# cxzheng/sprsolve

Hardware: AMD Instinct MI355X
Metric: BiCGStab iterations/s (f64, 50M-row 7-point 3-D Poisson) + CSR SpMV GB/s vs HBM roofline (higher is better)
Workload: dtype f64

## Files before the change

sprsolve_amd/csrc/bicg_fuse.hpp:

```cpp
#pragma once
#include "fused_launch.hpp"
#include "krylov.hpp"

namespace sprs {

template <class T, class V, bool PC>
struct BicgK1 {
    BicgState<T> *S; const Real<T> *partN; const T *partRho; int P; int mode;
    const T *v; const T *r; T *p; const V *dinv; T *y;
    T a, beta;
    unsigned int tag = 0; unsigned long long mb_timeout = 0;
    __device__ __forceinline__ bool prologue() {
        __shared__ Real<T> smD[NWAVE];
        __shared__ T smT[NWAVE];
        const int status = S->status;
        const Real<T> tol2 = S->tol2, r0_norm_tol = S->r0_norm_tol;
        const T w = S->w, rho_old = S->rho_old, alpha = S->alpha;
        T rho; Real<T> r_norm;
        if (mode == 0) {
            Real<T> sN; T sR;
            if (tag != 0) {
                if (status != ST_RUNNING) return false;
                if (!mbox_sum2(MboxSrc{reinterpret_cast<const unsigned long long *>(partN), P, tag, mb_timeout}, sN, sR)) {
                    if (first_thread()) S->status = ST_COMM_TIMEOUT;
                    return false;
                }
            } else {
                reduce_partials2(partN, partRho, P, smD, smT, sN, sR);
                if (status != ST_RUNNING) return false;
            }
            r_norm = ssqrt(sN);
            if (r_norm <= tol2) {
                if (first_thread()) { S->r_norm = r_norm; S->status = ST_CONVERGED; }
                return false;
            }
            rho = sR;
            if (sabs(rho) < r0_norm_tol) {
                if (first_thread()) { S->r_norm = r_norm; S->status = ST_RESTART; }
                return false;
            }
        } else {
            if (status != ST_RUNNING) return false;
            rho = S->rho; r_norm = S->r_norm;
        }
        beta = smul(sdiv(rho, rho_old), sdiv(alpha, w));
        a = smul(sneg(beta), w);
        if (first_thread()) { S->rho = rho; S->r_norm = r_norm; S->beta = beta; }
        return true;
    }
    template <int PK, bool NT> __device__ __forceinline__ void run(int64_t i) const {
        auto vv = ldp<T, PK, NT>(v, i); auto pv = ldp<T, PK, NT>(p, i); auto rv = ldp<T, PK, NT>(r, i);
        Pack<T, PK> yv;
        [[maybe_unused]] Pack<V, PK> dv;
        if (PC) dv = ldp<V, PK, NT>(dinv, i);
#pragma unroll
        for (int e = 0; e < PK; ++e) {
            T t = sadd(smul(vv.v[e], a), smul(pv.v[e], beta));
            t = sadd(t, smul(rv.v[e], sone<T>()));
            pv.v[e] = t;
            if (PC) yv.v[e] = smulv(t, dv.v[e]);
        }
        stp<T, PK, NT>(p, i, pv);
        if (PC) stp<T, PK, NT>(y, i, yv);
    }
    __device__ __forceinline__ void epilogue() const {}
};

template <class T, class V, bool PC>
struct BicgK3 {
    BicgState<T> *S; const T *partB; int P; int check_breakdown;
    const T *v; T *r; const V *dinv; T *z;
    T na;
    unsigned int tag = 0; unsigned long long mb_timeout = 0;
    __device__ __forceinline__ bool prologue() {
        __shared__ T smT[NWAVE];
        const int status = S->status;
        const T rho = S->rho;
        T tmp;
        if (tag != 0) {
            if (status != ST_RUNNING) return false;
            if (!mbox_sum1(MboxSrc{reinterpret_cast<const unsigned long long *>(partB), P, tag, mb_timeout}, tmp)) {
                if (first_thread()) S->status = ST_COMM_TIMEOUT;
                return false;
            }
        } else {
            tmp = reduce_partials(partB, P, smT);
            if (status != ST_RUNNING) return false;
        }
        if (check_breakdown && sabs(tmp) <= 0.0) {
            if (first_thread()) S->status = ST_BREAKDOWN;
            return false;
        }
        const T alpha = sdiv(rho, tmp);
        na = sneg(alpha);
        if (first_thread()) S->alpha = alpha;
        return true;
    }
    template <int PK, bool NT> __device__ __forceinline__ void run(int64_t i) const {
        auto vv = ldp<T, PK, NT>(v, i); auto rv = ldp<T, PK, NT>(r, i);
        Pack<T, PK> zv;
        [[maybe_unused]] Pack<V, PK> dv;
        if (PC) dv = ldp<V, PK, NT>(dinv, i);
#pragma unroll
        for (int e = 0; e < PK; ++e) {
            rv.v[e] = sadd(rv.v[e], smul(vv.v[e], na));
            if (PC) zv.v[e] = smulv(rv.v[e], dv.v[e]);
        }
        stp<T, PK, NT>(r, i, rv);
        if (PC) stp<T, PK, NT>(z, i, zv);
    }
    __device__ __forceinline__ void epilogue() const {}
};

int launch_chain_k4f(const sprs_csr *A, const SpmvRoute &rt, const BicgK3<double, double, false> &pro, const double *r, const double *v, double *s_out,
                     double *t, double *partTT, double *partTR, const int *status);
int launch_chain_k2f(const sprs_csr *A, const SpmvRoute &rt, const BicgK1<double, double, false> &pro, const double *v_old, const double *p, const double *r,
                     double *p_out, double *v_out, const double *r0, double *partB, const int *status);

template <class T, bool PC, bool SV = false>
struct BicgK5 {
    BicgState<T> *S; const T *partTT; const T *partTR; int P;
    const T *y; const T *z; const T *t; const T *r0; T *x; T *r; Real<T> *partN; T *partRho;
    Fin fin;
    T na, nw, w;
    Real<T> accN; T accR;
    unsigned int tag = 0; unsigned long long mb_timeout = 0;
    const T *sv = nullptr;
    __device__ __forceinline__ bool prologue() {
        __shared__ T smT[NWAVE];
        __shared__ T smT2[NWAVE];
        const int status = S->status;
        const T alpha = S->alpha;
        T tt, tr;
        if (tag != 0) {
            if (status != ST_RUNNING) { fin_idle(fin, true); return false; }
            if (!mbox_sum2(MboxSrc{reinterpret_cast<const unsigned long long *>(partTT), P, tag, mb_timeout}, tt, tr)) {
                if (first_thread()) S->status = ST_COMM_TIMEOUT;
                return false;
            }
        } else {
            reduce_partials2(partTT, partTR, P, smT, smT2, tt, tr);
        }
        if (status != ST_RUNNING) { fin_idle(fin, true); return false; }
        w = (sre(tt) > 0.0) ? sdiv(tr, tt) : szero<T>();
        na = sneg(alpha); nw = sneg(w);
        accN = 0.0; accR = szero<T>();
        return true;
    }
    template <int PK, bool NT> __device__ __forceinline__ void run(int64_t i) {
        auto xv = ldp<T, PK, NT>(x, i); auto yv = ldp<T, PK, NT>(y, i); auto rv = ldp<T, PK, NT>(r, i);
        auto tv = ldp<T, PK, NT>(t, i); auto qv = ldp<T, PK, NT>(r0, i);
        [[maybe_unused]] Pack<T, PK> zv;
        if (PC) zv = ldp<T, PK, NT>(z, i);
        if constexpr (SV) {
            const auto vv = ldp<T, PK, NT>(sv, i);
#pragma unroll
            for (int e = 0; e < PK; ++e) rv.v[e] = sadd(rv.v[e], smul(vv.v[e], na));
        }
#pragma unroll
        for (int e = 0; e < PK; ++e) {
            T xx = sadd(xv.v[e], smul(yv.v[e], na));
            xx = sadd(xx, smul(PC ? zv.v[e] : rv.v[e], nw));
            xv.v[e] = xx;
            const T rr = sadd(rv.v[e], smul(tv.v[e], nw));
            rv.v[e] = rr;
            accN = accN + ssq(rr);
            accR = sadd(accR, smul(sconj(qv.v[e]), rr));
        }
        stp<T, PK, NT>(x, i, xv);
        stp<T, PK, NT>(r, i, rv);
    }
    __device__ __forceinline__ void epilogue() {
        __shared__ Real<T> smD[NWAVE];
        __shared__ T smT[NWAVE];
        const Real<T> sN = block_sum(accN, smD);
        const T sR = block_sum(accR, smT);
        if (threadIdx.x == 0) { st_partial(fin, partN + blockIdx.x, sN); st_partial(fin, partRho + blockIdx.x, sR); }
        if (first_thread()) { S->w = w; S->rho_old = S->rho; S->its = S->its + 1; }
        if (fin.counter) finalize_last_block<Real<T>, T>(fin, true, smD, smT);
    }
};

}
```

sprsolve_amd/csrc/capi.hip:

```cpp
#include <sys/mman.h>

#include <cstdlib>
#include <memory>
#include <new>
#include <string>

#include "krylov.hpp"

using namespace sprs;

static_assert(sizeof(sprs_c64) == sizeof(cplx), "Complex<f64> layout");
static_assert(sizeof(sprs_c32) == sizeof(cplxf), "Complex<f32> layout");

#define SPRS_GUARD_BEGIN try {
#define SPRS_GUARD_END                         \
    }                                          \
    catch (const std::bad_alloc &) {           \
        return SPRS_ERR_HIP;                   \
    }                                          \
    catch (...) {                              \
        return SPRS_ERR_HIP;                   \
    }

extern "C" {
// ... 445 lines not shown
    h->dtype = dtype_of<T>::value;
    auto *s = new S<T>();
    h->impl = s;
    int st = mk(s);
    if (st != SPRS_OK) { s->destroy(); delete s; delete h; return st; }
    *out = h;
    return SPRS_OK;
}

template <template <class> class S>
int solver_destroy(sprs_solver_handle *h) {
    if (!h) return SPRS_OK;
    with_solver<S>(h->dtype, h->impl, [](auto *s) { (void)hipStreamSynchronize(s->ctx->stream); s->destroy(); delete s; return (int)SPRS_OK; });
    delete h;
    return SPRS_OK;
}

template <class T, class SolverT>
int solve(SolverT *s, bool host, const sprs_diag *P, const T *rhs, size_t rl, T *x, size_t xl, size_t max_iter, Real<T> tol,
          size_t *its, Real<T> *res) {
    if (!s || !rhs || !x) return SPRS_INVALID_ARGUMENT;
    if (rl != s->n) return SPRS_INCOMPATIBLE_RHS_SIZE;
    if (xl != s->n) return SPRS_INCOMPATIBLE_X_SIZE;
    sprs_ctx *c = s->ctx;
    CtxLock lock(c);
    if (!host && ((reinterpret_cast<uintptr_t>(rhs) | reinterpret_cast<uintptr_t>(x)) & 15) == 0)
        return s->solve_dev(P, rhs, rl, x, xl, max_iter, tol, its, res);
    const hipMemcpyKind in = host ? hipMemcpyHostToDevice : hipMemcpyDeviceToDevice, out = host ? hipMemcpyDeviceToHost : hipMemcpyDeviceToDevice;
    SPRS_HIP_TRY(c, hipSetDevice(c->device));
    if (!s->rhs_buf) SPRS_HIP_TRY(c, hipMalloc((void **)&s->rhs_buf, sizeof(T) * s->stride));
    if (!s->x_buf) SPRS_HIP_TRY(c, hipMalloc((void **)&s->x_buf, sizeof(T) * s->stride));
    SPRS_HIP_TRY(c, hipMemcpyAsync(s->rhs_buf, rhs, sizeof(T) * rl, in, c->stream));
    SPRS_HIP_TRY(c, hipMemcpyAsync(s->x_buf, x, sizeof(T) * xl, in, c->stream));
    int st = s->solve_dev(P, s->rhs_buf, rl, s->x_buf, xl, max_iter, tol, its, res);
    if (st >= SPRS_ERR_HIP) return st;
    SPRS_HIP_TRY(c, hipMemcpyAsync(x, s->x_buf, sizeof(T) * xl, out, c->stream));
    SPRS_HIP_TRY(c, hipStreamSynchronize(c->stream));
    return st;
}

template <class T>
int solve_many(CgMany<T> *s, bool host, const sprs_diag *P, const T *rhs, size_t rl, T *x, size_t xl, size_t k, size_t max_iter,
               Real<T> tol, size_t *its, Real<T> *res, int *status) {
    if (!s || !rhs || !x) return SPRS_INVALID_ARGUMENT;
    if (k < 1 || k > (size_t)s->kmax) return SPRS_INVALID_ARGUMENT;
    if (rl != s->n * k) return SPRS_INCOMPATIBLE_RHS_SIZE;
    if (xl != s->n * k) return SPRS_INCOMPATIBLE_X_SIZE;
    sprs_ctx *c = s->ctx;
    CtxLock lock(c);
    if (!host) return s->solve_dev(P, rhs, rl, x, xl, k, max_iter, tol, its, res, status);
    SPRS_HIP_TRY(c, hipSetDevice(c->device));
    const size_t cap = (s->n * (size_t)s->kmax) + 1;
    if (!s->rhs_buf) SPRS_HIP_TRY(c, hipMalloc((void **)&s->rhs_buf, sizeof(T) * cap));
    if (!s->x_buf) SPRS_HIP_TRY(c, hipMalloc((void **)&s->x_buf, sizeof(T) * cap));
    SPRS_HIP_TRY(c, hipMemcpyAsync(s->rhs_buf, rhs, sizeof(T) * rl, hipMemcpyHostToDevice, c->stream));
    SPRS_HIP_TRY(c, hipMemcpyAsync(s->x_buf, x, sizeof(T) * xl, hipMemcpyHostToDevice, c->stream));
    int st = s->solve_dev(P, s->rhs_buf, rl, s->x_buf, xl, k, max_iter, tol, its, res, status);
    if (st >= SPRS_ERR_HIP || st == SPRS_DIM_MISMATCH || st == SPRS_INVALID_ARGUMENT) return st;
    SPRS_HIP_TRY(c, hipMemcpyAsync(x, s->x_buf, sizeof(T) * xl, hipMemcpyDeviceToHost, c->stream));
    SPRS_HIP_TRY(c, hipStreamSynchronize(c->stream));
    return st;
}

template <template <class> class S, class T>
S<T> *impl_of(sprs_solver_handle *h) { return (h && h->dtype == dtype_of<T>::value) ? (S<T> *)h->impl : nullptr; }

}

template <class F>
static int with_base(void *solver, int kind, F &&f) {
    auto *h = (sprs_solver_handle *)solver;
    if (!h) return SPRS_INVALID_ARGUMENT;
    switch (kind) {
        case SPRS_SOLVER_BICGSTAB: return with_solver<BicgStab>(h->dtype, h->impl, f);
        case SPRS_SOLVER_CG: return with_solver<Cg>(h->dtype, h->impl, f);
        case SPRS_SOLVER_GMRES: return with_solver<Gmres>(h->dtype, h->impl, f);
        case SPRS_SOLVER_MINRES:
        case SPRS_SOLVER_CSMINRES: return with_solver<MinRes>(h->dtype, h->impl, f);
    }
    return SPRS_INVALID_ARGUMENT;
}


#define SPRS_CHK(c) do { if (!(c)) return SPRS_INVALID_ARGUMENT; } while (0)
#define SPRS_G(...) try { __VA_ARGS__ } catch (...) { return SPRS_ERR_HIP; }

extern "C" {

int sprs_csr_destroy(sprs_csr *A) {
    if (!A) return SPRS_OK;
    if (A->ctx) { (void)hipSetDevice(A->ctx->device); (void)hipStreamSynchronize(A->ctx->stream); }
    if (A->owns_arrays) {
        if (A->row_ptr) (void)hipFree(A->row_ptr);
        if (A->col_idx) (void)hipFree(A->col_idx);
        if (A->val) (void)hipFree(A->val);
    }
    if (A->rowblk) (void)hipFree(A->rowblk);
    if (A->blk_desc) (void)hipFree(A->blk_desc);
    if (A->blk_desc_eq) (void)hipFree(A->blk_desc_eq);
    if (A->tail) (void)hipFree(A->tail);
    free_dict(A);
    if (A->x_tmp) (void)hipFree(A->x_tmp);
    if (A->y_tmp) (void)hipFree(A->y_tmp);
    if (A->part) (void)hipFree(A->part);
    if (A->dist) {
        if (A->dist->send_idx) (void)hipFree(A->dist->send_idx);
        if (A->dist->send_buf) (void)hipFree(A->dist->send_buf);
        if (A->dist->ag_buf) (void)hipFree(A->dist->ag_buf);
        if (A->dist->order_int) (void)hipFree(A->dist->order_int);
        if (A->dist->order_bnd) (void)hipFree(A->dist->order_bnd);
        for (void *q : {(void *)A->dist->tile_int.list, (void *)A->dist->tile_int.xstart, (void *)A->dist->tile_int.left}) if (q) (void)hipFree(q);
        if (A->dist->order_int_w) (void)hipFree(A->dist->order_int_w);
        if (A->dist->order_bnd_w) (void)hipFree(A->dist->order_bnd_w);
        if (A->dist->ev_pack) (void)hipEventDestroy(A->dist->ev_pack);
        if (A->dist->ev_halo) (void)hipEventDestroy(A->dist->ev_halo);
        if (A->dist->comm_stream) (void)hipStreamDestroy(A->dist->comm_stream);
        delete A->dist;
    }
    delete A;
    return SPRS_OK;
}
int64_t sprs_csr_rows(const sprs_csr *A) { return A ? A->nrows : -1; }
int64_t sprs_csr_cols(const sprs_csr *A) { return A ? A->ncols : -1; }
int64_t sprs_csr_nnz(const sprs_csr *A) { return A ? A->nnz : -1; }
int sprs_csr_wide_blocks(const sprs_csr *A, int64_t *n_blocks, int64_t *n_uniform) {
    if (!A || !n_blocks || !n_uniform) return SPRS_INVALID_ARGUMENT;
    *n_blocks = 0; *n_uniform = 0;
    const SpmvRoute r = spmv_route(A, SpmvPart::Whole, false);
    if (r.format == 0) {
        *n_blocks = A->n_rowblk; *n_uniform = A->blk_desc_eq ? A->n_eq_blocks : 0;
        return SPRS_OK;
    }
    const sprs_dict *D = A->dict;
    const bool one_line = r.format == 2 && D->wide_desc && (A->nrows < 2 || A->ncols < 2) && A->ctx->spmv_wide != 0;
    const bool wide = (D->wide_desc && r.desc == D->wide_desc) || one_line;
    const void *src = wide ? D->wide_desc : (D->off_desc && r.desc == D->off_desc ? D->off_desc : nullptr);
    const int64_t nb = wide ? D->n_wide : (src ? A->n_rowblk : 0);
    if (!src || nb == 0) return SPRS_OK;
    sprs_ctx *c = A->ctx;
    CtxLock lock(c);
    std::vector<int32_t> d((size_t)nb * 4);
    SPRS_HIP_TRY(c, hipSetDevice(c->device));
    SPRS_HIP_TRY(c, hipMemcpyAsync(d.data(), src, d.size() * sizeof(int32_t), hipMemcpyDeviceToHost, c->stream));
    SPRS_HIP_TRY(c, hipStreamSynchronize(c->stream));
    *n_blocks = nb;
    for (int64_t j = 0; j < nb; ++j) *n_uniform += ((uint32_t)d[(size_t)j * 4 + 1] & sprs::UNI2) != 0;
    return SPRS_OK;
}
int sprs_csr_tile_plan(const sprs_csr *A, int64_t *n_tiles, int64_t *n_tile_blocks, int64_t *n_other_blocks) {
    if (!A || !n_tiles || !n_tile_blocks || !n_other_blocks) return SPRS_INVALID_ARGUMENT;
    *n_tiles = 0; *n_tile_blocks = 0; *n_other_blocks = 0;
    const bool split = A->dist && A->dist->order_int;
    const SpmvRoute r = spmv_route(A, split ? SpmvPart::Interior : SpmvPart::Whole, false);
    if (r.kernel != SpmvKernel::TilePair && r.kernel != SpmvKernel::TileOff) return SPRS_OK;
    const sprs_tile_plan &TP = *r.tile;
    *n_tiles = TP.n_tile; *n_tile_blocks = (int64_t)TP.n_tile * sprs::tile_blocks();
    if (split) *n_other_blocks = (A->n_rowblk + 1) / 2 - *n_tile_blocks;
    else *n_other_blocks = r.kernel == SpmvKernel::TilePair ? TP.n_left : (TP.n_left + 1) / 2;
    return SPRS_OK;
}
int sprs_csr_chain_plan(const sprs_csr *A, int64_t *n_tiles, int64_t *n_segments, int64_t *n_chains, int64_t *n_other_blocks) {
    if (!A || !n_tiles || !n_segments || !n_chains || !n_other_blocks) return SPRS_INVALID_ARGUMENT;
    *n_tiles = 0; *n_segments = 0; *n_chains = 0; *n_other_blocks = 0;
    const SpmvRoute r = spmv_route(A, SpmvPart::Whole, false);
    if (r.kernel != SpmvKernel::Chain) return SPRS_OK;
    *n_tiles = r.chain->n_tile; *n_segments = r.chain->n_seg; *n_chains = r.chain->n_chain; *n_other_blocks = r.chain->n_left;
    return SPRS_OK;
}
int sprs_csr_spmv_route(const sprs_csr *A, int part, int conj_x, int *kernel, int *format, int *grid, int64_t *n_blocks,
                        int *ordered, int *y_nt) {
    if (!A || part < 0 || part > 2 || !kernel || !format || !grid || !n_blocks || !ordered || !y_nt) return SPRS_INVALID_ARGUMENT;
    *kernel = -1; *format = 0; *grid = 0; *n_blocks = 0; *ordered = 0; *y_nt = 0;
    if (part != 0 && !(A->dist && A->dist->order_int)) return SPRS_OK;
    const SpmvRoute r = spmv_route(A, part == 0 ? SpmvPart::Whole : part == 1 ? SpmvPart::Interior : SpmvPart::Boundary, conj_x != 0);
    *kernel = (int)r.kernel; *format = r.format; *grid = r.grid; *n_blocks = r.count; *ordered = r.order ? 1 : 0; *y_nt = r.y_nt ? 1 : 0;
    return SPRS_OK;
}
int sprs_csr_stream_format(const sprs_csr *A, int *n_offsets, int *n_values) {
    if (!A) return -1;
    if (n_offsets) *n_offsets = A->dict ? A->dict->n_off : 0;
    if (n_values) *n_values = A->dict ? (A->dict->n_pair ? A->dict->n_pair : 0) : 0;
    return spmv_route(A, SpmvPart::Whole, false).format;
}

int sprs_diag_precond_destroy(sprs_diag *P) {
    if (!P) return SPRS_OK;
    if (P->ctx) { (void)hipSetDevice(P->ctx->device); (void)hipStreamSynchronize(P->ctx->stream); }
    if (P->dinv) (void)hipFree(P->dinv);
    if (P->in_tmp) (void)hipFree(P->in_tmp);
    if (P->out_tmp) (void)hipFree(P->out_tmp);
    delete P;
    return SPRS_OK;
}
int sprs_bicgstab_destroy(sprs_bicgstab *S) { return solver_destroy<BicgStab>(S); }
int sprs_minres_destroy(sprs_minres *S) { return solver_destroy<MinRes>(S); }
int sprs_csminres_destroy(sprs_csminres *S) { return solver_destroy<MinRes>(S); }
int sprs_cg_destroy(sprs_cg *S) { return solver_destroy<Cg>(S); }
int sprs_gmres_destroy(sprs_gmres *S) { return solver_destroy<Gmres>(S); }
int sprs_cgmany_destroy(sprs_cg_many *S) { return solver_destroy<CgMany>(S); }

#define SPRS_SOLVER_SOLVES(X, T, CT, R, NAME, S)                                                                       \
    int sprs_##NAME##_solve_##X(sprs_##NAME *h, const CT *rhs, size_t rl, CT *x, size_t xl, size_t mi, R tol, size_t *its, R *res) { \
        SPRS_G(return solve<T>(impl_of<S, T>(h), true, nullptr, (const T *)rhs, rl, (T *)x, xl, mi, tol, its, res);)   \
    }                                                                                                                  \
    int sprs_##NAME##_precond_solve_##X(sprs_##NAME *h, const sprs_diag *P, const CT *rhs, size_t rl, CT *x, size_t xl, size_t mi, R tol, size_t *its, R *res) { \
        SPRS_G(if (!P) return SPRS_INVALID_ARGUMENT; return solve<T>(impl_of<S, T>(h), true, P, (const T *)rhs, rl, (T *)x, xl, mi, tol, its, res);) \
    }                                                                                                                  \
    int sprs_##NAME##_solve_dev_##X(sprs_##NAME *h, const sprs_diag *P, const CT *rhs, size_t rl, CT *x, size_t xl, size_t mi, R tol, size_t *its, R *res) { \
        SPRS_G(return solve<T>(impl_of<S, T>(h), false, P, (const T *)rhs, rl, (T *)x, xl, mi, tol, its, res);)        \
    }
#define SPRS_SOLVER_API(X, T, CT, R, NAME, S, CREATE)                                                                  \
    int sprs_##NAME##_create_##X(const sprs_csr *A, size_t n, sprs_##NAME **out) {                                     \
        SPRS_G(return (solver_create<T, sprs_##NAME, S>(A, n, out, [&](auto *s) { return s->create CREATE; }));)       \
    }                                                                                                                  \
    SPRS_SOLVER_SOLVES(X, T, CT, R, NAME, S)

#define SPRS_API(X, T, CT, R)                                                                                          \
    int sprs_csr_create_##X(sprs_ctx *c, int64_t nr, int64_t nc, int64_t nnz, const int32_t *rp, const int32_t *ci,    \
                            const CT *v, int csc, sprs_csr **out) {                                                    \
        SPRS_G(return csr_create_host<T, int32_t>(c, nr, nc, nnz, rp, ci, (const T *)v, csc, out);)                    \
    }                                                                                                                  \
    int sprs_csr_create_i64_##X(sprs_ctx *c, int64_t nr, int64_t nc, int64_t nnz, const int64_t *rp,                   \
                                const int64_t *ci, const CT *v, int csc, sprs_csr **out) {                             \
        SPRS_G(return csr_create_host<T, int64_t>(c, nr, nc, nnz, rp, ci, (const T *)v, csc, out);)                    \
    }                                                                                                                  \
    int sprs_csr_create_dev_##X(sprs_ctx *c, int64_t nr, int64_t nc, int64_t nnz, const int32_t *rp,                   \
                                const int32_t *ci, const CT *v, int adopt, sprs_csr **out) {                           \
        SPRS_G(return csr_create_dev<T>(c, nr, nc, nnz, rp, ci, (const T *)v, adopt, out);)                            \
    }                                                                                                                  \
    int sprs_mul_vec_##X(const sprs_csr *A, const CT *x, size_t xl, CT *y, size_t yl) {                                \
        SPRS_G(return mul_vec_host<T>(A, (const T *)x, xl, (T *)y, yl, nullptr);)                                      \
    }                                                                                                                  \
    int sprs_mul_vec_dot_##X(const sprs_csr *A, const CT *x, size_t xl, CT *y, size_t yl, CT *d) {                     \
        SPRS_G(if (!d) return SPRS_INVALID_ARGUMENT; return mul_vec_host<T>(A, (const T *)x, xl, (T *)y, yl, (T *)d);) \
    }                                                                                                                  \
    int sprs_mul_vec_dev_##X(const sprs_csr *A, const CT *x, CT *y) { return mul_vec_dev<T>(A, (const T *)x, (T *)y, nullptr); } \
    int sprs_mul_vec_dot_dev_##X(const sprs_csr *A, const CT *x, CT *y, CT *d) {                                       \
        if (!d) return SPRS_INVALID_ARGUMENT;                                                                          \
        return mul_vec_dev<T>(A, (const T *)x, (T *)y, (T *)d);                                                        \
    }                                                                                                                  \
    int sprs_mul_vec_dev_timed_##X(const sprs_csr *A, const CT *x, CT *y, int reps, double *ms) {                      \
        return mul_vec_timed<T>(A, (const T *)x, (T *)y, reps, ms);                                                    \
    }                                                                                                                  \
    int sprs_mul_mat_##X(const sprs_csr *A, const CT *x, size_t xl, CT *y, size_t yl, size_t k) {                      \
        SPRS_G(return mul_mat_host<T>(A, (const T *)x, xl, (T *)y, yl, k);)                                            \
    }                                                                                                                  \
    int sprs_mul_mat_dev_##X(const sprs_csr *A, const CT *x, CT *y, size_t k) { return mul_mat_dev<T>(A, (const T *)x, (T *)y, k); } \
                                                               \
    int sprs_cgmany_create_##X(const sprs_csr *A, size_t n, size_t k, sprs_cg_many **out) {                           \
        SPRS_G(if (k < 1 || k > 8) { if (out) *out = nullptr; return SPRS_INVALID_ARGUMENT; }                          \
               return (solver_create<T, sprs_cg_many, CgMany>(A, n, out, [&](auto *s) { return s->create(A, n, k); }));) \
    }                                                                                                                  \
    int sprs_cgmany_solve_##X(sprs_cg_many *h, const sprs_diag *P, const CT *rhs, size_t rl, CT *x, size_t xl, size_t k, size_t mi, R tol, \
                               size_t *its, R *res, int *status) {                                                     \
        SPRS_G(return solve_many<T>(impl_of<CgMany, T>(h), true, P, (const T *)rhs, rl, (T *)x, xl, k, mi, tol, its, res, status);) \
    }                                                                                                                  \
    int sprs_cgmany_solve_dev_##X(sprs_cg_many *h, const sprs_diag *P, const CT *rhs, size_t rl, CT *x, size_t xl, size_t k, size_t mi, R tol, \
                                   size_t *its, R *res, int *status) {                                                 \
        SPRS_G(return solve_many<T>(impl_of<CgMany, T>(h), false, P, (const T *)rhs, rl, (T *)x, xl, k, mi, tol, its, res, status);) \
    }                                                                                                                  \
    int sprs_dot_##X(sprs_ctx *c, size_t n, const CT *x, const CT *y, CT *o) { SPRS_CHK(c && o); return dot_host<T>(c, n, (const T *)x, (const T *)y, false, (T *)o); } \
    int sprs_conj_dot_##X(sprs_ctx *c, size_t n, const CT *x, const CT *y, CT *o) { SPRS_CHK(c && o); return dot_host<T>(c, n, (const T *)x, (const T *)y, true, (T *)o); } \
    int sprs_norm2_##X(sprs_ctx *c, size_t n, const CT *x, R *o) { SPRS_CHK(c && o); return norm2_host<T>(c, n, (const T *)x, o); } \
    int sprs_scale_##X(sprs_ctx *c, size_t n, CT a, CT *x) { SPRS_CHK(c); T aa; memcpy(&aa, &a, sizeof(T)); return launch_scale<T>(c, n, aa, (T *)x); } \
    int sprs_rscale_##X(sprs_ctx *c, size_t n, R a, CT *x) { SPRS_CHK(c); return launch_rscale<T>(c, n, a, (T *)x); }  \
    int sprs_conj_##X(sprs_ctx *c, size_t n, const CT *in, CT *out) { SPRS_CHK(c); return launch_conj<T>(c, n, (const T *)in, (T *)out); } \
    int sprs_axpy_##X(sprs_ctx *c, size_t n, CT a, const CT *x, CT *y) { SPRS_CHK(c); T aa; memcpy(&aa, &a, sizeof(T)); return launch_axpy<T, T>(c, n, aa, (const T *)x, (T *)y); } \
    int sprs_axpby_##X(sprs_ctx *c, size_t n, CT a, const CT *x, CT b, CT *y) {                                        \
        SPRS_CHK(c); T aa, bb; memcpy(&aa, &a, sizeof(T)); memcpy(&bb, &b, sizeof(T));                                 \
        return launch_axpby<T>(c, n, aa, (const T *)x, bb, (T *)y);                                                    \
    }                                                                                                                  \
    int sprs_diag_mul_vec_##X(const sprs_diag *P, const CT *in, size_t il, CT *out, size_t ol) {                       \
        SPRS_G(return diag_apply_host<T>(P, (const T *)in, il, (T *)out, ol);)                                         \
    }                                                                                                                  \
    int sprs_diag_mul_vec_dev_##X(const sprs_diag *P, const CT *in, CT *out) { return diag_apply_dev<T>(P, (const T *)in, (T *)out); } \
    SPRS_SOLVER_API(X, T, CT, R, bicgstab, BicgStab, (A, n))                                                           \
    SPRS_SOLVER_API(X, T, CT, R, minres, MinRes, (A, n, false))                                                        \
    SPRS_SOLVER_API(X, T, CT, R, cg, Cg, (A, n))                                                                       \
                                                                  \
    int sprs_gmres_create_##X(const sprs_csr *A, size_t n, size_t restart, sprs_gmres **out) {                         \
        SPRS_G(if (restart > SPRS_GMRES_MAX_RESTART) return SPRS_INVALID_ARGUMENT;                                     \
               return (solver_create<T, sprs_gmres, Gmres>(A, n, out, [&](auto *s) { return s->create(A, n, restart); }));) \
    }                                                                                                                  \
    SPRS_SOLVER_SOLVES(X, T, CT, R, gmres, Gmres)                                                                      \
                                                                      \
    int sprs_csminres_create_##X(const sprs_csr *A, size_t n, sprs_csminres **out) {                                   \
        SPRS_G(return (solver_create<T, sprs_csminres, MinRes>(A, n, out, [&](auto *s) { return s->create(A, n, true); }));) \
    }                                                                                                                  \
    int sprs_csminres_solve_##X(sprs_csminres *h, const CT *rhs, size_t rl, CT *x, size_t xl, size_t mi, R tol, size_t *its, R *res) { \
        SPRS_G(return solve<T>(impl_of<MinRes, T>(h), true, nullptr, (const T *)rhs, rl, (T *)x, xl, mi, tol, its, res);) \
    }                                                                                                                  \
    int sprs_csminres_solve_dev_##X(sprs_csminres *h, const CT *rhs, size_t rl, CT *x, size_t xl, size_t mi, R tol, size_t *its, R *res) { \
        SPRS_G(return solve<T>(impl_of<MinRes, T>(h), false, nullptr, (const T *)rhs, rl, (T *)x, xl, mi, tol, its, res);) \
    }

SPRS_API(d, double, double, double)
SPRS_API(z, cplx, sprs_c64, double)
SPRS_API(s, float, float, float)
SPRS_API(c, cplxf, sprs_c32, float)

int sprs_axpy_zd(sprs_ctx *c, size_t n, double a, const sprs_c64 *x, sprs_c64 *y) { SPRS_CHK(c); return launch_axpy<cplx, double>(c, n, a, (const cplx *)x, (cplx *)y); }
int sprs_axpy_cs(sprs_ctx *c, size_t n, float a, const sprs_c32 *x, sprs_c32 *y) { SPRS_CHK(c); return launch_axpy<cplxf, float>(c, n, a, (const cplxf *)x, (cplxf *)y); }

int sprs_diag_precond_create_d(sprs_ctx *c, size_t n, const double *d, sprs_diag **out) { SPRS_G(return diag_create<double>(c, n, d, DT_D, out);) }
int sprs_diag_precond_create_zd(sprs_ctx *c, size_t n, const double *d, sprs_diag **out) { SPRS_G(return diag_create<double>(c, n, d, DT_Z, out);) }
int sprs_diag_precond_create_z(sprs_ctx *c, size_t n, const sprs_c64 *d, sprs_diag **out) { SPRS_G(return diag_create<cplx>(c, n, (const cplx *)d, DT_Z, out);) }
int sprs_diag_precond_create_s(sprs_ctx *c, size_t n, const float *d, sprs_diag **out) { SPRS_G(return diag_create<float>(c, n, d, DT_S, out);) }
int sprs_diag_precond_create_cs(sprs_ctx *c, size_t n, const float *d, sprs_diag **out) { SPRS_G(return diag_create<float>(c, n, d, DT_C, out);) }
int sprs_diag_precond_create_c(sprs_ctx *c, size_t n, const sprs_c32 *d, sprs_diag **out) { SPRS_G(return diag_create<cplxf>(c, n, (const cplxf *)d, DT_C, out);) }

int sprs_solver_set_mode(void *solver, int kind, int mode) {
    if (mode != 0 && mode != 1) return SPRS_INVALID_ARGUMENT;
    return with_base(solver, kind, [&](auto *b) { b->mode = mode; return (int)SPRS_OK; });
}
int sprs_solver_set_trace(void *solver, int kind, double *trace_host, size_t cap) {
    return with_base(solver, kind, [&](auto *b) { b->trace = trace_host; b->trace_cap = trace_host ? cap : 0; b->trace_rows = 0; return (int)SPRS_OK; });
}
int sprs_solver_trace_rows(const void *solver, int kind, size_t *rows_out) {
    if (!rows_out) return SPRS_INVALID_ARGUMENT;
// ... 35 lines not shown
```

sprsolve_amd/csrc/internal.hpp:

```cpp
#pragma once
#include <hip/hip_runtime.h>
#include <hip/hip_ext.h>
#include <cstdint>
#include <cstdio>
#include <cstring>
#include <cstdlib>
#include <ctime>
#include <mutex>
#include <type_traits>
#include <vector>

#include "../../include/sprsolve_hip.h"
#include "scalar.hpp"

namespace sprs {

constexpr int BLOCK = 256;
constexpr uint32_t UNI2 = 0x40000000u;
constexpr uint32_t SEAM2 = 0x20000000u;
constexpr int MAX_GRID = 4096;

enum : int { ST_RUNNING = 0, ST_CONVERGED = 1, ST_RESTART = 2, ST_BREAKDOWN = 3, ST_INVALID_PC = 4,
             ST_COMM_TIMEOUT = 5 };

// ... 6 lines not shown
    int world, rank;
};

struct Fin {
    unsigned int *counter = nullptr;
    const void *base0 = nullptr, *base1 = nullptr;
    void *out0 = nullptr, *out1 = nullptr;
    int P = 0;
    const P2pBox *box = nullptr;
    unsigned int tag = 0;
    unsigned int mb_off = 0;
};

}

struct sprs_ctx {
    int device = 0;
    hipStream_t stream = nullptr;
    bool own_stream = false;
    int num_cu = 256;
    int grid = 512;
    int spmv_grid = -1;
    int xcd_chunk = -1;
    int spmv_dict = -1;
    int spmv_wide = -1;
    int spmv_wideload = -1;
    int spmv_eqrows = -1;
    int spmv_period = -1;
    int spmv_triple = -1;
    int spmv_seam = -1;
    int spmv_tile = -1;
    int spmv_chain = -1;
    int spmv_fuse = -1;
    int ew_chunk = -1;
    int stream_nt = -1;
    int spmv_uniform = -1;
    int halo_overlap = 1;
    int gs_graph = 0;
    int p2p_allreduce = -1;
    int p2p_timeout_ms = 20000;
    int poll = 16;
    double *d_part = nullptr;
    double *d_scal = nullptr;
    double *h_scal = nullptr;
    mutable char err[512] = {0};
    hipEvent_t prof_start = nullptr, prof_stop = nullptr;
    mutable std::recursive_mutex mu;
};
struct CtxLock {
    std::unique_lock<std::recursive_mutex> lk;
    explicit CtxLock(const sprs_ctx *c) { if (c) lk = std::unique_lock<std::recursive_mutex>(c->mu); }
};

#define SPRS_HIP_TRY(ctx, expr)                                                                     \
    do {                                                                                            \
        hipError_t e__ = (expr);                                                                    \
        if (e__ != hipSuccess) {                                                                    \
            snprintf((ctx)->err, sizeof((ctx)->err), "%s:%d: %s -> %s", __FILE__, __LINE__, #expr,  \
                     hipGetErrorString(e__));                                                       \
            return SPRS_ERR_HIP;                                                                    \
        }                                                                                           \
    } while (0)

#define SPRS_LAUNCH_SPMV(c, kernel, grid, ...)                                                                            \
    do {                                                                                                                 \
        if ((c)->prof_start && (c)->prof_stop)                                                                           \
            hipExtLaunchKernelGGL(kernel, dim3(grid), dim3(sprs::BLOCK), 0, (c)->stream, (c)->prof_start, (c)->prof_stop, 0, __VA_ARGS__); \
        else                                                                                                             \
            hipLaunchKernelGGL(kernel, dim3(grid), dim3(sprs::BLOCK), 0, (c)->stream, __VA_ARGS__);                      \
    } while (0)

struct CreateTrace {
    bool on; double t0;
    static double now() { timespec ts; clock_gettime(CLOCK_MONOTONIC, &ts); return ts.tv_sec * 1e3 + ts.tv_nsec * 1e-6; }
    CreateTrace() : on(getenv("SPRS_CREATE_TRACE") != nullptr), t0(now()) {}
    void lap(const char *what) { if (!on) return; const double t = now(); fprintf(stderr, "[sprs create] %-28s %8.2f ms\n", what, t - t0); t0 = t; }
};

#define SPRS_TRY(expr)                       \
    do {                                     \
        int s__ = (expr);                    \
        if (s__ != SPRS_OK) return s__;      \
    } while (0)

struct sprs_comm {
    sprs_ctx *ctx = nullptr;
    void *nccl = nullptr;
    int world = 1, rank = 0;
    bool p2p = false;
    void *mbox = nullptr;
    void *peer_map[8] = {nullptr};
    sprs::P2pBox *d_box = nullptr;
    unsigned int seq[4] = {0, 0, 0, 0};
};

struct sprs_tile_plan {
    int32_t *list = nullptr;
    int32_t *xstart = nullptr;
    int32_t *left = nullptr;
    int n_tile = 0, n_left = 0;
    int ul = 0, fl = 0, fh = 0;
    int w = 0;
    int32_t off[8] = {0, 0, 0, 0, 0, 0, 0, 0};
    double val[8] = {0, 0, 0, 0, 0, 0, 0, 0};
    std::vector<int32_t> h_list, h_xstart;
};

struct sprs_chain_plan {
    int32_t *tiles = nullptr;
    int32_t *segs = nullptr;
    int32_t *xstart = nullptr;
    int32_t *left = nullptr;
    int n_tile = 0, n_seg = 0, n_chain = 0, n_left = 0;
    int ul = 0, tri = 0;
    int32_t off[8] = {0, 0, 0, 0, 0, 0, 0, 0};
    double val[8] = {0, 0, 0, 0, 0, 0, 0, 0};
};

struct sprs_dist_info {
    sprs_comm *comm = nullptr;
    int64_t n_local = 0, n_ext = 0;
    std::vector<int> peer;
    std::vector<int64_t> send_off, recv_off;
    int32_t *send_idx = nullptr;
    void *send_buf = nullptr;
    int64_t ag_slice = 0;
    void *ag_buf = nullptr;
    int32_t *order_int = nullptr, *order_bnd = nullptr;
    int32_t n_int = 0, n_bnd = 0;
    int32_t *order_int_w = nullptr, *order_bnd_w = nullptr;
    sprs_tile_plan tile_int;
    bool tile_int_off = false;
    int32_t n_int_w = 0, n_bnd_w = 0;
    hipStream_t comm_stream = nullptr;
    hipEvent_t ev_pack = nullptr, ev_halo = nullptr;
};

struct sprs_dict {
    uint8_t *idx_code = nullptr;
    uint8_t *pair_code = nullptr;
    int32_t *off_tab = nullptr;
    int32_t *pair_off = nullptr;
    void *pair_val = nullptr;
    void *rowval = nullptr;
    int n_off = 0, n_val = 0, n_pair = 0;
    void *wide_desc = nullptr;
    int n_wide = 0;
    int32_t *wide_order = nullptr;
    int32_t *off_order = nullptr;
    int64_t period = 0;
    int64_t max_off = -1;
    sprs_tile_plan tile_pair, tile_off;
    sprs_chain_plan chain_pair;
    void *owide_desc = nullptr;
    int n_owide = 0;
    void *off_desc = nullptr;
    int n_off_uniform = 0;
};

struct sprs_csr {
    sprs_ctx *ctx = nullptr;
    int dtype = 0;
    int64_t nrows = 0, ncols = 0, nnz = 0;
    int32_t *row_ptr = nullptr;
    int32_t *col_idx = nullptr;
    void *val = nullptr;
    bool owns_arrays = true;
    bool was_csc = false;
    int32_t *rowblk = nullptr;
    int32_t n_rowblk = 0;
    void *blk_desc = nullptr;
    void *blk_desc_eq = nullptr;
    int32_t n_eq_blocks = 0;
    void *tail = nullptr;
    void *x_tmp = nullptr, *y_tmp = nullptr;
    double *part = nullptr;
    sprs_dist_info *dist = nullptr;
    sprs_dict *dict = nullptr;
};

struct sprs_diag {
    sprs_ctx *ctx = nullptr;
    int t_dtype = 0;
    int v_complex = 0;
    size_t n = 0;
    void *dinv = nullptr;
    void *in_tmp = nullptr, *out_tmp = nullptr;
};

namespace sprs {

enum class SpmvPart { Whole, Interior, Boundary };
enum class SpmvKernel {
    Csr,
    CsrWide,
    Dict,
    DictWide,
    Pair2,
    TilePair,
    TileOff,
    Chain,
};
struct BlkDesc;
struct SpmvRoute {
    SpmvKernel kernel;
    int format;
    int grid;
    int xcd_chunk;
    const BlkDesc *desc;
    const int32_t *order;
    int count;
    const sprs_tile_plan *tile;
    const sprs_chain_plan *chain;
    bool y_nt;
};
SpmvRoute spmv_route(const sprs_csr *A, SpmvPart part, bool conj_x);
template <class T>
int launch_spmv(const sprs_csr *A, SpmvPart part, const T *x, T *y, int dot_mode, const T *u, T *part0, T *part1,
                const int *status, bool conj_x = false, const Fin *fin = nullptr);
int spmv_num_partials(const sprs_csr *A);
template <class F>
inline void with_dot(int dot_mode, bool flag, F &&f) {
    auto go = [&](auto dm) { if (flag) f(dm, std::true_type{}); else f(dm, std::false_type{}); };
    if (dot_mode == 0) go(std::integral_constant<int, 0>{});
    else if (dot_mode == 1) go(std::integral_constant<int, 1>{});
    else go(std::integral_constant<int, 2>{});
}
int tile_blocks();
int build_rowblocks(sprs_csr *A, const int32_t *host_row_ptr);
int validate_cols_device(const sprs_csr *A);
int rowblk_spans(const sprs_csr *A, std::vector<int32_t> &lo, std::vector<int32_t> &hi);
int build_dict(sprs_csr *A, bool has_vector_blocks, const std::vector<int32_t> &blk, const std::vector<int32_t> &blk_pa);
void free_dict(sprs_csr *A);
bool fused_chunked(const sprs_csr *A);
template <class T>
int launch_dict(const sprs_csr *A, const SpmvRoute &r, const T *x, T *y, int dot_mode, const T *u, T *part0, T *part1,
                const int *status, bool conj_x, const Fin &fin);
int launch_dict_wide(const sprs_csr *A, const SpmvRoute &r, const double *x, double *y, int dot_mode, const double *u,
                     double *part0, double *part1, const int *status, const Fin &fin);
int launch_pair2(const sprs_csr *A, const SpmvRoute &r, const double *x, double *y, int dot_mode, const double *u,
                 double *part0, double *part1, const int *status, const Fin &fin);
int launch_tile_pair(const sprs_csr *A, const SpmvRoute &r, const double *x, double *y, int dot_mode, const double *u,
                     double *part0, double *part1, const int *status, const Fin &fin);
int launch_tile_off(const sprs_csr *A, const SpmvRoute &r, const double *x, double *y, int dot_mode, const double *u,
                    double *part0, double *part1, const int *status, const Fin &fin);
int launch_chain_pair(const sprs_csr *A, const SpmvRoute &r, const double *x, double *y, int dot_mode, const double *u,
                      double *part0, double *part1, const int *status, const Fin &fin);

template <class T>
int launch_spmm(const sprs_csr *A, const T *x, T *y, int ld, int k, int dot_mode, const T *u, T *part, const int *running);
int spmm_grid(const sprs_csr *A);

template <class T, class S> int launch_axpy(sprs_ctx *c, size_t n, S a, const T *x, T *y);
template <class T> int launch_axpby(sprs_ctx *c, size_t n, T a, const T *x, T b, T *y);
template <class T> int launch_scale(sprs_ctx *c, size_t n, T a, T *x);
template <class T> int launch_rscale(sprs_ctx *c, size_t n, Real<T> a, T *x);
template <class T> int launch_conj(sprs_ctx *c, size_t n, const T *in, T *out);
template <class T, class V> int launch_diag_apply(sprs_ctx *c, size_t n, const V *dinv, const T *in, T *out);
template <class V> int launch_diag_inv(sprs_ctx *c, size_t n, const V *diag, V *dinv);
template <class T> int dot_host(sprs_ctx *c, size_t n, const T *x, const T *y, bool conj, T *out, sprs_comm *comm = nullptr);
template <class T> int norm2_host(sprs_ctx *c, size_t n, const T *x, Real<T> *out, sprs_comm *comm = nullptr);
template <class T> int reduce_partials_host(sprs_ctx *c, const T *part, int P, T *out, sprs_comm *comm = nullptr);

template <class T> int halo_exchange(const sprs_csr *A, T *x_ext);
template <class T> int halo_begin(const sprs_csr *A, T *x_ext);
int halo_wait(const sprs_csr *A);
template <class T>
int dist_spmv(const sprs_csr *A, T *x_ext, T *y, int dot_mode, const T *u, T *part0, T *part1, const int *status, bool conj_x,
              const Fin *fin = nullptr);
int allreduce_sum(sprs_comm *comm, void *dev, size_t count, bool f32 = false);

inline int grid_for(const sprs_ctx *c) {
    int g = c->grid;
    if (g < 8) g = 8;
    if (g > MAX_GRID) g = MAX_GRID;
    return g & ~7;
}

inline bool stream_loads_nt(const sprs_ctx *c, size_t vector_bytes) {
    if (c->stream_nt >= 0) return c->stream_nt != 0;
    return vector_bytes >= (size_t)72 << 20;
}
inline bool is_cache_resident(const sprs_csr *A) {
    const double s = (double)dtype_size(A->dtype);
    return (double)A->nnz * (s + 4) + 3.0 * A->nrows * s < 192.0 * 1024 * 1024;
}

inline bool tile_wanted(const sprs_ctx *c, size_t vector_bytes) {
    if (c->spmv_tile >= 0) return c->spmv_tile != 0;
    return vector_bytes >= (size_t)44 << 20;
}

inline int balanced_grid(const sprs_ctx *c, int64_t work) {
    const int g0 = grid_for(c);
    if (work <= g0) return (int)(work < 1 ? 1 : work);
    const int64_t trips = (work + g0 - 1) / g0;
    int64_t g = (work + trips - 1) / trips;
    g = (g + 7) & ~(int64_t)7;
    return (int)(g > g0 ? g0 : g);
}

}
```

sprsolve_amd/csrc/spmv.hip:

```cpp
#include <algorithm>
#include <memory>
#include <system_error>
#include <thread>

#include "device.hpp"

namespace sprs {

struct BlkDescHost { int32_t ra, rb, pa, nn; };

template <class F>
static void host_parallel_for(int64_t n, int64_t min_chunk, F &&f) {
    auto call = [&](int64_t a, int64_t b, int t) {
        if constexpr (std::is_invocable_v<F, int64_t, int64_t, int>) f(a, b, t); else f(a, b);
    };
    int64_t T = std::min<int64_t>(std::max(1u, std::thread::hardware_concurrency()), 16);
    T = std::max<int64_t>(1, std::min<int64_t>(T, n / std::max<int64_t>(min_chunk, 1)));
    if (T <= 1) { call(0, n, 0); return; }
    std::vector<std::thread> th;
    const int64_t per = (n + T - 1) / T;
    for (int64_t t = 0; t < T; ++t) {
        const int64_t a = t * per, b = std::min<int64_t>(n, a + per);
        if (a >= b) break;
        try { th.emplace_back(call, a, b, (int)t); } catch (const std::system_error &) { call(a, b, (int)t); }
// ... 367 lines not shown
    for (; b < bend; b += bstep) {
        const BlkDesc d = desc[order ? order[b] : b];
        if (run_state != ST_RUNNING) { fin_idle(fin, DOT == 2); return; }
        const bool eq_rows = eq_desc != 0 && ((uint32_t)d.rb & UNI2) != 0;
        const int ra = d.ra, rb = d.rb & (eq_desc ? 0x3fffffff : 0x7fffffff);
        if (d.rb >= 0) {
            const int pa = d.pa, nn = eq_desc ? (d.nn & 0xffff) : d.nn;
            const int shift = pa & 3, tot = nn + shift;
            const int r = ra + lane;
            const bool has_row = r < rb;
            const int rcl = has_row ? r : rb - 1;
            int s, e;
            if (eq_rows) { const int L = d.nn >> 16; s = (rcl - ra) * L; e = s + L; }
            else { s = row_ptr[rcl] - pa; e = row_ptr[rcl + 1] - pa; }
            [[maybe_unused]] T uu;
            if (DOT != 0) uu = u[rcl];
            if (nn > 0) {
                const int g0 = (pa - shift) >> 2, lastq = (tot - 1) >> 2;
                v4i32 c[2]; D2v v[2][2];
#pragma unroll
                for (int i = 0; i < 2; ++i) {
                    const int G = g0 + min(lane + i * WAVE, lastq);
                    const bool tl = G == g_last;
                    const v4i32 *cp = tl ? tail_c : col4 + G;
                    const D2v *vp = tl ? tail_v : val2 + 2 * (int64_t)G;
                    c[i] = *cp; v[i][0] = vp[0]; v[i][1] = vp[1];
                }
                T xg[8];
#pragma unroll
                for (int i = 0; i < 2; ++i) { xg[4 * i] = x[c[i].x]; xg[4 * i + 1] = x[c[i].y]; xg[4 * i + 2] = x[c[i].z]; xg[4 * i + 3] = x[c[i].w]; }
#pragma unroll
                for (int i = 0; i < 2; ++i) {
                    const int k = 4 * (lane + i * WAVE);
                    const D2v p0{xg[4 * i] * v[i][0].a, xg[4 * i + 1] * v[i][0].b}, p1{xg[4 * i + 2] * v[i][1].a, xg[4 * i + 3] * v[i][1].b};
                    if (k < tot) { *reinterpret_cast<D2v *>(prod + k) = p0; *reinterpret_cast<D2v *>(prod + k + 2) = p1; }
                }
            }
            wave_lds_fence();
            if (has_row) {
                T acc = 0.0;
                const int len = e - s;
                const T *pr = prod + shift;
                if (len <= 8) {
                    T pv[8];
#pragma unroll
                    for (int j = 0; j < 8; ++j) pv[j] = pr[min(s + j, CAP + 3)];
#pragma unroll
                    for (int j = 0; j < 8; ++j)
                        if (j < len) acc = acc + pv[j];
                } else {
                    for (int k = s; k < e; ++k) acc = acc + pr[k];
                }
                if constexpr (YNT) __builtin_nontemporal_store(acc, y + r);
                else y[r] = acc;
                if (DOT == 1) d0 = d0 + uu * acc;
                if (DOT == 2) { d0 = d0 + acc * acc; d1 = d1 + acc * uu; }
            }
            wave_lds_fence();
        } else {
            const int r = ra;
            const int s = row_ptr[r], e = row_ptr[r + 1];
            T acc = 0.0;
            for (int k = s + lane; k < e; k += WAVE) { const int cj = col_idx[k]; const T vj = val[k]; acc = acc + x[cj] * vj; }
            acc = wave_sum(acc);
            if (lane == 0) {
                y[r] = acc;
                if (DOT == 1) d0 = d0 + u[r] * acc;
                if (DOT == 2) { d0 = d0 + acc * acc; d1 = d1 + acc * u[r]; }
            }
        }
    }
    if (run_state != ST_RUNNING) { fin_idle(fin, DOT == 2); return; }
    if (DOT >= 1) {
        d0 = block_sum(d0, red);
        if (tid == 0) st_partial(fin, part0 + blockIdx.x, d0);
    }
    if (DOT == 2) {
        d1 = block_sum(d1, red);
        if (tid == 0) st_partial(fin, part1 + blockIdx.x, d1);
    }
    if (DOT >= 1 && fin.counter) finalize_last_block<T, T>(fin, DOT == 2, red, red);
}

__global__ __launch_bounds__(BLOCK) void rowblk_span_kernel(int n_rowblk, const int32_t *__restrict__ rowblk,
                                                            const int32_t *__restrict__ row_ptr,
                                                            const int32_t *__restrict__ col_idx, int32_t *__restrict__ lo,
                                                            int32_t *__restrict__ hi) {
    const int lane = threadIdx.x & (WAVE - 1);
    for (int b = blockIdx.x * NWAVE + (threadIdx.x >> 6); b < n_rowblk; b += gridDim.x * NWAVE) {
        const int ra = (int)((uint32_t)rowblk[b] & ~VEC_FLAG), rb = (int)((uint32_t)rowblk[b + 1] & ~VEC_FLAG);
        const int pa = row_ptr[ra], pb = row_ptr[rb];
        int mn = INT32_MAX, mx = -1;
        for (int k = pa + lane; k < pb; k += WAVE) { const int cidx = col_idx[k]; mn = min(mn, cidx); mx = max(mx, cidx); }
        for (int off = WAVE / 2; off > 0; off >>= 1) { mn = min(mn, __shfl_down(mn, off, WAVE)); mx = max(mx, __shfl_down(mx, off, WAVE)); }
        if (lane == 0) { lo[b] = mn; hi[b] = mx; }
    }
}

__global__ __launch_bounds__(BLOCK) void validate_cols_kernel(int64_t nnz, const int32_t *__restrict__ col_idx, int32_t ncols,
                                                              int *__restrict__ bad) {
    int local = 0;
    for (int64_t k = (int64_t)blockIdx.x * BLOCK + threadIdx.x; k < nnz; k += (int64_t)gridDim.x * BLOCK) {
        const int32_t cidx = col_idx[k];
        local |= (cidx < 0) | (cidx >= ncols);
    }
    if (local) atomicOr(bad, 1);
}
int validate_cols_device(const sprs_csr *A) {
    sprs_ctx *c = A->ctx;
    if (A->nnz == 0) return SPRS_OK;
    CtxLock lock(c);
    int *d_bad = reinterpret_cast<int *>(c->d_scal);
    SPRS_HIP_TRY(c, hipMemsetAsync(d_bad, 0, sizeof(int), c->stream));
    const int g = (int)std::min<int64_t>((A->nnz + BLOCK - 1) / BLOCK, 2048);
    hipLaunchKernelGGL(validate_cols_kernel, dim3(g), dim3(BLOCK), 0, c->stream, A->nnz, A->col_idx, (int32_t)A->ncols, d_bad);
    SPRS_HIP_TRY(c, hipGetLastError());
    int bad = 0;
    SPRS_HIP_TRY(c, hipMemcpyAsync(&bad, d_bad, sizeof(int), hipMemcpyDeviceToHost, c->stream));
    SPRS_HIP_TRY(c, hipStreamSynchronize(c->stream));
    return bad ? SPRS_INVALID_ARGUMENT : SPRS_OK;
}

int rowblk_spans(const sprs_csr *A, std::vector<int32_t> &lo, std::vector<int32_t> &hi) {
    sprs_ctx *c = A->ctx;
    const int nb = A->n_rowblk;
    lo.assign((size_t)nb, INT32_MAX); hi.assign((size_t)nb, -1);
    if (nb == 0) return SPRS_OK;
    int32_t *d_lo = nullptr, *d_hi = nullptr;
    SPRS_HIP_TRY(c, hipMalloc((void **)&d_lo, sizeof(int32_t) * nb));
    SPRS_HIP_TRY(c, hipMalloc((void **)&d_hi, sizeof(int32_t) * nb));
    const int g = std::max(1, std::min(2048, (nb + NWAVE - 1) / NWAVE));
    hipLaunchKernelGGL(rowblk_span_kernel, dim3(g), dim3(BLOCK), 0, c->stream, nb, A->rowblk, A->row_ptr, A->col_idx, d_lo, d_hi);
    hipError_t e1 = hipMemcpyAsync(lo.data(), d_lo, sizeof(int32_t) * nb, hipMemcpyDeviceToHost, c->stream);
    hipError_t e2 = hipMemcpyAsync(hi.data(), d_hi, sizeof(int32_t) * nb, hipMemcpyDeviceToHost, c->stream);
    hipError_t e3 = hipStreamSynchronize(c->stream);
    (void)hipFree(d_lo); (void)hipFree(d_hi);
    SPRS_HIP_TRY(c, e1); SPRS_HIP_TRY(c, e2); SPRS_HIP_TRY(c, e3);
    return SPRS_OK;
}

SpmvRoute spmv_route(const sprs_csr *A, SpmvPart part, bool conj_x) {
    const sprs_ctx *c = A->ctx;
    const sprs_dict *D = A->dict;
    const sprs_dist_info *P = A->dist;
    const bool whole = part == SpmvPart::Whole, f64 = A->dtype == DT_D;
    const bool wide = c->spmv_wide != 0, uni = c->spmv_uniform != 0, tiles = c->spmv_tile != 0 && wide;
    const bool wideload = A->tail != nullptr && c->spmv_wideload != 0;
    SpmvRoute r{};
    if (D && c->spmv_dict != 0 && (uint64_t)std::max(A->ncols, A->nrows + 1) * std::max<size_t>(dtype_size(A->dtype), 4) < (1ull << 32)) {
        if (D->pair_code && c->spmv_dict != 1) r.format = 2;
        else if (c->spmv_dict != -1 || !dtype_is_complex(A->dtype)) r.format = 1;
    }
    const bool pair = r.format == 2;
    const sprs_chain_plan *chain = pair && !P && c->spmv_chain != 0 && tiles && uni && D->chain_pair.n_tile > 0 ? &D->chain_pair : nullptr;
    const sprs_tile_plan *tile = !tiles ? nullptr
                               : pair ? (D->tile_pair.n_tile > 0 ? &D->tile_pair : nullptr)
                               : (r.format == 1 && wideload && uni && D->tile_off.n_tile > 0 ? &D->tile_off : nullptr);

    int g = c->spmv_grid;
    if (g <= 0) {
        if (chain) {
            g = c->num_cu * 2;
        } else {
            g = c->num_cu * ((r.format == 0 && wideload && !is_cache_resident(A)) ? 3 : 4);
            if (tile) g = std::min(g, std::max(64, (tile->n_tile / 3) & ~7));
        }
    }
    g = std::min(std::max(g, 8), MAX_GRID / 2) & ~7;
    r.order = whole ? nullptr : part == SpmvPart::Interior ? P->order_int : P->order_bnd;
    r.count = whole ? A->n_rowblk : part == SpmvPart::Interior ? P->n_int : P->n_bnd;
    const int need = std::max(8, (((r.count + NWAVE - 1) / NWAVE + 7) / 8) * 8);
    r.grid = std::min(g, need);
    r.xcd_chunk = c->xcd_chunk < 0 ? (is_cache_resident(A) ? 1 : 0) : c->xcd_chunk;
    r.y_nt = stream_loads_nt(c, (size_t)A->nrows * dtype_size(A->dtype));

    if (r.format == 0) {
        r.kernel = f64 && wideload ? SpmvKernel::CsrWide : SpmvKernel::Csr;
        r.desc = reinterpret_cast<const BlkDesc *>(A->blk_desc_eq ? A->blk_desc_eq : A->blk_desc);
        return r;
    }
    if (f64 && whole && c->spmv_period != 0 && D->wide_order) r.xcd_chunk = 0;
    const sprs_tile_plan *tp = whole ? tile : part == SpmvPart::Interior && tiles && P->tile_int.n_tile > 0 && P->tile_int_off == !pair ? &P->tile_int : nullptr;
    if (f64 && pair) {
        r.desc = reinterpret_cast<const BlkDesc *>(D->wide_desc);
        if (chain && whole) { r.kernel = SpmvKernel::Chain; r.chain = chain; return r; }
        if (tp) { r.kernel = SpmvKernel::TilePair; r.tile = tp; return r; }
        const int32_t *order_w = whole ? (c->spmv_period != 0 ? D->wide_order : nullptr) : part == SpmvPart::Interior ? P->order_int_w : P->order_bnd_w;
        if (D->wide_desc && wide && (whole || order_w) && A->nrows >= 2 && A->ncols >= 2) {
            r.kernel = SpmvKernel::Pair2;
            r.order = order_w;
            r.count = whole ? D->n_wide : part == SpmvPart::Interior ? P->n_int_w : P->n_bnd_w;
            return r;
        }
    }
    if (!pair && whole && c->spmv_period > 0 && D->off_order) { r.order = D->off_order; r.xcd_chunk = 0; }
    r.desc = reinterpret_cast<const BlkDesc *>((!pair && D->off_desc && uni) ? D->off_desc : A->blk_desc);
    r.kernel = SpmvKernel::Dict;
    if (f64 && !pair && wideload) {
        r.kernel = SpmvKernel::DictWide;
        if (tp && D->owide_desc && uni && !conj_x) { r.kernel = SpmvKernel::TileOff; r.tile = tp; }
    }
    return r;
}

bool fused_chunked(const sprs_csr *A) {
    const sprs_ctx *c = A->ctx;
    if (c->ew_chunk >= 0) return c->ew_chunk != 0;
    if (A->dist || c->xcd_chunk == 0 || !is_cache_resident(A)) return false;
    return A->dict && A->dict->max_off >= 0 && A->dict->max_off * 32 <= (int64_t)A->nrows;
}

template <class T>
int launch_spmv(const sprs_csr *A, SpmvPart part, const T *x, T *y, int dot_mode, const T *u, T *part0, T *part1,
                const int *status, bool conj_x, const Fin *finp) {
    const Fin fin = (finp && dot_mode != 0) ? *finp : Fin{};
    const SpmvRoute r = spmv_route(A, part, conj_x);
    sprs_ctx *c = A->ctx;
    const T *v = reinterpret_cast<const T *>(A->val);
    const int eq = A->blk_desc_eq ? 1 : 0;
    if constexpr (dtype_of<T>::value == DT_D) {
        switch (r.kernel) {
            case SpmvKernel::CsrWide: {
                const v4i32 *tc = reinterpret_cast<const v4i32 *>(A->tail);
                const D2v *tv = reinterpret_cast<const D2v *>(reinterpret_cast<const char *>(A->tail) + 16);
                const int g_last = (int)((A->nnz - 1) >> 2);
                with_dot(dot_mode, r.y_nt, [&](auto dm, auto ynt) {
                    SPRS_LAUNCH_SPMV(c, (spmv_wide_kernel<decltype(dm)::value, decltype(ynt)::value>), r.grid, r.count, r.xcd_chunk, eq, r.desc,
                                     r.order, A->row_ptr, A->col_idx, v, tc, tv, g_last, x, y, u, part0, part1, status, fin);
                });
                SPRS_HIP_TRY(c, hipGetLastError());
                return SPRS_OK;
            }
            case SpmvKernel::DictWide: return launch_dict_wide(A, r, x, y, dot_mode, u, part0, part1, status, fin);
            case SpmvKernel::Pair2: return launch_pair2(A, r, x, y, dot_mode, u, part0, part1, status, fin);
            case SpmvKernel::TilePair: return launch_tile_pair(A, r, x, y, dot_mode, u, part0, part1, status, fin);
            case SpmvKernel::TileOff: return launch_tile_off(A, r, x, y, dot_mode, u, part0, part1, status, fin);
            case SpmvKernel::Chain: return launch_chain_pair(A, r, x, y, dot_mode, u, part0, part1, status, fin);
            default: break;
        }
    }
    if (r.kernel == SpmvKernel::Dict) return launch_dict<T>(A, r, x, y, dot_mode, u, part0, part1, status, conj_x, fin);
    if (r.kernel != SpmvKernel::Csr) return SPRS_INVALID_ARGUMENT;
    with_dot(dot_mode, conj_x && is_complex<T>::value, [&](auto dm, auto cj) {
        SPRS_LAUNCH_SPMV(c, (spmv_kernel<T, decltype(dm)::value, decltype(cj)::value>), r.grid, r.count, r.xcd_chunk, eq, r.desc, r.order,
                         A->row_ptr, A->col_idx, v, x, y, u, part0, part1, status, fin);
    });
    SPRS_HIP_TRY(c, hipGetLastError());
    return SPRS_OK;
}

int spmv_num_partials(const sprs_csr *A) {
    if (A->dist && A->dist->order_int)
        return spmv_route(A, SpmvPart::Interior, false).grid + spmv_route(A, SpmvPart::Boundary, false).grid;
    return spmv_route(A, SpmvPart::Whole, false).grid;
}

#define SPRS_INST_SPMV(T) \
    template int launch_spmv<T>(const sprs_csr *, SpmvPart, const T *, T *, int, const T *, T *, T *, const int *, bool, const Fin *);
SPRS_INST_SPMV(double)
SPRS_INST_SPMV(cplx)
SPRS_INST_SPMV(float)
SPRS_INST_SPMV(cplxf)

}
```

sprsolve_amd/csrc/spmv_chain.hip:

```cpp
#include "spmv_dict_dev.hpp"
#include "bicg_fuse.hpp"

namespace sprs {
namespace {

constexpr int CH_ROWS = CH_B * 2 * WAVE;
constexpr int CH_W = TILE_W;
constexpr int CH_WL = CH_ROWS + 2 * CH_W;

struct NoPro { __device__ __forceinline__ bool prologue() { return true; } };
template <int FUSE, class PRO, int DOT, bool UX, int UL, bool TRI>
__global__ __launch_bounds__(BLOCK) void spmv_chain_kernel(const int4 *__restrict__ tiles, const int2 *__restrict__ segs, const int32_t *__restrict__ xstart,
                                                           const BlkDesc *__restrict__ desc, const TilePat pat,
                                                           int n_left, const int32_t *__restrict__ left_order,
                                                           const int32_t *__restrict__ row_ptr, const uint8_t *__restrict__ code,
                                                           const int32_t *__restrict__ off_tab, const double *__restrict__ val_tab,
                                                           const double *__restrict__ x, double *__restrict__ y, const double *__restrict__ u,
                                                           double *__restrict__ part0, double *__restrict__ part1,
                                                           const int *__restrict__ status, int nrows, int ncols, const Fin fin,
                                                           PRO pro, const double *__restrict__ in1, const double *__restrict__ in2,
                                                           double *__restrict__ own) {
    using T = double;
    constexpr int NV = FUSE == 0 ? 1 : FUSE;
    static_assert(FUSE == 0 || (FUSE == 2 && DOT == 2 && UX) || (FUSE == 3 && DOT == 1 && !UX), "fused flavours: K3 into K4, K1 into K2");
// ... 90 lines not shown
                for (int q = 0; q < NQ; ++q) {
                    const u4v w4 = __builtin_nontemporal_load(reinterpret_cast<const u4v *>(u + (ts + ((q * NWAVE + wv) << 7) + 2 * lane)));
                    __builtin_memcpy(&uu[q], &w4, 16);
                }
            }
            T opl[UL], oph[UL], ux0 = 0.0, ux1 = 0.0;
            auto read_ops = [&](int q) {
                const int l = ((q * NWAVE + wv) << 7) + 2 * lane;
                const D2 f0 = *reinterpret_cast<const D2 *>(wp + l), f1 = *reinterpret_cast<const D2 *>(wn + l);
                opl[0] = f0.lo; oph[0] = f0.hi; opl[UL - 1] = f1.lo; oph[UL - 1] = f1.hi;
                if constexpr (TRI) {
#pragma unroll
                    for (int t = 0; t < NN; ++t) {
                        if (t == TC - 1 || t == TC + 1) continue;
                        const D2 v2 = *reinterpret_cast<const D2 *>(wc + l + pat.off[1 + t]);
                        opl[1 + t] = v2.lo; oph[1 + t] = v2.hi;
                    }
                    if constexpr (NN >= 3) {
                        const int oc = pat.off[1 + TC];
                        opl[TC] = wc[l + oc - 1]; oph[TC] = opl[1 + TC];
                        opl[2 + TC] = oph[1 + TC]; oph[2 + TC] = wc[l + oc + 2];
                    }
                } else {
#pragma unroll
                    for (int t = 0; t < NN; ++t) { opl[1 + t] = wc[l + pat.off[1 + t]]; oph[1 + t] = wc[l + pat.off[1 + t] + 1]; }
                }
                if ((DOT != 0 && UX) || FUSE != 0) { const D2 c2 = *reinterpret_cast<const D2 *>(wc + l); ux0 = c2.lo; ux1 = c2.hi; }
            };
            read_ops(0);
#pragma unroll
            for (int q = 0; q < NQ; ++q) {
                const uint32_t rbq = (uint32_t)__builtin_amdgcn_readfirstlane((int)rbc[q]);
                const bool seam = (rbq & SEAM2) != 0;
                T pl[UL], ph[UL];
#pragma unroll
                for (int t = 0; t < UL; ++t) { pl[t] = opl[t]; ph[t] = oph[t]; }
                const T u0 = (DOT != 0 && !UX) ? uu[q].lo : ux0, u1 = (DOT != 0 && !UX) ? uu[q].hi : ux1;
                [[maybe_unused]] const D2 mine{ux0, ux1};
                if (q + 1 < NQ) read_ops(q + 1);
                T acc0 = 0.0, acc1 = 0.0;
                if (!seam) {
#pragma unroll
                    for (int t = 0; t < UL; ++t) {
                        acc0 = acc0 + pl[t] * pat.val[t];
                        acc1 = acc1 + ph[t] * pat.val[t];
                    }
                } else {
                    const int seam1 = __builtin_amdgcn_readfirstlane(nnc[q]) >> 16, seam2 = (int)(rbq & 0x3ffffffu);
                    const int kk = seam1 & 127, maskA = (seam1 >> 7) & 255, maskB = seam2 & 255;
                    const bool a0 = 2 * lane == kk, a1 = 2 * lane + 1 == kk, b0s = 2 * lane == kk + 1, b1s = 2 * lane + 1 == kk + 1;
                    if ((seam2 & 0x3000000) == 0) {
#pragma unroll
                        for (int t = 0; t < UL; ++t) {
                            const bool am = ((maskA >> t) & 1) == 0, bm = ((maskB >> t) & 1) == 0;
                            const T n0 = acc0 + pl[t] * pat.val[t], n1 = acc1 + ph[t] * pat.val[t];
                            if (!am && !bm) { acc0 = n0; acc1 = n1; }
                            else {
                                acc0 = ((am && a0) || (bm && b0s)) ? acc0 : n0;
                                acc1 = ((am && a1) || (bm && b1s)) ? acc1 : n1;
                            }
                        }
                    } else {
                        const T valA = s_pair[(seam2 >> 8) & 255].val, valB = s_pair[(seam2 >> 16) & 255].val;
                        const bool ovA = ((seam2 >> 24) & 1) != 0, ovB = ((seam2 >> 25) & 1) != 0;
                        const int pm0 = a0 ? maskA : (b0s ? maskB : 255), pm1 = a1 ? maskA : (b1s ? maskB : 255);
                        const bool o0 = (a0 && ovA) || (b0s && ovB), o1 = (a1 && ovA) || (b1s && ovB);
                        const T v0 = a0 ? valA : valB, v1 = a1 ? valA : valB;
#pragma unroll
                        for (int t = 0; t < UL; ++t) {
                            const T n0 = acc0 + pl[t] * (o0 ? v0 : pat.val[t]), n1 = acc1 + ph[t] * (o1 ? v1 : pat.val[t]);
                            acc0 = ((pm0 >> t) & 1) ? n0 : acc0;
                            acc1 = ((pm1 >> t) & 1) ? n1 : acc1;
                        }
                    }
                }
                const D2 yy{acc0, acc1};
                u4v qv;
                __builtin_memcpy(&qv, &yy, 16);
                __builtin_nontemporal_store(qv, reinterpret_cast<u4v *>(y + (ts + ((q * NWAVE + wv) << 7) + 2 * lane)));
                if constexpr (FUSE == 3) {
                    u4v ov;
                    __builtin_memcpy(&ov, &mine, 16);
                    __builtin_nontemporal_store(ov, reinterpret_cast<u4v *>(own + (ts + ((q * NWAVE + wv) << 7) + 2 * lane)));
                }
                if (DOT == 1) { d0 = d0 + u0 * acc0; d0 = d0 + u1 * acc1; }
                if (DOT == 2) { d0 = d0 + acc0 * acc0; d1 = d1 + acc0 * u0; d0 = d0 + acc1 * acc1; d1 = d1 + acc1 * u1; }
            }
            __syncthreads();
            ts_prev = ts;
            const int o = sp; sp = sc; sc = sn; sn = o;
        };
        if constexpr (PF == 2) {
            for (int k = 0; k < L; k += 2) { body(k, R0); if (k + 1 < L) body(k + 1, R1); }
        } else {
            for (int k = 0; k < L; ++k) body(k, R0);
        }
    }
    if (n_left > 0) {
        __syncthreads();
        uint32_t (*s_c)[CW2] = reinterpret_cast<uint32_t (*)[CW2]>(&win[0][0]);
        for (int i = lane; i < CW2; i += WAVE) s_c[wv][i] = 0;
        if constexpr (FUSE == 0)
            pair2_walk<DOT, true>(n_left, 0, desc, left_order, row_ptr, code, XPlain{reinterpret_cast<const char *>(x)}, y, u, nrows, ncols, s_pair, s_c, d0, d1);
        else
            pair2_walk<DOT, true, XFused<NV>>(n_left, 0, desc, left_order, row_ptr, code,
                                              XFused<NV>{reinterpret_cast<const char *>(x), reinterpret_cast<const char *>(in1), reinterpret_cast<const char *>(in2), c0, c1},
                                              y, UX ? nullptr : u, nrows, ncols, s_pair, s_c, d0, d1, own);
    }
    if (DOT >= 1) {
        d0 = block_sum(d0, red);
        if (tid == 0) st_partial(fin, part0 + blockIdx.x, d0);
    }
    if (DOT == 2) {
        d1 = block_sum(d1, red);
        if (tid == 0) st_partial(fin, part1 + blockIdx.x, d1);
    }
    if (DOT >= 1 && fin.counter) finalize_last_block<T, T>(fin, DOT == 2, red, red);
}

}

int chain_rows() { return CH_ROWS; }

int launch_chain_pair(const sprs_csr *A, const SpmvRoute &r, const double *x, double *y, int dot_mode, const double *u,
                      double *part0, double *part1, const int *status, const Fin &fin) {
    sprs_ctx *c = A->ctx;
    const sprs_dict *D = A->dict;
    const sprs_chain_plan &CP = *r.chain;
    const int g = r.grid;
    const BlkDesc *wd = r.desc;
    const double *pvd = reinterpret_cast<const double *>(D->pair_val);
    TilePat tp;
    for (int t = 0; t < 8; ++t) { tp.off[t] = CP.off[t]; tp.val[t] = CP.val[t]; }
    const bool ux = dot_mode != 0 && u == x;
#define SPRS_CSPMV(DM, UXV, U, TR) SPRS_LAUNCH_SPMV(c, (spmv_chain_kernel<0, NoPro, DM, UXV, U, TR>), g, reinterpret_cast<const int4 *>(CP.tiles), reinterpret_cast<const int2 *>(CP.segs), \
                                                    CP.xstart, wd, tp, CP.n_left, CP.left, A->row_ptr, D->pair_code, D->pair_off, pvd, x, y, u, part0, part1, status,   \
                                                    (int)A->nrows, (int)A->ncols, fin, NoPro{}, nullptr, nullptr, nullptr)
#define SPRS_CSHAPE(U, TR)                                                                                           \
    if (CP.ul == U && (CP.tri != 0) == TR) {                                                                         \
        if (dot_mode == 0) SPRS_CSPMV(0, false, U, TR);                                                              \
        else if (dot_mode == 1) { if (ux) SPRS_CSPMV(1, true, U, TR); else SPRS_CSPMV(1, false, U, TR); }            \
        else if (ux) SPRS_CSPMV(2, true, U, TR); else SPRS_CSPMV(2, false, U, TR);                                   \
    }
    SPRS_CHAIN_SHAPES(SPRS_CSHAPE)
#undef SPRS_CSHAPE
#undef SPRS_CSPMV
    SPRS_HIP_TRY(c, hipGetLastError());
    return SPRS_OK;
}


int launch_chain_k4f(const sprs_csr *A, const SpmvRoute &rt, const BicgK3<double, double, false> &pro, const double *r, const double *v, double *s_out,
                     double *t, double *partTT, double *partTR, const int *status) {
    sprs_ctx *c = A->ctx;
    const sprs_dict *D = A->dict;
    const sprs_chain_plan &CP = *rt.chain;
    const int g = rt.grid;
    const BlkDesc *wd = rt.desc;
    const double *pvd = reinterpret_cast<const double *>(D->pair_val);
    TilePat tp;
    for (int k = 0; k < 8; ++k) { tp.off[k] = CP.off[k]; tp.val[k] = CP.val[k]; }
    typedef BicgK3<double, double, false> K3;
#define SPRS_C4F(U, TR)                                                                                                 \
    if (CP.ul == U && (CP.tri != 0) == TR)                                                                              \
        SPRS_LAUNCH_SPMV(c, (spmv_chain_kernel<2, K3, 2, true, U, TR>), g, reinterpret_cast<const int4 *>(CP.tiles), reinterpret_cast<const int2 *>(CP.segs), \
                         CP.xstart, wd, tp, CP.n_left, CP.left, A->row_ptr, D->pair_code, D->pair_off, pvd, r, t, (const double *)nullptr, partTT, partTR, status, \
                         (int)A->nrows, (int)A->ncols, Fin{}, pro, v, (const double *)nullptr, s_out);
    SPRS_CHAIN_SHAPES(SPRS_C4F)
#undef SPRS_C4F
    SPRS_HIP_TRY(c, hipGetLastError());
    return SPRS_OK;
}

int launch_chain_k2f(const sprs_csr *A, const SpmvRoute &rt, const BicgK1<double, double, false> &pro, const double *v_old, const double *p, const double *r,
                     double *p_out, double *v_out, const double *r0, double *partB, const int *status) {
    sprs_ctx *c = A->ctx;
    const sprs_dict *D = A->dict;
    const sprs_chain_plan &CP = *rt.chain;
    const int g = rt.grid;
    const BlkDesc *wd = rt.desc;
    const double *pvd = reinterpret_cast<const double *>(D->pair_val);
    TilePat tp;
    for (int k = 0; k < 8; ++k) { tp.off[k] = CP.off[k]; tp.val[k] = CP.val[k]; }
    typedef BicgK1<double, double, false> K1;
#define SPRS_C2F(U, TR)                                                                                                 \
    if (CP.ul == U && (CP.tri != 0) == TR)                                                                              \
        SPRS_LAUNCH_SPMV(c, (spmv_chain_kernel<3, K1, 1, false, U, TR>), g, reinterpret_cast<const int4 *>(CP.tiles), reinterpret_cast<const int2 *>(CP.segs), \
                         CP.xstart, wd, tp, CP.n_left, CP.left, A->row_ptr, D->pair_code, D->pair_off, pvd, v_old, v_out, r0, partB, (double *)nullptr, status, \
                         (int)A->nrows, (int)A->ncols, Fin{}, pro, p, r, p_out);
    SPRS_CHAIN_SHAPES(SPRS_C2F)
#undef SPRS_C2F
    SPRS_HIP_TRY(c, hipGetLastError());
    return SPRS_OK;
}

}
```

sprsolve_amd/csrc/spmv_dict.hip:

```cpp
#include <algorithm>
#include <cstring>
#include <map>

#include "spmv_dict_dev.hpp"
#include "minres_fuse.hpp"

namespace sprs {

namespace {

constexpr int HSLOTS = 1024;
constexpr uint32_t EMPTY32 = 0x80000000u;
constexpr uint64_t EMPTY64 = 0xFFFFFFFFFFFFFFFFull;

__device__ __forceinline__ uint32_t hash32(uint32_t k) { k ^= k >> 16; k *= 0x7feb352du; k ^= k >> 15; k *= 0x846ca68bu; k ^= k >> 16; return k; }
__device__ __forceinline__ uint32_t hash64(uint64_t k) { k ^= k >> 33; k *= 0xff51afd7ed558ccdull; k ^= k >> 33; return (uint32_t)k; }

__device__ __forceinline__ uint64_t key_of(double v) { return (uint64_t)__double_as_longlong(v); }
__device__ __forceinline__ uint64_t key_of(float v) { return (uint64_t)__float_as_uint(v); }

__device__ __forceinline__ int probe32(uint32_t *tab, int *count, uint32_t key, bool insert) {
    uint32_t h = hash32(key) & (HSLOTS - 1);
    for (int t = 0; t < HSLOTS; ++t, h = (h + 1) & (HSLOTS - 1)) {
        uint32_t cur = __hip_atomic_load(tab + h, __ATOMIC_RELAXED, __HIP_MEMORY_SCOPE_AGENT);
// ... 397 lines not shown
            if (sub) continue;
            mask[h] = 0;
            if (len[h] == 1) {
                const int cd = code[start[h]], o = off_tab[cd];
                for (int q = 0; q < Lmax && mask[h] == 0; ++q) if (off_tab[A[q]] == o) mask[h] = 1 << q;
                if (mask[h] != 0) ovc[h] = cd; else bad = true;
            } else bad = true;
        }
        if (__builtin_amdgcn_ballot_w64(bad) != 0) continue;
        if ((int64_t)d.ra + omin < 0 || (int64_t)d.rb - 1 + omax > (int64_t)ncols - 1) continue;
        const uint64_t e0 = __builtin_amdgcn_ballot_w64(mask[0] != full), e1 = __builtin_amdgcn_ballot_w64(mask[1] != full);
        const int ne = __builtin_popcountll(e0) + __builtin_popcountll(e1);
        if (ne < 1 || ne > 2) continue;
        const int k = e0 ? (int)__builtin_ctzll(e0) : WAVE + (int)__builtin_ctzll(e1);
        const int k1 = k + 1;
        if (ne == 2 && k1 >= 2 * WAVE) continue;
        const int mA = __shfl(k < WAVE ? mask[0] : mask[1], k & (WAVE - 1), WAVE);
        const int cA = __shfl(k < WAVE ? ovc[0] : ovc[1], k & (WAVE - 1), WAVE);
        int mB = full, cB = -1;
        if (k1 < 2 * WAVE) {
            mB = __shfl(k1 < WAVE ? mask[0] : mask[1], k1 & (WAVE - 1), WAVE);
            cB = __shfl(k1 < WAVE ? ovc[0] : ovc[1], k1 & (WAVE - 1), WAVE);
        }
        if (ne == 2 && mB == full) continue;
        if (lane == 0) {
            int centre = 0;
            for (int j = 1; triple != 0 && j + 1 < Lmax && centre == 0; ++j) {
                const int o = off_tab[A[j]];
                if (off_tab[A[j - 1]] == o - 1 && off_tab[A[j + 1]] == o + 1) centre = j;
            }
            const uint32_t mB8 = mB == full ? 0xffu : (uint32_t)mB;
            const uint32_t rbw = UNI2 | SEAM2 | mB8 | ((uint32_t)(cA < 0 ? 0 : cA) << 8) | ((uint32_t)(cB < 0 ? 0 : cB) << 16) |
                                 (cA >= 0 ? 1u << 24 : 0u) | (cB >= 0 ? 1u << 25 : 0u);
            desc[b] = BlkDesc{d.ra, (int32_t)rbw, pA, Lmax | (centre << 8) | (k << 16) | (mA << 23)};
        }
    }
}

template <int DOT, bool YNT>
__global__ __launch_bounds__(BLOCK) void spmv_pair2_kernel(int n_wide, int xcd_chunk, const BlkDesc *__restrict__ desc,
                                                           const int32_t *__restrict__ order,
                                                           const int32_t *__restrict__ row_ptr,
                                                           const uint8_t *__restrict__ code,
                                                           const int32_t *__restrict__ off_tab,
                                                           const double *__restrict__ val_tab, const double *__restrict__ x,
                                                           double *__restrict__ y, const double *__restrict__ u,
                                                           double *__restrict__ part0, double *__restrict__ part1,
                                                           const int *__restrict__ status, int nrows, int ncols, const Fin fin) {
    using T = double;
    __shared__ PairEnt<T> s_pair[TAB];
    __shared__ __attribute__((aligned(16))) uint32_t s_c[NWAVE][CW2];
    __shared__ T red[NWAVE];
    const int run_state = status != nullptr ? *status : (int)ST_RUNNING;

    const int tid = threadIdx.x, lane = tid & (WAVE - 1);
    const int wv = __builtin_amdgcn_readfirstlane(tid >> 6);
    stage_pair(s_pair, tid, off_tab[tid] * 8, val_tab[tid]);
    for (int i = lane; i < CW2; i += WAVE) s_c[wv][i] = 0;
    __syncthreads();
    if (run_state != ST_RUNNING) { fin_idle(fin, DOT == 2); return; }

    T d0 = 0.0, d1 = 0.0;
    pair2_walk<DOT, YNT>(n_wide, xcd_chunk, desc, order, row_ptr, code, XPlain{reinterpret_cast<const char *>(x)}, y, u, nrows, ncols, s_pair, s_c, d0, d1);
    if (DOT >= 1) {
        d0 = block_sum(d0, red);
        if (tid == 0) st_partial(fin, part0 + blockIdx.x, d0);
    }
    if (DOT == 2) {
        d1 = block_sum(d1, red);
        if (tid == 0) st_partial(fin, part1 + blockIdx.x, d1);
    }
    if (DOT >= 1 && fin.counter) finalize_last_block<T, T>(fin, DOT == 2, red, red);
}

__global__ __launch_bounds__(BLOCK) void tile_mark_kernel(int n_cand, const BlkDesc *__restrict__ desc, const uint8_t *__restrict__ code,
                                                          unsigned long long *__restrict__ pat_out, int *__restrict__ len_out) {
    const int t = blockIdx.x * BLOCK + threadIdx.x;
    if (t >= n_cand) return;
    unsigned long long pat0 = 0;
    int L0 = 0, ra0 = 0;
    bool ok = true;
    for (int i = 0; i < TILE_B && ok; ++i) {
        const BlkDesc d = desc[t * TILE_B + i];
        const uint32_t rb = (uint32_t)d.rb;
        ok = (rb & UNI2) != 0;
        if (!ok) break;
        const bool seam = (rb & SEAM2) != 0;
        const int L = d.nn & 0xff;
        const int nr = seam ? 2 * WAVE : (int)(rb & ~UNI2) - d.ra;
        unsigned long long pat = 0;
        for (int j = 0; j < L && j < 8; ++j) pat |= (unsigned long long)code[d.pa + j] << (8 * j);
        if (i == 0) { pat0 = pat; L0 = L; ra0 = d.ra; }
        ok = nr == 2 * WAVE && L == L0 && L >= 1 && L <= 8 && pat == pat0 && d.ra == ra0 + i * 2 * WAVE;
    }
    pat_out[t] = ok ? pat0 : 0ull;
    len_out[t] = ok ? L0 : 0;
}

__global__ __launch_bounds__(BLOCK) void tile_flag_kernel(int n_wide, const BlkDesc *__restrict__ desc, const uint8_t *__restrict__ code,
                                                          unsigned long long pat, int L, uint8_t *__restrict__ flag) {
    const int j = blockIdx.x * BLOCK + threadIdx.x;
    if (j >= n_wide) return;
    const BlkDesc d = desc[j];
    const uint32_t rb = (uint32_t)d.rb;
    bool ok = (rb & UNI2) != 0 && (d.nn & 0xff) == L;
    if (ok) {
        const bool seam = (rb & SEAM2) != 0;
        ok = seam || (int)(rb & ~UNI2) - d.ra == 2 * WAVE;
        unsigned long long p = 0;
        for (int t = 0; t < L && t < 8; ++t) p |= (unsigned long long)code[d.pa + t] << (8 * t);
        ok = ok && p == pat;
    }
    flag[j] = ok ? 1 : 0;
}

template <class FirstRow>
static std::vector<int32_t> xcd_period_order(int nblk, int64_t G, FirstRow first_row) {
    std::vector<std::vector<int32_t>> q(8);
    for (int j = 0; j < nblk; ++j) q[(size_t)((first_row(j) / G) % 8)].push_back(j);
    std::vector<int32_t> ord((size_t)nblk);
    size_t pos[8] = {0, 0, 0, 0, 0, 0, 0, 0}, filled = 0;
    while (filled < (size_t)nblk) {
        for (int x = 0; x < 8 && filled < (size_t)nblk; ++x) {
            for (int k = 0; k < NWAVE && filled < (size_t)nblk; ++k) {
                int src = x;
                if (pos[src] >= q[src].size()) {
                    size_t best = 0;
                    for (int y2 = 0; y2 < 8; ++y2)
                        if (q[y2].size() - pos[y2] > best) { best = q[y2].size() - pos[y2]; src = y2; }
                }
                ord[filled++] = q[src][pos[src]++];
            }
        }
    }
    return ord;
}

static bool tile_shape_built(int ul, int fl, int fh, int w) {
#define SPRS_TILE_HAS(U, L, H) if (ul == U && fl == L && fh == H) return true;
    if (w == TILE_W) { SPRS_TILE_SHAPES(SPRS_TILE_HAS) }
    if (w == TILE_W_WIDE) { SPRS_TILE_SHAPES_WIDE(SPRS_TILE_HAS) }
#undef SPRS_TILE_HAS
    return false;
}

struct BlkDescHost2 { int32_t ra, rb, pa, nn; };
template <class T> struct has_val_dict { static constexpr bool value = false; };
template <> struct has_val_dict<double> { static constexpr bool value = true; };
template <> struct has_val_dict<float> { static constexpr bool value = true; };
template <class T> struct has_pair_codes { static constexpr bool value = has_val_dict<T>::value || is_complex<T>::value; };

template <class MakeLeft>
static int build_chain_plan(sprs_csr *A, sprs_chain_plan &CP, const std::vector<BlkDescHost2> &wd, const std::vector<uint8_t> &flag, int UL,
                            const int32_t *off, const double *val, MakeLeft &&make_left) {
    sprs_ctx *c = A->ctx;
    const int nw = (int)wd.size();
    const int64_t Pf = off[UL - 1];
    if (UL < 3 || UL > 7 || (UL & 1) == 0 || -(int64_t)off[0] != Pf || (Pf & 1) || Pf < 2 * (int64_t)TILE_W) return SPRS_OK;
    for (int t = 1; t + 1 < UL; ++t) if (off[t] < -(TILE_W - 2) || off[t] > TILE_W - 2) return SPRS_OK;
    bool shape_ok = false;
#define SPRS_CH_HAS(U, TR) if (UL == U) shape_ok = true;
    SPRS_CHAIN_SHAPES(SPRS_CH_HAS)
#undef SPRS_CH_HAS
    if (!shape_ok) return SPRS_OK;
    const int CHR = CH_B * 2 * WAVE;
    const int NN = UL - 2, TC = NN / 2;
    bool tri = (off[1 + TC] & 1) == 0;
    for (int t = 0; t < NN && tri; ++t) {
        if (t == TC - 1) tri = off[1 + t] == off[1 + TC] - 1;
        else if (t == TC + 1) tri = off[1 + t] == off[1 + TC] + 1;
        else tri = (off[1 + t] & 1) == 0;
    }
    if (!tri && UL == 3) return SPRS_OK;
    std::vector<int32_t> tb;
    std::vector<char> in_chain((size_t)nw, 0);
    int64_t flagged = 0;
    for (int j = 0; j < nw;) {
        if (!flag[(size_t)j]) { ++j; continue; }
        int e = j + 1;
        while (e < nw && flag[(size_t)e] && wd[(size_t)e].ra == wd[(size_t)e - 1].ra + 2 * WAVE) ++e;
        flagged += e - j;
        for (int b = j; b + CH_B <= e; b += CH_B) {
            const int64_t ra = wd[(size_t)b].ra;
            if (ra - Pf < 0 || ra + CHR + Pf > A->ncols) continue;
            tb.push_back(b);
        }
        j = e;
    }
    const int nt = (int)tb.size();
    if (nt < 64) return SPRS_OK;
    std::vector<int32_t> next((size_t)nt, -1), prev((size_t)nt, -1);
    {
        std::vector<int64_t> ras((size_t)nt);
        for (int i = 0; i < nt; ++i) ras[(size_t)i] = wd[(size_t)tb[(size_t)i]].ra;
        for (int i = 0; i < nt; ++i) {
            const int64_t want = ras[(size_t)i] + Pf;
            const auto it = std::lower_bound(ras.begin(), ras.end(), want - 127);
            if (it == ras.end() || *it > want + 127) continue;
            const int j2 = (int)(it - ras.begin());
            if (prev[(size_t)j2] >= 0) continue;
            next[(size_t)i] = j2; prev[(size_t)j2] = i;
        }
    }
    struct Chain { int head; int len; int64_t col; };
    std::vector<Chain> chains;
    for (int i = 0; i < nt; ++i) {
        if (prev[(size_t)i] >= 0) continue;
        int len = 0;
        for (int q = i; q >= 0; q = next[(size_t)q]) ++len;
        chains.push_back(Chain{i, len, (int64_t)wd[(size_t)tb[(size_t)i]].ra % Pf});
    }
    std::stable_sort(chains.begin(), chains.end(), [](const Chain &a, const Chain &b) { return a.col < b.col; });
    const int nch = (int)chains.size();
    const int G = 2 * c->num_cu;
    std::vector<int32_t> tiles, segs, xstart(9, 0);
    int64_t covered = 0;
    int n_seg = 0;
    for (int xq = 0; xq < 8; ++xq) {
        xstart[(size_t)xq] = n_seg;
        const int c_lo = (int)((int64_t)nch * xq / 8), c_hi = (int)((int64_t)nch * (xq + 1) / 8);
        std::vector<std::vector<std::pair<int, int>>> cs((size_t)(c_hi - c_lo));
        size_t maxq = 0;
        for (int ci = c_lo; ci < c_hi; ++ci) {
            const int len = chains[(size_t)ci].len;
            int q = std::max(1, G / std::max(nch, 1));
            q = std::max(1, std::min(q, len / 8));
            for (int k = 0; k < q; ++k) {
                const int a = (int)((int64_t)len * k / q), b = (int)((int64_t)len * (k + 1) / q);
                if (b > a) cs[(size_t)(ci - c_lo)].push_back({a, b - a});
            }
            maxq = std::max(maxq, cs[(size_t)(ci - c_lo)].size());
        }
        std::vector<std::vector<int32_t>> ids((size_t)(c_hi - c_lo));
        for (int ci = c_lo; ci < c_hi; ++ci)
            for (int q = chains[(size_t)ci].head; q >= 0; q = next[(size_t)q]) ids[(size_t)(ci - c_lo)].push_back(q);
        for (size_t k = 0; k < maxq; ++k)
            for (int ci = c_lo; ci < c_hi; ++ci) {
                const auto &sv = cs[(size_t)(ci - c_lo)];
                if (k >= sv.size()) continue;
                const auto &idv = ids[(size_t)(ci - c_lo)];
                segs.push_back((int32_t)(tiles.size() / 4)); segs.push_back(sv[k].second);
                for (int p2 = sv[k].first; p2 < sv[k].first + sv[k].second; ++p2) {
                    const int ti = idv[(size_t)p2];
                    const int b0 = tb[(size_t)ti];
                    const int32_t ra = wd[(size_t)b0].ra;
                    const int32_t ra_next = next[(size_t)ti] >= 0 ? wd[(size_t)tb[(size_t)next[(size_t)ti]]].ra : (int32_t)(ra + Pf);
                    tiles.push_back(b0); tiles.push_back(ra); tiles.push_back(ra_next); tiles.push_back(0);
                    for (int qb = 0; qb < CH_B; ++qb) in_chain[(size_t)(b0 + qb)] = 1;
                    covered += CH_B;
                }
                ++n_seg;
            }
    }
    xstart[8] = n_seg;
    const int n_tile = (int)(tiles.size() / 4);
    const bool fills = n_seg * 2 >= G && covered * 2 >= flagged && n_tile >= 6 * n_seg;
    if (n_tile == 0 || (c->spmv_chain < 0 && !fills)) return SPRS_OK;
    std::vector<int32_t> left;
    make_left(in_chain, left);
    auto drop = [&]() { for (void *q : {(void *)CP.tiles, (void *)CP.segs, (void *)CP.xstart, (void *)CP.left}) if (q) (void)hipFree(q); CP = sprs_chain_plan(); };
#define CH_TRY(expr) do { hipError_t e__ = (expr); if (e__ != hipSuccess) { snprintf(c->err, sizeof(c->err), "%s:%d: %s -> %s", __FILE__, __LINE__, #expr, hipGetErrorString(e__)); drop(); return SPRS_ERR_HIP; } } while (0)
    CH_TRY(hipMalloc((void **)&CP.tiles, sizeof(int32_t) * tiles.size()));
    CH_TRY(hipMalloc((void **)&CP.segs, sizeof(int32_t) * segs.size()));
    CH_TRY(hipMalloc((void **)&CP.xstart, sizeof(int32_t) * 9));
    CH_TRY(hipMalloc((void **)&CP.left, sizeof(int32_t) * std::max<size_t>(left.size(), 1)));
    CH_TRY(hipMemcpyAsync(CP.tiles, tiles.data(), sizeof(int32_t) * tiles.size(), hipMemcpyHostToDevice, c->stream));
    CH_TRY(hipMemcpyAsync(CP.segs, segs.data(), sizeof(int32_t) * segs.size(), hipMemcpyHostToDevice, c->stream));
    CH_TRY(hipMemcpyAsync(CP.xstart, xstart.data(), sizeof(int32_t) * 9, hipMemcpyHostToDevice, c->stream));
    if (!left.empty()) CH_TRY(hipMemcpyAsync(CP.left, left.data(), sizeof(int32_t) * left.size(), hipMemcpyHostToDevice, c->stream));
    CH_TRY(hipStreamSynchronize(c->stream));
#undef CH_TRY
    CP.n_tile = n_tile; CP.n_seg = n_seg; CP.n_chain = nch; CP.n_left = (int)left.size();
    CP.ul = UL; CP.tri = tri ? 1 : 0;
    for (int t = 0; t < 8; ++t) { CP.off[t] = t < UL ? off[t] : 0; CP.val[t] = t < UL ? val[t] : 0.0; }
    return SPRS_OK;
}

template <class MakeLeft>
static int build_tile_plan(sprs_csr *A, sprs_tile_plan &TP, const BlkDesc *desc_dev, const uint8_t *code_dev, const std::vector<BlkDescHost2> &wd,
                           const int32_t *off_tab, const double *val_tab, bool wide_window_ok, MakeLeft &&make_left, sprs_chain_plan *CP = nullptr) {
    sprs_ctx *c = A->ctx;
    const int nw = (int)wd.size();
    const int n_cand = nw / TILE_B;
    if (!(tile_wanted(c, (size_t)A->nrows * sizeof(double)) && c->spmv_uniform != 0 && c->spmv_wide != 0 && n_cand >= 16 && A->ncols >= TILE_ROWS + 2 * TILE_W)) return SPRS_OK;
    unsigned long long *pat_d = nullptr; int *len_d = nullptr; uint8_t *flag_d = nullptr;
    auto drop = [&]() { for (void *q : {(void *)pat_d, (void *)len_d, (void *)flag_d}) if (q) (void)hipFree(q); pat_d = nullptr; len_d = nullptr; flag_d = nullptr; };
#define TILE_TRY(expr) do { hipError_t e__ = (expr); if (e__ != hipSuccess) { snprintf(c->err, sizeof(c->err), "%s:%d: %s -> %s", __FILE__, __LINE__, #expr, hipGetErrorString(e__)); drop(); return SPRS_ERR_HIP; } } while (0)
    TILE_TRY(hipMalloc((void **)&pat_d, sizeof(unsigned long long) * (size_t)n_cand));
    TILE_TRY(hipMalloc((void **)&len_d, sizeof(int) * (size_t)n_cand));
    hipLaunchKernelGGL(tile_mark_kernel, dim3((n_cand + BLOCK - 1) / BLOCK), dim3(BLOCK), 0, c->stream, n_cand, desc_dev, code_dev, pat_d, len_d);
    TILE_TRY(hipGetLastError());
    std::vector<unsigned long long> h_pat((size_t)n_cand);
    std::vector<int> h_len((size_t)n_cand);
    TILE_TRY(hipMemcpyAsync(h_pat.data(), pat_d, sizeof(unsigned long long) * (size_t)n_cand, hipMemcpyDeviceToHost, c->stream));
    TILE_TRY(hipMemcpyAsync(h_len.data(), len_d, sizeof(int) * (size_t)n_cand, hipMemcpyDeviceToHost, c->stream));
    TILE_TRY(hipStreamSynchronize(c->stream));
    std::map<std::pair<unsigned long long, int>, int> hist;
    for (int t = 0; t < n_cand; ++t) if (h_len[(size_t)t] > 0) ++hist[{h_pat[(size_t)t], h_len[(size_t)t]}];
    std::pair<unsigned long long, int> canon{0ull, 0};
    int best = 0;
    for (const auto &kv : hist) if (kv.second > best) { best = kv.second; canon = kv.first; }
    const int UL = canon.second;
    int FL = 0, FH = 0, WIN = 0;
    bool shape_ok = false;
    int64_t far_band = 0;
    if (best >= 8 && UL >= 1) {
        int32_t o[8];
        for (int t = 0; t < UL; ++t) {
            const int cd = (int)((canon.first >> (8 * t)) & 255u);
            o[t] = off_tab[cd];
            TP.off[t] = o[t];
            TP.val[t] = val_tab ? val_tab[cd] : 0.0;
        }
        double best_cost = 1e9;
        for (int w : {TILE_W, TILE_W_WIDE}) {
            if (w == TILE_W_WIDE && !wide_window_ok) continue;
            const int NEAR = w - 2;
            int fl = 0, fh = 0;
            while (fl < UL && o[fl] < -NEAR) ++fl;
            while (fh < UL - fl && o[UL - 1 - fh] > NEAR) ++fh;
            bool ok = UL - fl - fh >= 1 && tile_shape_built(UL, fl, fh, w);
            for (int t = fl; t < UL - fh; ++t) ok = ok && o[t] >= -NEAR && o[t] <= NEAR;
            const double cost = (double)(TILE_ROWS + 2 * w) / TILE_ROWS + fl + fh;
            if (ok && cost < best_cost) { shape_ok = true; best_cost = cost; FL = fl; FH = fh; WIN = w; }
        }
        for (int t = 0; t < FL; ++t) far_band = std::max<int64_t>(far_band, std::llabs((long long)o[t]));
        for (int t = UL - FH; t < UL; ++t) far_band = std::max<int64_t>(far_band, std::llabs((long long)o[t]));
    }
    if (!shape_ok || A->ncols < TILE_ROWS + 2 * WIN) { drop(); return SPRS_OK; }
    TILE_TRY(hipMalloc((void **)&flag_d, (size_t)nw));
    hipLaunchKernelGGL(tile_flag_kernel, dim3((nw + BLOCK - 1) / BLOCK), dim3(BLOCK), 0, c->stream, nw, desc_dev, code_dev, canon.first, UL, flag_d);
    TILE_TRY(hipGetLastError());
    std::vector<uint8_t> flag((size_t)nw);
    TILE_TRY(hipMemcpyAsync(flag.data(), flag_d, (size_t)nw, hipMemcpyDeviceToHost, c->stream));
    TILE_TRY(hipStreamSynchronize(c->stream));
    if (!val_tab)
        for (int j = 0; j < nw; ++j) if ((int64_t)wd[(size_t)j].pa + 2 * WAVE * UL + 2 > A->nnz) flag[(size_t)j] = 0;
    if (CP && c->spmv_chain != 0 && val_tab) {
        if (const int st = build_chain_plan(A, *CP, wd, flag, UL, TP.off, TP.val, make_left)) { drop(); return st; }
    }
    std::vector<int32_t> starts;
    std::vector<char> in_tile((size_t)nw, 0);
    for (int j = 0; j < nw;) {
        if (!flag[(size_t)j]) { ++j; continue; }
        int e = j + 1;
        while (e < nw && flag[(size_t)e] && wd[(size_t)e].ra == wd[(size_t)e - 1].ra + 2 * WAVE) ++e;
        int b = j;
        int64_t lo_need = WIN, hi_need = WIN;
        for (int t = 0; t < FL; ++t) lo_need = std::max<int64_t>(lo_need, -(int64_t)TP.off[t]);
        for (int t = UL - FH; t < UL; ++t) hi_need = std::max<int64_t>(hi_need, (int64_t)TP.off[t]);
        while (b < e && (int64_t)wd[(size_t)b].ra - lo_need < 0) ++b;
        for (; b + TILE_B <= e; b += TILE_B) {
            if ((int64_t)wd[(size_t)b].ra + TILE_ROWS + hi_need > A->ncols) break;
            starts.push_back(b);
            for (int q = 0; q < TILE_B; ++q) in_tile[(size_t)(b + q)] = 1;
        }
        j = e;
    }
    const int n_elig = (int)starts.size();
    if (n_elig < 8) { drop(); return SPRS_OK; }
    const bool periodic = far_band >= 8 * (int64_t)TILE_ROWS && far_band * 4 <= A->nrows && c->spmv_period != 0;
    std::vector<std::vector<int32_t>> sec(8);
    {
        std::vector<int32_t> by_phase((size_t)n_elig);
        for (int i = 0; i < n_elig; ++i) by_phase[(size_t)i] = i;
        if (periodic)
            std::stable_sort(by_phase.begin(), by_phase.end(), [&](int32_t a, int32_t b) {
                return (int64_t)wd[(size_t)starts[(size_t)a]].ra % far_band < (int64_t)wd[(size_t)starts[(size_t)b]].ra % far_band; });
        for (int i = 0; i < n_elig; ++i) sec[(size_t)(((int64_t)i * 8) / n_elig)].push_back(starts[(size_t)by_phase[(size_t)i]]);
        for (auto &v : sec) std::sort(v.begin(), v.end());
    }
    std::vector<int32_t> list, xstart(9, 0), left;
    for (int xq = 0; xq < 8; ++xq) {
        xstart[(size_t)xq] = (int32_t)(list.size() / 2);
        for (int32_t b0 : sec[(size_t)xq]) { list.push_back(b0); list.push_back(wd[(size_t)b0].ra); }
    }
    xstart[8] = (int32_t)(list.size() / 2);
    make_left(in_tile, left);
    TILE_TRY(hipMalloc((void **)&TP.list, sizeof(int32_t) * list.size()));
    TILE_TRY(hipMalloc((void **)&TP.xstart, sizeof(int32_t) * 9));
    TILE_TRY(hipMalloc((void **)&TP.left, sizeof(int32_t) * std::max<size_t>(left.size(), 1)));
    TILE_TRY(hipMemcpyAsync(TP.list, list.data(), sizeof(int32_t) * list.size(), hipMemcpyHostToDevice, c->stream));
    TILE_TRY(hipMemcpyAsync(TP.xstart, xstart.data(), sizeof(int32_t) * 9, hipMemcpyHostToDevice, c->stream));
    if (!left.empty()) TILE_TRY(hipMemcpyAsync(TP.left, left.data(), sizeof(int32_t) * left.size(), hipMemcpyHostToDevice, c->stream));
    TILE_TRY(hipStreamSynchronize(c->stream));
    TP.n_tile = n_elig; TP.n_left = (int)left.size();
    TP.ul = UL; TP.fl = FL; TP.fh = FH; TP.w = WIN;
    TP.h_list = list; TP.h_xstart = xstart;
    drop();
#undef TILE_TRY
    return SPRS_OK;
}

template <class T>
int build_dict_t(sprs_csr *A, const std::vector<int32_t> &blk, const std::vector<int32_t> &blk_pa) {
    sprs_ctx *c = A->ctx;
    constexpr bool VALS = has_val_dict<T>::value;
    CreateTrace tr;
    const bool want_vals = VALS && c->spmv_dict != 1;
    const int n = (int)A->nrows;
    uint32_t *off_h = nullptr; unsigned long long *val_h = nullptr; int *counts = nullptr;
    uint8_t *slot_codes = nullptr;
    auto cleanup = [&]() {
        if (off_h) (void)hipFree(off_h);
        if (val_h) (void)hipFree(val_h);
        if (counts) (void)hipFree(counts);
        if (slot_codes) (void)hipFree(slot_codes);
    };
#define DICT_TRY(expr) do { hipError_t e__ = (expr); if (e__ != hipSuccess) { snprintf(c->err, sizeof(c->err), "%s:%d: %s -> %s", __FILE__, __LINE__, #expr, hipGetErrorString(e__)); cleanup(); return SPRS_ERR_HIP; } } while (0)
    DICT_TRY(hipMalloc((void **)&off_h, sizeof(uint32_t) * HSLOTS));
    DICT_TRY(hipMalloc((void **)&val_h, sizeof(unsigned long long) * HSLOTS));
    DICT_TRY(hipMalloc((void **)&counts, sizeof(int) * 4));
    DICT_TRY(hipMalloc((void **)&slot_codes, 2 * HSLOTS));
    std::vector<uint32_t> h_off(HSLOTS, EMPTY32);
    std::vector<unsigned long long> h_val(HSLOTS, EMPTY64);
    DICT_TRY(hipMemcpyAsync(off_h, h_off.data(), sizeof(uint32_t) * HSLOTS, hipMemcpyHostToDevice, c->stream));
    DICT_TRY(hipMemcpyAsync(val_h, h_val.data(), sizeof(unsigned long long) * HSLOTS, hipMemcpyHostToDevice, c->stream));
    DICT_TRY(hipMemsetAsync(counts, 0, sizeof(int) * 4, c->stream));
    const int g = std::max(1, std::min(c->num_cu * 8, (n + BLOCK - 1) / BLOCK));
    const T *val = reinterpret_cast<const T *>(A->val);
    if (want_vals)
        hipLaunchKernelGGL((dict_collect_kernel<T, VALS>), dim3(g), dim3(BLOCK), 0, c->stream, n, A->row_ptr, A->col_idx, val, off_h, val_h, counts);
    else
        hipLaunchKernelGGL((dict_collect_kernel<T, false>), dim3(g), dim3(BLOCK), 0, c->stream, n, A->row_ptr, A->col_idx, val, off_h, val_h, counts);
    DICT_TRY(hipGetLastError());
    int h_counts[4] = {0, 0, 0, 0};
    DICT_TRY(hipMemcpyAsync(h_counts, counts, sizeof(int) * 4, hipMemcpyDeviceToHost, c->stream));
    DICT_TRY(hipMemcpyAsync(h_off.data(), off_h, sizeof(uint32_t) * HSLOTS, hipMemcpyDeviceToHost, c->stream));
    DICT_TRY(hipMemcpyAsync(h_val.data(), val_h, sizeof(unsigned long long) * HSLOTS, hipMemcpyDeviceToHost, c->stream));
    DICT_TRY(hipStreamSynchronize(c->stream));
    tr.lap("    dict collect");
    if (h_counts[0] > TAB || h_counts[0] == 0) { cleanup(); return SPRS_OK; }
    const bool use_vals = want_vals && h_counts[2] == 0 && h_counts[1] > 0 && h_counts[1] <= TAB;
    std::vector<std::pair<int32_t, int>> offs;
    std::vector<std::pair<uint64_t, int>> vals;
    for (int sl = 0; sl < HSLOTS; ++sl) {
        if (h_off[sl] != EMPTY32) offs.push_back({(int32_t)h_off[sl], sl});
        if (use_vals && h_val[sl] != EMPTY64) vals.push_back({(uint64_t)h_val[sl], sl});
    }
    std::sort(offs.begin(), offs.end());
    std::sort(vals.begin(), vals.end());
    if ((int)offs.size() != h_counts[0] || (use_vals && (int)vals.size() != h_counts[1])) { cleanup(); return SPRS_OK; }
    std::vector<uint8_t> codes(2 * HSLOTS, 0);
    std::vector<int32_t> off_tab(TAB, 0);
    std::vector<T> val_tab(TAB, szero<T>());
    for (size_t i = 0; i < offs.size(); ++i) { off_tab[i] = offs[i].first; codes[(size_t)offs[i].second] = (uint8_t)i; }
    if constexpr (VALS) {
        for (size_t i = 0; i < vals.size(); ++i) {
            T v;
            if constexpr (sizeof(T) == 8) { uint64_t k = vals[i].first; memcpy(&v, &k, 8); }
            else { uint32_t k = (uint32_t)vals[i].first; memcpy(&v, &k, 4); }
            val_tab[i] = v;
            codes[HSLOTS + (size_t)vals[i].second] = (uint8_t)i;
        }
    }
    DICT_TRY(hipMemcpyAsync(slot_codes, codes.data(), 2 * HSLOTS, hipMemcpyHostToDevice, c->stream));
    auto *D = new sprs_dict();
    A->dict = D;
    const size_t nb = ((size_t)A->nnz + 3) / 4 * 4 + 64;
    uint8_t *val_code = nullptr, *seen = nullptr;
    auto cleanup2 = [&]() { cleanup(); if (val_code) (void)hipFree(val_code); if (seen) (void)hipFree(seen); };
#define DICT_TRY2(expr) do { hipError_t e__ = (expr); if (e__ != hipSuccess) { snprintf(c->err, sizeof(c->err), "%s:%d: %s -> %s", __FILE__, __LINE__, #expr, hipGetErrorString(e__)); cleanup2(); free_dict(A); return SPRS_ERR_HIP; } } while (0)
    DICT_TRY2(hipMalloc((void **)&D->idx_code, nb));
    DICT_TRY2(hipMemsetAsync(D->idx_code, 0, nb, c->stream));
    DICT_TRY2(hipMalloc((void **)&D->off_tab, sizeof(int32_t) * TAB));
    DICT_TRY2(hipMemcpyAsync(D->off_tab, off_tab.data(), sizeof(int32_t) * TAB, hipMemcpyHostToDevice, c->stream));
    if (use_vals) {
        DICT_TRY2(hipMalloc((void **)&val_code, nb));
        DICT_TRY2(hipMemsetAsync(val_code, 0, nb, c->stream));
    }
    D->n_off = (int)offs.size(); D->n_val = use_vals ? (int)vals.size() : 0;
    for (const auto &o : offs) D->max_off = std::max<int64_t>(D->max_off, std::llabs((long long)o.first));
    int *bad = counts + 3;
    if (use_vals)
        hipLaunchKernelGGL((dict_encode_kernel<T, VALS>), dim3(g), dim3(BLOCK), 0, c->stream, n, A->row_ptr, A->col_idx, val, off_h,
                           slot_codes, val_h, slot_codes + HSLOTS, D->idx_code, val_code, bad);
    else
        hipLaunchKernelGGL((dict_encode_kernel<T, false>), dim3(g), dim3(BLOCK), 0, c->stream, n, A->row_ptr, A->col_idx, val, off_h,
                           slot_codes, val_h, slot_codes + HSLOTS, D->idx_code, val_code, bad);
    DICT_TRY2(hipGetLastError());
    DICT_TRY2(hipMemcpyAsync(h_counts, counts, sizeof(int) * 4, hipMemcpyDeviceToHost, c->stream));
    DICT_TRY2(hipStreamSynchronize(c->stream));
    tr.lap("    dict encode");
    if (h_counts[3] != 0) { cleanup2(); free_dict(A); return SPRS_OK; }
    {
        int64_t P = 0;
        for (const auto &o : offs) P = std::max<int64_t>(P, std::llabs((long long)o.first));
        const int64_t G = P / 8;
        if (c->spmv_period > 0 && G >= 16 * 128 && P * 4 <= A->nrows && A->n_rowblk >= 8 * NWAVE * 8) {
            const std::vector<int32_t> ord = xcd_period_order(A->n_rowblk, G, [&](int j) { return (int64_t)blk[(size_t)j]; });
            DICT_TRY2(hipMalloc((void **)&D->off_order, sizeof(int32_t) * ord.size()));
            DICT_TRY2(hipMemcpyAsync(D->off_order, ord.data(), sizeof(int32_t) * ord.size(), hipMemcpyHostToDevice, c->stream));
// ... 35 lines not shown
            CP_TRY(hipMemcpyAsync(&np, cp_cnt, sizeof(int), hipMemcpyDeviceToHost, c->stream));
            CP_TRY(hipStreamSynchronize(c->stream));
            if (np <= CP_DIAG) {
                hipLaunchKernelGGL((cpair_gather_kernel<T>), dim3(CP_SLOTS / BLOCK), dim3(BLOCK), 0, c->stream, cp_tab, D->idx_code, val, cp_oc, cp_val);
                CP_TRY(hipGetLastError());
                std::vector<int32_t> h_tab(CP_SLOTS);
                std::vector<uint8_t> h_oc(CP_SLOTS), h_code(CP_SLOTS, 0);
                std::vector<T> h_val(CP_SLOTS);
                CP_TRY(hipMemcpyAsync(h_tab.data(), cp_tab, sizeof(int32_t) * CP_SLOTS, hipMemcpyDeviceToHost, c->stream));
                CP_TRY(hipMemcpyAsync(h_oc.data(), cp_oc, CP_SLOTS, hipMemcpyDeviceToHost, c->stream));
                CP_TRY(hipMemcpyAsync(h_val.data(), cp_val, sizeof(T) * CP_SLOTS, hipMemcpyDeviceToHost, c->stream));
                CP_TRY(hipStreamSynchronize(c->stream));
                std::vector<int> slots;
                for (int sl = 0; sl < CP_SLOTS; ++sl) if (h_tab[(size_t)sl] >= 0) slots.push_back(sl);
                std::sort(slots.begin(), slots.end(), [&](int a, int b) {
                    const int32_t oa = off_tab[h_oc[(size_t)a]], ob = off_tab[h_oc[(size_t)b]];
                    if (oa != ob) return oa < ob;
                    return memcmp(&h_val[(size_t)a], &h_val[(size_t)b], sizeof(T)) < 0;
                });
                if ((int)slots.size() == np) {
                    std::vector<int32_t> pair_off(TAB, 0);
                    std::vector<T> pair_val(TAB, szero<T>());
                    for (size_t i = 0; i < slots.size(); ++i) {
                        h_code[(size_t)slots[i]] = (uint8_t)i;
                        pair_off[i] = off_tab[h_oc[(size_t)slots[i]]]; pair_val[i] = h_val[(size_t)slots[i]];
                    }
                    CP_TRY(hipMalloc((void **)&D->pair_code, nb));
                    CP_TRY(hipMemsetAsync(D->pair_code, 0, nb, c->stream));
                    CP_TRY(hipMalloc((void **)&D->pair_off, sizeof(int32_t) * TAB));
                    CP_TRY(hipMalloc(&D->pair_val, sizeof(T) * TAB));
                    CP_TRY(hipMalloc(&D->rowval, sizeof(T) * (size_t)std::max(n, 1)));
                    CP_TRY(hipMemcpyAsync(D->pair_off, pair_off.data(), sizeof(int32_t) * TAB, hipMemcpyHostToDevice, c->stream));
                    CP_TRY(hipMemcpyAsync(D->pair_val, pair_val.data(), sizeof(T) * TAB, hipMemcpyHostToDevice, c->stream));
                    CP_TRY(hipMemcpyAsync(cp_code, h_code.data(), CP_SLOTS, hipMemcpyHostToDevice, c->stream));
                    CP_TRY(hipMemsetAsync(bad, 0, sizeof(int), c->stream));
                    hipLaunchKernelGGL((cpair_encode_kernel<T>), dim3(g), dim3(BLOCK), 0, c->stream, n, A->row_ptr, D->idx_code, val, diag_code, cp_tab,
                                       cp_oc, cp_val, cp_code, D->pair_code, reinterpret_cast<T *>(D->rowval), bad);
                    CP_TRY(hipGetLastError());
                    int h_bad = 0;
                    CP_TRY(hipMemcpyAsync(&h_bad, bad, sizeof(int), hipMemcpyDeviceToHost, c->stream));
                    CP_TRY(hipStreamSynchronize(c->stream));
                    if (h_bad) {
                        for (void **q : {(void **)&D->pair_code, (void **)&D->pair_off, &D->pair_val, &D->rowval}) { (void)hipFree(*q); *q = nullptr; }
                    } else {
                        D->n_pair = np + (diag_code >= 0 ? 1 : 0);
                    }
                }
            }
            cp_free();
#undef CP_TRY
            tr.lap("    complex pair codes (row-value slot)");
        }
    }
    if (use_vals) {
        const int gk = (int)std::max<int64_t>(1, std::min<int64_t>(c->num_cu * 8, (A->nnz + BLOCK - 1) / BLOCK));
        DICT_TRY2(hipMalloc((void **)&seen, 65536 + 65536));
        DICT_TRY2(hipMemsetAsync(seen, 0, 65536, c->stream));
        hipLaunchKernelGGL(dict_pair_mark_kernel, dim3(gk), dim3(BLOCK), 0, c->stream, A->nnz, D->idx_code, val_code, seen);
        DICT_TRY2(hipGetLastError());
        std::vector<uint8_t> h_seen(65536), pair_of(65536, 0);
        DICT_TRY2(hipMemcpyAsync(h_seen.data(), seen, 65536, hipMemcpyDeviceToHost, c->stream));
        DICT_TRY2(hipStreamSynchronize(c->stream));
        std::vector<int32_t> pair_off(TAB, 0);
        std::vector<T> pair_val(TAB, szero<T>());
        int np = 0;
        for (int pr = 0; pr < 65536; ++pr) {
            if (!h_seen[pr]) continue;
            if (np < TAB) { pair_of[pr] = (uint8_t)np; pair_off[np] = off_tab[pr & 255]; pair_val[np] = val_tab[pr >> 8]; }
            ++np;
        }
        if (np >= 1 && np <= TAB) {
            DICT_TRY2(hipMalloc((void **)&D->pair_code, nb));
            DICT_TRY2(hipMemsetAsync(D->pair_code, 0, nb, c->stream));
            DICT_TRY2(hipMalloc((void **)&D->pair_off, sizeof(int32_t) * TAB));
            DICT_TRY2(hipMalloc(&D->pair_val, sizeof(T) * TAB));
            DICT_TRY2(hipMemcpyAsync(D->pair_off, pair_off.data(), sizeof(int32_t) * TAB, hipMemcpyHostToDevice, c->stream));
            DICT_TRY2(hipMemcpyAsync(D->pair_val, pair_val.data(), sizeof(T) * TAB, hipMemcpyHostToDevice, c->stream));
            DICT_TRY2(hipMemcpyAsync(seen + 65536, pair_of.data(), 65536, hipMemcpyHostToDevice, c->stream));
            hipLaunchKernelGGL(dict_pair_encode_kernel, dim3(gk), dim3(BLOCK), 0, c->stream, A->nnz, D->idx_code, val_code,
                               seen + 65536, D->pair_code);
            DICT_TRY2(hipGetLastError());
            DICT_TRY2(hipStreamSynchronize(c->stream));
            tr.lap("    pair mark + encode");
            D->n_pair = np;
            if constexpr (sizeof(T) == 8 && !is_complex<T>::value) {
                const int nb64 = A->n_rowblk, nw = (nb64 + 1) / 2;
                std::vector<BlkDescHost2> wd((size_t)nw);
                for (int j = 0; j < nw; ++j) {
                    const size_t b0 = (size_t)2 * j, b1 = (size_t)std::min(2 * j + 2, nb64);
                    const int32_t ra = blk[b0], rb = blk[b1];
                    wd[(size_t)j] = BlkDescHost2{ra, rb, blk_pa[b0], blk_pa[b1] - blk_pa[b0]};
                }
                DICT_TRY2(hipMalloc(&D->wide_desc, sizeof(BlkDescHost2) * (size_t)std::max(nw, 1)));
                DICT_TRY2(hipMemcpyAsync(D->wide_desc, wd.data(), sizeof(BlkDescHost2) * (size_t)nw, hipMemcpyHostToDevice, c->stream));
                if (c->spmv_uniform != 0 && nw > 0) {
                    const int gu = std::max(1, std::min(c->num_cu * 8, (nw + NWAVE - 1) / NWAVE));
                    hipLaunchKernelGGL(mark_uniform_kernel, dim3(gu), dim3(BLOCK), 0, c->stream, nw,
                                       reinterpret_cast<BlkDesc *>(D->wide_desc), A->row_ptr, D->pair_code, UNI2_MAXLEN,
                                       (const int32_t *)D->pair_off, c->spmv_triple != 0 ? 1 : 0, c->spmv_seam != 0 ? 1 : 0,
                                       (int)A->ncols);
                    DICT_TRY2(hipGetLastError());
                }
                DICT_TRY2(hipStreamSynchronize(c->stream));
                D->n_wide = nw;
                int64_t P = 0;
                for (const auto &o : offs) P = std::max<int64_t>(P, std::llabs((long long)o.first));
                const int64_t G = P / 8;
                std::vector<int32_t> ord;
                if (c->spmv_period != 0 && G >= 16 * 128 && P * 4 <= A->nrows && nw >= 8 * NWAVE * 8) {
                    ord = xcd_period_order(nw, G, [&](int j) { return (int64_t)wd[(size_t)j].ra; });
                    DICT_TRY2(hipMalloc((void **)&D->wide_order, sizeof(int32_t) * (size_t)nw));
                    DICT_TRY2(hipMemcpyAsync(D->wide_order, ord.data(), sizeof(int32_t) * (size_t)nw, hipMemcpyHostToDevice, c->stream));
                    DICT_TRY2(hipStreamSynchronize(c->stream));
                    D->period = P;
                }
                tr.lap("    wide descriptors, marks, period order");
                {
                    std::vector<int32_t> left_order;
                    if (const int st = build_tile_plan(A, D->tile_pair, reinterpret_cast<const BlkDesc *>(D->wide_desc), (const uint8_t *)D->pair_code, wd,
                                                       pair_off.data(), reinterpret_cast<const double *>(pair_val.data()), true, [&](std::vector<char> &in_tile, std::vector<int32_t> &left) {
                            for (int pos = 0; pos < nw; ++pos) {
                                const int j = ord.empty() ? pos : ord[(size_t)pos];
                                if (!in_tile[(size_t)j]) left.push_back(j);
                            }
                        }, &D->chain_pair)) { cleanup2(); free_dict(A); return st; }
                    tr.lap("    tile plan");
                }
            }
        }
    }
    if constexpr (sizeof(T) == 8 && !is_complex<T>::value) {
        if (tile_wanted(c, (size_t)A->nrows * sizeof(T)) && (D->pair_code == nullptr || c->spmv_dict == 1) && c->spmv_uniform != 0 && c->spmv_wide != 0 && A->n_rowblk >= 2 * TILE_B * 16) {
            const int nb64 = A->n_rowblk, nw = (nb64 + 1) / 2;
            std::vector<BlkDescHost2> owd((size_t)nw);
            for (int j = 0; j < nw; ++j) {
                const size_t b0 = (size_t)2 * j, b1 = (size_t)std::min(2 * j + 2, nb64);
                owd[(size_t)j] = BlkDescHost2{blk[b0], blk[b1], blk_pa[b0], blk_pa[b1] - blk_pa[b0]};
            }
            DICT_TRY2(hipMalloc(&D->owide_desc, sizeof(BlkDescHost2) * (size_t)nw));
            DICT_TRY2(hipMemcpyAsync(D->owide_desc, owd.data(), sizeof(BlkDescHost2) * (size_t)nw, hipMemcpyHostToDevice, c->stream));
            const int gu = std::max(1, std::min(c->num_cu * 8, (nw + NWAVE - 1) / NWAVE));
            hipLaunchKernelGGL(mark_uniform_kernel, dim3(gu), dim3(BLOCK), 0, c->stream, nw, reinterpret_cast<BlkDesc *>(D->owide_desc), A->row_ptr,
                               D->idx_code, UNI2_MAXLEN, (const int32_t *)D->off_tab, 0, c->spmv_seam != 0 ? 1 : 0, (int)A->ncols);
            DICT_TRY2(hipGetLastError());
            DICT_TRY2(hipStreamSynchronize(c->stream));
            D->n_owide = nw;
            if (const int st = build_tile_plan(A, D->tile_off, reinterpret_cast<const BlkDesc *>(D->owide_desc), (const uint8_t *)D->idx_code, owd,
                                               off_tab.data(), (const double *)nullptr, false, [&](std::vector<char> &in_tile, std::vector<int32_t> &left) {
                    for (int j = 0; j < nw; ++j) {
                        if (in_tile[(size_t)j]) continue;
                        left.push_back(2 * j);
                        if (2 * j + 1 < nb64) left.push_back(2 * j + 1);
                    }
                })) { cleanup2(); free_dict(A); return st; }
            if (D->tile_off.n_tile == 0) { (void)hipFree(D->owide_desc); D->owide_desc = nullptr; D->n_owide = 0; }
            tr.lap("    tile plan (offset stream)");
        }
    }
    cleanup2();
    return SPRS_OK;
#undef DICT_TRY
#undef DICT_TRY2
}

}

int tile_blocks() { return TILE_B; }
void free_dict(sprs_csr *A) {
    if (!A || !A->dict) return;
    sprs_dict *D = A->dict;
    for (void *q : {(void *)D->idx_code, (void *)D->pair_code, (void *)D->off_tab, (void *)D->pair_off, D->pair_val, D->wide_desc, D->off_desc, (void *)D->wide_order, (void *)D->off_order,
                    (void *)D->tile_pair.list, (void *)D->tile_pair.xstart, (void *)D->tile_pair.left,
                    (void *)D->tile_off.list, (void *)D->tile_off.xstart, (void *)D->tile_off.left, D->owide_desc,
                    (void *)D->chain_pair.tiles, (void *)D->chain_pair.segs, (void *)D->chain_pair.xstart, (void *)D->chain_pair.left, D->rowval})
        if (q) (void)hipFree(q);
    delete D;
    A->dict = nullptr;
}

int build_dict(sprs_csr *A, bool has_vector_blocks, const std::vector<int32_t> &blk, const std::vector<int32_t> &blk_pa) {
    if (A->ctx->spmv_dict == 0 || has_vector_blocks || A->nnz == 0 || A->nrows == 0) return SPRS_OK;
    switch (A->dtype) {
        case DT_D: return build_dict_t<double>(A, blk, blk_pa);
        case DT_Z: return build_dict_t<cplx>(A, blk, blk_pa);
        case DT_S: return build_dict_t<float>(A, blk, blk_pa);
        default: return build_dict_t<cplxf>(A, blk, blk_pa);
    }
}

template <class T>
int launch_dict(const sprs_csr *A, const SpmvRoute &r, const T *x, T *y, int dot_mode, const T *u, T *part0, T *part1,
                const int *status, bool conj_x, const Fin &fin) {
    sprs_ctx *c = A->ctx;
    const sprs_dict *D = A->dict;
    const bool pair = r.format == 2;
    const uint8_t *code = pair ? D->pair_code : D->idx_code;
    const int32_t *otab = pair ? D->pair_off : D->off_tab;
    with_dot(dot_mode, conj_x && is_complex<T>::value, [&](auto dm, auto cj) {
#define SPRS_DSPMV(PR) SPRS_LAUNCH_SPMV(c, (spmv_dict_kernel<T, decltype(dm)::value, decltype(cj)::value, PR>), r.grid, r.count, r.xcd_chunk, r.desc, \
                                        r.order, A->row_ptr, code, otab, reinterpret_cast<const T *>(D->pair_val), reinterpret_cast<const T *>(A->val), \
                                        x, y, u, part0, part1, status, fin, (const V2d *)nullptr, -1, reinterpret_cast<const T *>(D->rowval))
        if (pair) SPRS_DSPMV((has_pair_codes<T>::value)); else SPRS_DSPMV(false);
#undef SPRS_DSPMV
    });
    SPRS_HIP_TRY(c, hipGetLastError());
    return SPRS_OK;
}
template int launch_dict<double>(const sprs_csr *, const SpmvRoute &, const double *, double *, int, const double *, double *, double *, const int *, bool, const Fin &);
template int launch_dict<cplx>(const sprs_csr *, const SpmvRoute &, const cplx *, cplx *, int, const cplx *, cplx *, cplx *, const int *, bool, const Fin &);
template int launch_dict<float>(const sprs_csr *, const SpmvRoute &, const float *, float *, int, const float *, float *, float *, const int *, bool, const Fin &);
template int launch_dict<cplxf>(const sprs_csr *, const SpmvRoute &, const cplxf *, cplxf *, int, const cplxf *, cplxf *, cplxf *, const int *, bool, const Fin &);

int launch_dict_wide(const sprs_csr *A, const SpmvRoute &r, const double *x, double *y, int dot_mode, const double *u,
                     double *part0, double *part1, const int *status, const Fin &fin) {
    sprs_ctx *c = A->ctx;
    const sprs_dict *D = A->dict;
    int g2_last;
    const V2d *tail2 = dict_tail2(A, g2_last);
    with_dot(dot_mode, false, [&](auto dm, auto) {
        SPRS_LAUNCH_SPMV(c, (spmv_dict_kernel<double, decltype(dm)::value, false, false, true>), r.grid, r.count, r.xcd_chunk, r.desc, r.order,
                         A->row_ptr, D->idx_code, D->off_tab, reinterpret_cast<const double *>(D->pair_val), reinterpret_cast<const double *>(A->val),
                         x, y, u, part0, part1, status, fin, tail2, g2_last, (const double *)nullptr);
    });
    SPRS_HIP_TRY(c, hipGetLastError());
    return SPRS_OK;
}

int launch_pair2(const sprs_csr *A, const SpmvRoute &r, const double *x, double *y, int dot_mode, const double *u,
                 double *part0, double *part1, const int *status, const Fin &fin) {
    sprs_ctx *c = A->ctx;
    const sprs_dict *D = A->dict;
    with_dot(dot_mode, r.y_nt, [&](auto dm, auto ynt) {
        SPRS_LAUNCH_SPMV(c, (spmv_pair2_kernel<decltype(dm)::value, decltype(ynt)::value>), r.grid, r.count, r.xcd_chunk, r.desc, r.order,
                         A->row_ptr, D->pair_code, D->pair_off, reinterpret_cast<const double *>(D->pair_val), x, y, u, part0, part1, status,
                         (int)A->nrows, (int)A->ncols, fin);
    });
    SPRS_HIP_TRY(c, hipGetLastError());
    return SPRS_OK;
}

template <class T, bool SAUNDERS>
int launch_spmv_scaled(const sprs_csr *A, const MinresM3<T, false, SAUNDERS> &m3, const T *raw, T *y, T *partAlpha) {
    sprs_ctx *c = A->ctx;
    const sprs_dict *D = A->dict;
    const SpmvRoute r = spmv_route(A, SpmvPart::Whole, false);
    const bool pair = r.format == 2;
    const uint8_t *code = pair ? D->pair_code : D->idx_code;
    const int32_t *otab = pair ? D->pair_off : D->off_tab;
    const T *v = reinterpret_cast<const T *>(A->val);
    const T *pv = reinterpret_cast<const T *>(D->pair_val);
    typedef MinresM3<T, false, SAUNDERS> M3;
    constexpr bool CJ = SAUNDERS && is_complex<T>::value;
    if constexpr (sizeof(T) == 8 && !is_complex<T>::value) {
        int g2_last;
        const V2d *tail2 = dict_tail2(A, g2_last);
        SPRS_LAUNCH_SPMV(c, (spmv_dict_scaled_kernel<T, false, false, true, M3>), r.grid, r.count, r.xcd_chunk, r.desc, r.order, A->row_ptr, code,
                         otab, pv, v, raw, y, partAlpha, tail2, g2_last, (const T *)nullptr, m3);
    } else {
#define SPRS_M3L(PR) SPRS_LAUNCH_SPMV(c, (spmv_dict_scaled_kernel<T, CJ, PR, false, M3>), r.grid, r.count, r.xcd_chunk, r.desc, r.order, A->row_ptr, code, otab, pv, v, \
                                      raw, y, partAlpha, (const V2d *)nullptr, -1, reinterpret_cast<const T *>(D->rowval), m3)
        if (pair) SPRS_M3L((has_pair_codes<T>::value)); else SPRS_M3L(false);
#undef SPRS_M3L
    }
    SPRS_HIP_TRY(c, hipGetLastError());
    return SPRS_OK;
}
template int launch_spmv_scaled<double, false>(const sprs_csr *, const MinresM3<double, false, false> &, const double *, double *, double *);
template int launch_spmv_scaled<cplx, false>(const sprs_csr *, const MinresM3<cplx, false, false> &, const cplx *, cplx *, cplx *);
template int launch_spmv_scaled<cplx, true>(const sprs_csr *, const MinresM3<cplx, false, true> &, const cplx *, cplx *, cplx *);

}
```

sprsolve_amd/csrc/spmv_dict_dev.hpp:

```cpp
#pragma once
#include "device.hpp"

namespace sprs {

struct alignas(16) V2d { double a, b; };

namespace {

constexpr int TAB = 256;

constexpr int CPAD = 16;

template <class T> struct alignas(sizeof(T) >= 8 ? 16 : 8) PairEnt { int32_t off8; T val; };
template <class T>
__device__ __forceinline__ void stage_pair(PairEnt<T> *s_pair, int i, int32_t off8, T val) {
    s_pair[i].off8 = off8;
    s_pair[i].val = val;
}

template <class T, bool PAIR, int ITEMS>
struct BlkLoads {
    int ra, rb, pa, nn;
    int ulen;
    int s;
    T uu;
    T rv;
    uint32_t wc[2];
    int di[2];
    T vv[PAIR ? 1 : ITEMS];
};

struct NoScale { static constexpr bool ON = false; };
template <class T>
struct ScaleEw {
    static constexpr bool ON = true;
    Real<T> scale;
};

template <class T, int DOT, bool CONJX, bool PAIR, bool WV, class EW = NoScale>
__device__ __forceinline__ void dict_walk(int n_rowblk, int xcd_chunk, const BlkDesc *__restrict__ desc, const int32_t *__restrict__ order,
                                          const int32_t *__restrict__ row_ptr, const uint8_t *__restrict__ code,
                                          const T *__restrict__ val, const T *__restrict__ x, T *__restrict__ y, const T *__restrict__ u,
                                          const V2d *__restrict__ tail2, int g2_last,
                                          const PairEnt<T> *s_pair, const int32_t *s_off8, uint32_t (*s_c)[(nnz_cap<T>::value + 3 + CPAD + 3) / 4],
                                          T *s_v, int s_v_stride, T &d0, T &d1, const T *__restrict__ rowval = nullptr, const EW ew = EW{}) {
    static_assert(!EW::ON || DOT == 1, "the scaled operand is also the dot operand: u == x");
    constexpr int CAP = nnz_cap<T>::value;
    constexpr bool RV = PAIR && is_complex<T>::value;
    constexpr int ITEMS = CAP / WAVE;
    using Loads = BlkLoads<T, PAIR, ITEMS>;
    const int tid = threadIdx.x, lane = tid & (WAVE - 1);
    const int wv = __builtin_amdgcn_readfirstlane(tid >> 6);
    const uint8_t *cb = reinterpret_cast<const uint8_t *>(s_c[wv]);
    [[maybe_unused]] T *vs = s_v + (PAIR ? 0 : wv) * (size_t)s_v_stride;
    const char *xbytes = reinterpret_cast<const char *>(x);

    int b, bstep, bend;
    if (xcd_chunk) {
        const int chunk = (n_rowblk + 7) >> 3;
        const int xcd = blockIdx.x & 7;
        b = xcd * chunk + (blockIdx.x >> 3) * NWAVE + wv;
        bstep = (gridDim.x >> 3) * NWAVE;
        bend = min(n_rowblk, (xcd + 1) * chunk);
    } else {
        b = blockIdx.x * NWAVE + wv; bstep = gridDim.x * NWAVE; bend = n_rowblk;
    }
    if (b >= bend) b = bend;

    typedef int v4i __attribute__((ext_vector_type(4)));
    typedef const v4i __attribute__((address_space(1))) *gv4i_p;
    typedef const int32_t __attribute__((address_space(1))) *gi32_p;
    uintptr_t desc_a = reinterpret_cast<uintptr_t>(desc), order_a = reinterpret_cast<uintptr_t>(order);
    asm volatile("" : "+v"(desc_a));
    asm volatile("" : "+v"(order_a));
    const gv4i_p desc_v = reinterpret_cast<gv4i_p>(desc_a);
    const gi32_p order_v = reinterpret_cast<gi32_p>(order_a);
    auto load_desc = [&](int bi) -> BlkDesc { const v4i q = desc_v[bi]; return BlkDesc{q.x, q.y, q.z, q.w}; };
    auto block_index = [&](int bi) -> int { return order ? order_v[bi] : bi; };
    auto uniform = [&](const BlkDesc &d) -> BlkDesc {
        return BlkDesc{__builtin_amdgcn_readfirstlane(d.ra), __builtin_amdgcn_readfirstlane(d.rb),
                       __builtin_amdgcn_readfirstlane(d.pa), __builtin_amdgcn_readfirstlane(d.nn)};
    };
    auto issue = [&](const BlkDesc &d, Loads &L) {
        L.ra = d.ra; L.rb = d.rb & 0x3fffffff; L.pa = d.pa;
        const bool uni = ((uint32_t)d.rb & UNI2) != 0;
        L.ulen = uni ? d.nn : 0;
        L.nn = uni ? (L.rb - L.ra) * d.nn : d.nn;
        const int r = L.ra + lane;
        const int rcl = r < L.rb ? r : L.rb - 1;
        if (uni) L.s = L.pa + (rcl - L.ra) * L.ulen;
        else L.s = *reinterpret_cast<const int32_t *>(reinterpret_cast<const char *>(row_ptr) + (uint32_t)rcl * 4u);
        if (DOT != 0) L.uu = *reinterpret_cast<const T *>(reinterpret_cast<const char *>(u) + (uint32_t)rcl * (uint32_t)sizeof(T));
        if constexpr (RV) L.rv = *reinterpret_cast<const T *>(reinterpret_cast<const char *>(rowval) + (uint32_t)rcl * (uint32_t)sizeof(T));
        const int shift = L.pa & 3;
        const int nd = max((shift + (uni ? L.ulen : L.nn) + 3) >> 2, 1);
#pragma unroll
        for (int i = 0; i < 2; ++i) {
            L.di[i] = min(lane + i * WAVE, nd - 1);
            L.wc[i] = *reinterpret_cast<const uint32_t *>(reinterpret_cast<const char *>(code) + (uint32_t)(L.pa - shift + 4 * L.di[i]));
        }
        if constexpr (!PAIR) {
            [[maybe_unused]] const int last = max(L.nn - 1, 0);
            if constexpr (WV) {
                const int vsh = L.pa & 1, g0 = (L.pa - vsh) >> 1, lastq = max(L.nn + vsh - 1, 0) >> 1;
                const V2d *val2 = reinterpret_cast<const V2d *>(val);
#pragma unroll
                for (int i = 0; i < ITEMS / 2; ++i) {
                    const int G = g0 + min(lane + i * WAVE, lastq);
                    const V2d q = *(G == g2_last ? tail2 : val2 + G);
                    L.vv[2 * i] = q.a; L.vv[2 * i + 1] = q.b;
                }
            } else {
#pragma unroll
                for (int i = 0; i < ITEMS; ++i) L.vv[i] = val[L.pa + min(lane + i * WAVE, last)];
            }
        }
    };
    auto stage = [&](const Loads &L) {
        const int shift = L.pa & 3;
        if (L.nn > 0) {
#pragma unroll
            for (int i = 0; i < 2; ++i) s_c[wv][L.di[i]] = L.wc[i];
            if constexpr (CAP / 4 + 1 > 2 * WAVE) {
                if (L.ulen == 0 && ((shift + L.nn + 3) >> 2) > 2 * WAVE && lane == 0)
                    s_c[wv][2 * WAVE] = reinterpret_cast<const uint32_t *>(code + (L.pa - shift))[2 * WAVE];
            }
            if constexpr (!PAIR) {
                if constexpr (WV) {
                    const int tot = L.nn + (L.pa & 1);
#pragma unroll
                    for (int i = 0; i < ITEMS / 2; ++i) {
                        const int k = 2 * (lane + i * WAVE);
                        if (k < tot) *reinterpret_cast<V2d *>(vs + k) = V2d{L.vv[2 * i], L.vv[2 * i + 1]};
                    }
                } else {
#pragma unroll
                for (int i = 0; i < ITEMS; ++i) {
                    const int k = lane + i * WAVE;
                    if (k < L.nn) vs[k] = L.vv[i];
                }
                }
            }
        }
    };

    int c_ra = 0, c_rb = 0, c_s = 0, c_len = 0, c_shift = 0;
    [[maybe_unused]] int c_vsh = 0;
    bool c_uni = false;
    T c_uu = szero<T>();
    [[maybe_unused]] T c_rv = szero<T>();
    auto adopt = [&](const Loads &L) {
        if constexpr (RV) c_rv = L.rv;
        const int r = L.ra + lane;
        c_ra = L.ra; c_rb = L.rb; c_shift = L.pa & 3; c_uni = L.ulen > 0;
        if constexpr (WV) c_vsh = L.pa & 1;
        c_s = L.s - L.pa;
        int e = __shfl_down(L.s, 1, WAVE);
        if (r == L.rb - 1) e = L.pa + L.nn;
        c_len = r < L.rb ? e - L.s : 0;
        if (DOT != 0) c_uu = L.uu;
    };
    BlkDesc dn{0, 1, 0, 0};
    int o2 = 0;
    if (b < bend) {
        Loads first;
        issue(uniform(load_desc(__builtin_amdgcn_readfirstlane(block_index(b)))), first);
        if (b + bstep < bend) dn = uniform(load_desc(__builtin_amdgcn_readfirstlane(block_index(b + bstep))));
        if (b + 2 * bstep < bend) o2 = __builtin_amdgcn_readfirstlane(block_index(b + 2 * bstep));
        stage(first);
        adopt(first);
    }
    for (; b < bend; b += bstep) {
        const bool more = b + bstep < bend;
        Loads nxt;
        BlkDesc dn2{0, 1, 0, 0};
        int o3 = 0;
        if (b + 2 * bstep < bend) dn2 = load_desc(o2);
        if (b + 3 * bstep < bend) o3 = block_index(b + 3 * bstep);
        if (more) issue(dn, nxt);
        wave_lds_fence();
        const int r = c_ra + lane;
        const uint32_t r8 = (uint32_t)r * (uint32_t)sizeof(T);
        const int s = c_s, len = c_len;
        T acc = szero<T>();
        for (int j0 = 0; __builtin_amdgcn_ballot_w64(j0 < len) != 0; j0 += 8) {
            const int kb = min(s + j0, CAP);
            const uint8_t *cp = cb + c_shift + (c_uni ? j0 : kb);
            T xg[8], av[8];
#pragma unroll
            for (int t = 0; t < 8; ++t) { xg[t] = szero<T>(); av[t] = szero<T>(); }
            const uint64_t m4 = __builtin_amdgcn_ballot_w64(j0 + 4 < len), m5 = __builtin_amdgcn_ballot_w64(j0 + 5 < len),
                           m6 = __builtin_amdgcn_ballot_w64(j0 + 6 < len), m7 = __builtin_amdgcn_ballot_w64(j0 + 7 < len);
#pragma unroll
            for (int t = 0; t < 8; ++t) {
                if (t == 4 && m4 == 0) break;
                if (t == 5 && m5 == 0) break;
                if (t == 6 && m6 == 0) break;
                if (t == 7 && m7 == 0) break;
                const bool valid = j0 + t < len;
                const int cd = cp[t];
                int off8;
                if constexpr (PAIR) {
                    const PairEnt<T> e = s_pair[cd]; off8 = e.off8; av[t] = e.val;
                    if constexpr (RV) { if (cd == 255) av[t] = c_rv; }
                }
                else { off8 = s_off8[cd]; av[t] = vs[(WV ? c_vsh : 0) + kb + t]; }
                const uint32_t vo = valid ? r8 + (uint32_t)off8 : 0u;
                xg[t] = *reinterpret_cast<const T *>(xbytes + vo);
            }
            __builtin_amdgcn_sched_barrier(0);
#pragma unroll
            for (int t = 0; t < 8; ++t)
                if (j0 + t < len) {
                    T xv = xg[t];
                    if constexpr (EW::ON) xv = smulr(xv, ew.scale);
                    acc = sadd(acc, smul(CONJX ? sconj(xv) : xv, av[t]));
                }
        }
        if (r < c_rb) {
            *reinterpret_cast<T *>(reinterpret_cast<char *>(y) + r8) = acc;
            if constexpr (EW::ON) c_uu = smulr(c_uu, ew.scale);
            if (DOT == 1) d0 = sadd(d0, smul(sconj(c_uu), acc));
            if (DOT == 2) { d0 = sadd(d0, smul(sconj(acc), acc)); d1 = sadd(d1, smul(sconj(acc), c_uu)); }
        }
        wave_lds_fence();
        if (more) { stage(nxt); adopt(nxt); }
        dn = uniform(dn2); o2 = __builtin_amdgcn_readfirstlane(o3);
    }
}

struct alignas(16) D2 { double lo, hi; };
typedef unsigned int u4v __attribute__((ext_vector_type(4)));
constexpr int CAP2 = 2 * nnz_cap<double>::value;
constexpr int CW2 = (CAP2 + 3 + CPAD + 15) / 16 * 4;

constexpr int UNI_OFF_MAXLEN = 32;
constexpr int UNI2_MAXLEN = 8;

__device__ __forceinline__ double comb_k3(double r, double v, double na) { return r + v * na; }
__device__ __forceinline__ double comb_k1(double v, double p, double r, double a, double beta) { double t = v * a + p * beta; t = t + r * 1.0; return t; }
struct XPlain {
    static constexpr bool FUSED = false;
    const char *xb;
    __device__ __forceinline__ D2 ld2(int64_t soff, uint32_t voff) const { return *reinterpret_cast<const D2 *>(xb + soff + voff); }
    __device__ __forceinline__ double ld1(uint32_t voff) const { return *reinterpret_cast<const double *>(xb + voff); }
    __device__ __forceinline__ double lds(int64_t soff) const { return *reinterpret_cast<const double *>(xb + soff); }
};
template <int NV>
struct XFused {
    static constexpr bool FUSED = true;
    const char *b0, *b1, *b2;
    double c0, c1;
    __device__ __forceinline__ double one(double a, double b, double c) const { return NV == 2 ? comb_k3(a, b, c0) : comb_k1(a, b, c, c0, c1); }
    __device__ __forceinline__ D2 ld2(int64_t soff, uint32_t voff) const {
        const D2 a = *reinterpret_cast<const D2 *>(b0 + soff + voff), b = *reinterpret_cast<const D2 *>(b1 + soff + voff);
        D2 c{0.0, 0.0};
        if (NV == 3) c = *reinterpret_cast<const D2 *>(b2 + soff + voff);
        return D2{one(a.lo, b.lo, c.lo), one(a.hi, b.hi, c.hi)};
    }
    __device__ __forceinline__ double ld1(uint32_t voff) const {
        const double a = *reinterpret_cast<const double *>(b0 + voff), b = *reinterpret_cast<const double *>(b1 + voff);
        const double c = NV == 3 ? *reinterpret_cast<const double *>(b2 + voff) : 0.0;
        return one(a, b, c);
    }
    __device__ __forceinline__ double lds(int64_t soff) const {
        const double a = *reinterpret_cast<const double *>(b0 + soff), b = *reinterpret_cast<const double *>(b1 + soff);
        const double c = NV == 3 ? *reinterpret_cast<const double *>(b2 + soff) : 0.0;
        return one(a, b, c);
    }
};

__device__ __forceinline__ double wave_shift_up(double prev_for_lane0, double v) {
    const long long o = __double_as_longlong(prev_for_lane0), q = __double_as_longlong(v);
    const uint32_t lo = (uint32_t)__builtin_amdgcn_update_dpp((int)(uint32_t)o, (int)(uint32_t)q, 0x138, 0xf, 0xf, false);
    const uint32_t hi = (uint32_t)__builtin_amdgcn_update_dpp((int)(uint32_t)(o >> 32), (int)(uint32_t)(q >> 32), 0x138, 0xf, 0xf, false);
    return __longlong_as_double((long long)(((uint64_t)hi << 32) | lo));
}
__device__ __forceinline__ double wave_shift_down(double next_for_last_lane, double v) {
    const long long o = __double_as_longlong(next_for_last_lane), q = __double_as_longlong(v);
    const uint32_t lo = (uint32_t)__builtin_amdgcn_update_dpp((int)(uint32_t)o, (int)(uint32_t)q, 0x130, 0xf, 0xf, false);
    const uint32_t hi = (uint32_t)__builtin_amdgcn_update_dpp((int)(uint32_t)(o >> 32), (int)(uint32_t)(q >> 32), 0x130, 0xf, 0xf, false);
    return __longlong_as_double((long long)(((uint64_t)hi << 32) | lo));
}
template <int UL, int SC, class XS, class AfterLoads>
__device__ __forceinline__ void full_uniform_block(const PairEnt<double> *s_pair, uint64_t pat, int ulen, bool seam, int seam1, int seam2, const XS &xs,
                                                   uint32_t r8, uint32_t ra8, int lane, AfterLoads &&after_loads,
                                                   double &acc0, double &acc1) {
    using T = double;
    T pl[8], ph[8], av[8];
    int off8c = 0;
#pragma unroll
    for (int t = 0; t < 8; ++t) { pl[t] = 0.0; ph[t] = 0.0; av[t] = 0.0; }
#pragma unroll
    for (int t = 0; t < 8; ++t) {
        if (UL == 0 ? t >= ulen : t >= UL) break;
        const PairEnt<T> e = s_pair[(int)((pat >> (8 * t)) & 255u)];
        const int off8 = __builtin_amdgcn_readfirstlane(e.off8);
        const uint32_t vlo = __builtin_amdgcn_readfirstlane((int)(uint32_t)__double_as_longlong(e.val));
        const uint32_t vhi = __builtin_amdgcn_readfirstlane((int)(uint32_t)(__double_as_longlong(e.val) >> 32));
        av[t] = __longlong_as_double((long long)(((uint64_t)vhi << 32) | vlo));
        if (SC > 0 && (t == SC - 1 || t == SC + 1)) continue;
        const D2 px = xs.ld2((int64_t)off8, r8);
        pl[t] = px.lo; ph[t] = px.hi;
        if (SC > 0 && t == SC) off8c = off8;
    }
    T e_lo = 0.0, e_hi = 0.0;
    if (SC > 0) {
        const int64_t xe = (int64_t)off8c + ra8;
        e_lo = xs.lds(xe - 8); e_hi = xs.lds(xe + 2 * WAVE * 8);
    }
    after_loads();
    __builtin_amdgcn_sched_barrier(0);
    if (SC > 0) {
        constexpr int C = SC > 0 ? SC : 1;
        const T left = wave_shift_up(e_lo, ph[C]), right = wave_shift_down(e_hi, pl[C]);
        pl[C - 1] = left; ph[C - 1] = pl[C];
        pl[C + 1] = ph[C]; ph[C + 1] = right;
    }
    if (!seam) {
#pragma unroll
        for (int t = 0; t < 8; ++t) {
            if (UL == 0 ? t >= ulen : t >= UL) break;
            acc0 = acc0 + pl[t] * av[t];
            acc1 = acc1 + ph[t] * av[t];
        }
    } else {
        const int k = seam1 & 127, maskA = (seam1 >> 7) & 255, maskB = seam2 & 255;
        const T valA = s_pair[(seam2 >> 8) & 255].val, valB = s_pair[(seam2 >> 16) & 255].val;
        const bool ovA = ((seam2 >> 24) & 1) != 0, ovB = ((seam2 >> 25) & 1) != 0;
        const bool a0 = 2 * lane == k, a1 = 2 * lane + 1 == k, b0 = 2 * lane == k + 1, b1 = 2 * lane + 1 == k + 1;
        const int pm0 = a0 ? maskA : (b0 ? maskB : 255), pm1 = a1 ? maskA : (b1 ? maskB : 255);
        const bool o0 = (a0 && ovA) || (b0 && ovB), o1 = (a1 && ovA) || (b1 && ovB);
        const T v0 = a0 ? valA : valB, v1 = a1 ? valA : valB;
#pragma unroll
        for (int t = 0; t < 8; ++t) {
            if (UL == 0 ? t >= ulen : t >= UL) break;
            const T n0 = acc0 + pl[t] * (o0 ? v0 : av[t]), n1 = acc1 + ph[t] * (o1 ? v1 : av[t]);
            acc0 = ((pm0 >> t) & 1) ? n0 : acc0;
            acc1 = ((pm1 >> t) & 1) ? n1 : acc1;
        }
    }
}
template <class XS, class AfterLoads>
__device__ __forceinline__ void full_uniform_dispatch(const PairEnt<double> *s_pair, uint64_t pat, int ulen, int sc, bool seam, int seam1, int seam2, const XS &xs,
                                                      uint32_t r8, uint32_t ra8, int lane, AfterLoads &&after_loads,
                                                      double &acc0, double &acc1) {
    if (ulen == 7 && sc == 3) full_uniform_block<7, 3>(s_pair, pat, ulen, seam, seam1, seam2, xs, r8, ra8, lane, after_loads, acc0, acc1);
    else if (ulen == 5 && sc == 2) full_uniform_block<5, 2>(s_pair, pat, ulen, seam, seam1, seam2, xs, r8, ra8, lane, after_loads, acc0, acc1);
    else if (ulen == 3 && sc == 1) full_uniform_block<3, 1>(s_pair, pat, ulen, seam, seam1, seam2, xs, r8, ra8, lane, after_loads, acc0, acc1);
    else full_uniform_block<0, 0>(s_pair, pat, ulen, seam, seam1, seam2, xs, r8, ra8, lane, after_loads, acc0, acc1);
}


struct Blk2Loads {
    int ra, rb, pa, nn;
    bool uni; int ulen;
    int tri;
    bool is_seam; int seam1, seam2;
    int a, b;
    double u0, u1;
    double o0, o1;
    u4v wc;
    int di;
};

template <int DOT, bool YNT, class XS = XPlain>
__device__ __forceinline__ void pair2_walk(int n_wide, int xcd_chunk, const BlkDesc *__restrict__ desc,
                                           const int32_t *__restrict__ order, const int32_t *__restrict__ row_ptr,
                                           const uint8_t *__restrict__ code, const XS xs,
                                           double *__restrict__ y, const double *__restrict__ u, int nrows, int ncols,
                                           const PairEnt<double> *s_pair, uint32_t (*s_c)[CW2], double &d0, double &d1,
                                           double *__restrict__ own = nullptr) {
    using T = double;
// ... 70 lines not shown
    auto stage = [&](const Blk2Loads &L) {
        const int shift = L.pa & 3;
        c_uni = L.uni;
        if constexpr (XS::FUSED) { c_o0 = L.o0; c_o1 = L.o1; }
        if (L.uni) {
            const uint64_t lo = (uint64_t)__builtin_amdgcn_readfirstlane(L.wc.x) | ((uint64_t)__builtin_amdgcn_readfirstlane(L.wc.y) << 32);
            const uint64_t hi = (uint64_t)__builtin_amdgcn_readfirstlane(L.wc.z);
            c_pat = shift ? (lo >> (8 * shift)) | (hi << (64 - 8 * shift)) : lo;
            const int r0 = L.ra + 2 * lane;
            c_ra = L.ra; c_rb = L.rb; c_shift = shift; c_tri = L.tri; c_seam = L.is_seam; c_seam1 = L.seam1; c_seam2 = L.seam2;
            c_s0 = 0; c_s1 = 0;
            c_len0 = r0 < L.rb ? L.ulen : 0;
            c_len1 = r0 + 1 < L.rb ? L.ulen : 0;
            if (DOT != 0) { c_u0 = L.u0; c_u1 = L.u1; }
            return;
        }
        if (L.nn > 0) {
            *reinterpret_cast<u4v *>(&s_c[wv][4 * L.di]) = L.wc;
            if (shift + L.nn > CAP2 && lane == 0)
                s_c[wv][CAP2 / 4] = *reinterpret_cast<const uint32_t *>(code + (L.pa - shift) + CAP2);
        }
        const int r0 = L.ra + 2 * lane;
        int c = __shfl_down(L.a, 1, WAVE);
        if (r0 + 2 >= L.rb) c = L.pa + L.nn;
        c_ra = L.ra; c_rb = L.rb; c_shift = shift;
        c_s0 = L.a - L.pa; c_s1 = L.b - L.pa;
        c_len0 = r0 < L.rb ? L.b - L.a : 0;
        c_len1 = r0 + 1 < L.rb ? c - L.b : 0;
        if (DOT != 0) { c_u0 = L.u0; c_u1 = L.u1; }
    };

    BlkDesc dn{0, 1, 0, 0};
    int o2 = 0;
    if (b < bend) {
        Blk2Loads first;
        issue(uniform(load_desc(__builtin_amdgcn_readfirstlane(block_index(b)))), first);
        if (b + bstep < bend) dn = uniform(load_desc(__builtin_amdgcn_readfirstlane(block_index(b + bstep))));
        if (b + 2 * bstep < bend) o2 = __builtin_amdgcn_readfirstlane(block_index(b + 2 * bstep));
        stage(first);
    }
    for (; b < bend; b += bstep) {
        const bool more = b + bstep < bend;
        Blk2Loads nxt;
        BlkDesc dn2{0, 1, 0, 0};
        int o3 = 0;
        if (b + 3 * bstep < bend) o3 = block_index(b + 3 * bstep);
        if (more) issue(dn, nxt);
        const bool want_dn2 = b + 2 * bstep < bend;
        auto after_gathers = [&]() { if (want_dn2) dn2 = load_desc(o2); };
        wave_lds_fence();
        const int r0 = c_ra + 2 * lane;
        const uint32_t r8 = (uint32_t)r0 * 8u;
        const int len0 = c_len0, len1 = c_len1, lenm = max(len0, len1);
        T acc0 = 0.0, acc1 = 0.0;
        if (c_uni) {
            const int ulen = __builtin_amdgcn_readfirstlane(lenm);
            T pl[8], ph[8], av[8];
            uint32_t hi_bits = 0;
#pragma unroll
            for (int t = 0; t < 8; ++t) { pl[t] = 0.0; ph[t] = 0.0; av[t] = 0.0; }
            if (c_rb - c_ra == 2 * WAVE) {
                full_uniform_dispatch(s_pair, c_pat, ulen, c_tri, c_seam, c_seam1, c_seam2, xs, r8, (uint32_t)c_ra * 8u, lane, after_gathers, acc0, acc1);
            } else {
#pragma unroll
            for (int t = 0; t < 8; ++t) {
                if (t >= ulen) break;
                const PairEnt<T> e = s_pair[(int)((c_pat >> (8 * t)) & 255u)];
                av[t] = e.val;
                const uint32_t vo0 = len0 > 0 ? r8 + (uint32_t)e.off8 : 0u;
                const uint32_t vp = min(vo0, xlast_pair);
                hi_bits |= (vo0 != vp ? 1u : 0u) << t;
                const D2 px = xs.ld2(0, vp);
                pl[t] = px.lo; ph[t] = px.hi;
            }
            after_gathers();
            __builtin_amdgcn_sched_barrier(0);
#pragma unroll
            for (int t = 0; t < 8; ++t) {
                if (t >= ulen) break;
                if (len0 > 0) acc0 = acc0 + (((hi_bits >> t) & 1u) ? ph[t] : pl[t]) * av[t];
                if (len1 > 0) acc1 = acc1 + ph[t] * av[t];
            }
            }
        } else {
        if (__builtin_amdgcn_ballot_w64(0 < lenm) == 0) after_gathers();
        for (int j0 = 0; __builtin_amdgcn_ballot_w64(j0 < lenm) != 0; j0 += 8) {
            const uint8_t *cp0 = cb + c_shift + min(c_s0 + j0, CAP2);
            const uint8_t *cp1 = cb + c_shift + min(c_s1 + j0, CAP2);
            T pl[8], ph[8];
            T xg1[8];
            uint32_t same_bits = 0, hi_bits = 0;
#pragma unroll
            for (int t = 0; t < 8; ++t) { pl[t] = 0.0; ph[t] = 0.0; xg1[t] = 0.0; }
            const uint64_t m4 = __builtin_amdgcn_ballot_w64(j0 + 4 < lenm), m5 = __builtin_amdgcn_ballot_w64(j0 + 5 < lenm),
                           m6 = __builtin_amdgcn_ballot_w64(j0 + 6 < lenm), m7 = __builtin_amdgcn_ballot_w64(j0 + 7 < lenm);
#pragma unroll
            for (int t = 0; t < 8; ++t) {
                if (t == 4 && m4 == 0) break;
                if (t == 5 && m5 == 0) break;
                if (t == 6 && m6 == 0) break;
                if (t == 7 && m7 == 0) break;
                const bool v0 = j0 + t < len0, v1 = j0 + t < len1;
                const int off0 = s_pair[cp0[t]].off8, off1 = s_pair[cp1[t]].off8;
                const bool same = v0 && v1 && off0 == off1;
                const uint32_t vo0 = v0 ? r8 + (uint32_t)off0 : 0u;
                const uint32_t vp = min(vo0, xlast_pair);
                same_bits |= (same ? 1u : 0u) << t;
                hi_bits |= (vo0 != vp ? 1u : 0u) << t;
                const D2 px = xs.ld2(0, vp);
                pl[t] = px.lo; ph[t] = px.hi;
                const bool need1 = v1 && !same;
                if (__builtin_amdgcn_ballot_w64(need1) != 0)
                    xg1[t] = xs.ld1(need1 ? r8 + 8u + (uint32_t)off1 : 0u);
            }
            if (j0 == 0) after_gathers();
            __builtin_amdgcn_sched_barrier(0);
            asm volatile("" ::: "memory");
#pragma unroll
            for (int t = 0; t < 8; ++t) {
                if (j0 + t < len0) acc0 = acc0 + (((hi_bits >> t) & 1u) ? ph[t] : pl[t]) * s_pair[cp0[t]].val;
                if (j0 + t < len1) acc1 = acc1 + (((same_bits >> t) & 1u) ? ph[t] : xg1[t]) * s_pair[cp1[t]].val;
            }
        }
        }
        if (r0 + 1 < c_rb) {
            if constexpr (YNT) {
                const D2 yy{acc0, acc1};
                u4v q;
                __builtin_memcpy(&q, &yy, 16);
                __builtin_nontemporal_store(q, reinterpret_cast<u4v *>(reinterpret_cast<char *>(y) + r8));
            } else {
                *reinterpret_cast<D2 *>(reinterpret_cast<char *>(y) + r8) = D2{acc0, acc1};
            }
            if (DOT == 1) { d0 = d0 + c_u0 * acc0; d0 = d0 + c_u1 * acc1; }
            if (DOT == 2) { d0 = d0 + acc0 * acc0; d1 = d1 + acc0 * c_u0; d0 = d0 + acc1 * acc1; d1 = d1 + acc1 * c_u1; }
            if constexpr (XS::FUSED) { if (own != nullptr) *reinterpret_cast<D2 *>(reinterpret_cast<char *>(own) + r8) = D2{c_o0, c_o1}; }
        } else if (r0 < c_rb) {
            if constexpr (XS::FUSED) { if (own != nullptr) *reinterpret_cast<T *>(reinterpret_cast<char *>(own) + r8) = c_o0; }
            *reinterpret_cast<T *>(reinterpret_cast<char *>(y) + r8) = acc0;
            if (DOT == 1) d0 = d0 + c_u0 * acc0;
            if (DOT == 2) { d0 = d0 + acc0 * acc0; d1 = d1 + acc0 * c_u0; }
        }
        wave_lds_fence();
        if (more) stage(nxt);
        dn = uniform(dn2); o2 = __builtin_amdgcn_readfirstlane(o3);
    }
}

constexpr int TILE_ROWS = 4096, TILE_W = 512, TILE_W_WIDE = 1536, TILE_B = TILE_ROWS / (2 * WAVE);
struct TilePat { int32_t off[8]; double val[8]; };

#define SPRS_TILE_SHAPES(X) X(7, 1, 1) X(5, 1, 1) X(5, 0, 0) X(3, 0, 0) X(3, 1, 1) X(7, 0, 0)
#define SPRS_TILE_SHAPES_WIDE(X) X(7, 1, 1) X(5, 1, 1) X(5, 0, 0) X(7, 0, 0)
constexpr int CH_B = 16;
#define SPRS_CHAIN_SHAPES(X) X(7, true) X(7, false) X(5, true) X(5, false) X(3, true)
}

inline const V2d *dict_tail2(const sprs_csr *A, int &g2_last) {
    g2_last = (int)((A->nnz - 1) >> 1);
    return reinterpret_cast<const V2d *>(reinterpret_cast<const char *>(A->tail) + 16) + (g2_last - 2 * (int)((A->nnz - 1) >> 2));
}

int chain_rows();

}
```

Measured before the change: 838.2.

## Add chained tile SpMV kernel for f64 offset-code format with fused BiCGStab updates

Adds a chained-tile SpMV path for the f64 offset-stream dictionary format, which previously only had the independent TileOff kernel. The new kernel keeps a sliding three-window LDS copy of x across consecutive tiles in a chain, so neighbouring stencil planes are reused instead of re-read. It can also fuse the BiCGStab K1/K3 vector updates into the window staging. The dict walk for leftover blocks gains a fused-operand variant. Routing selects it when offset tiles and a chain plan exist, at the cost of extra plan construction, LDS pressure and code complexity.

```diff
diff --git a/sprsolve_amd/csrc/bicg_fuse.hpp b/sprsolve_amd/csrc/bicg_fuse.hpp
--- a/sprsolve_amd/csrc/bicg_fuse.hpp
+++ b/sprsolve_amd/csrc/bicg_fuse.hpp
@@ -116,6 +116,10 @@
                      double *t, double *partTT, double *partTR, const int *status);
 int launch_chain_k2f(const sprs_csr *A, const SpmvRoute &rt, const BicgK1<double, double, false> &pro, const double *v_old, const double *p, const double *r,
                      double *p_out, double *v_out, const double *r0, double *partB, const int *status);
+int launch_chain_off_k4f(const sprs_csr *A, const SpmvRoute &rt, const BicgK3<double, double, false> &pro, const double *r, const double *v, double *s_out,
+                         double *t, double *partTT, double *partTR, const int *status);
+int launch_chain_off_k2f(const sprs_csr *A, const SpmvRoute &rt, const BicgK1<double, double, false> &pro, const double *v_old, const double *p, const double *r,
+                         double *p_out, double *v_out, const double *r0, double *partB, const int *status);
 
 template <class T, bool PC, bool SV = false>
 struct BicgK5 {
diff --git a/sprsolve_amd/csrc/capi.hip b/sprsolve_amd/csrc/capi.hip
--- a/sprsolve_amd/csrc/capi.hip
+++ b/sprsolve_amd/csrc/capi.hip
@@ -621,7 +621,8 @@
     *n_tiles = 0; *n_tile_blocks = 0; *n_other_blocks = 0;
     const bool split = A->dist && A->dist->order_int;
     const SpmvRoute r = spmv_route(A, split ? SpmvPart::Interior : SpmvPart::Whole, false);
-    if (r.kernel != SpmvKernel::TilePair && r.kernel != SpmvKernel::TileOff) return SPRS_OK;
+    const bool chain_off = r.kernel == SpmvKernel::Chain && r.format == 1 && r.tile;
+    if (r.kernel != SpmvKernel::TilePair && r.kernel != SpmvKernel::TileOff && !chain_off) return SPRS_OK;
     const sprs_tile_plan &TP = *r.tile;
     *n_tiles = TP.n_tile; *n_tile_blocks = (int64_t)TP.n_tile * sprs::tile_blocks();
     if (split) *n_other_blocks = (A->n_rowblk + 1) / 2 - *n_tile_blocks;
@@ -633,7 +634,8 @@
     *n_tiles = 0; *n_segments = 0; *n_chains = 0; *n_other_blocks = 0;
     const SpmvRoute r = spmv_route(A, SpmvPart::Whole, false);
     if (r.kernel != SpmvKernel::Chain) return SPRS_OK;
-    *n_tiles = r.chain->n_tile; *n_segments = r.chain->n_seg; *n_chains = r.chain->n_chain; *n_other_blocks = r.chain->n_left;
+    *n_tiles = r.chain->n_tile; *n_segments = r.chain->n_seg; *n_chains = r.chain->n_chain;
+    *n_other_blocks = r.format == 1 ? (r.chain->n_left + 1) / 2 : r.chain->n_left;
     return SPRS_OK;
 }
 int sprs_csr_spmv_route(const sprs_csr *A, int part, int conj_x, int *kernel, int *format, int *grid, int64_t *n_blocks,
diff --git a/sprsolve_amd/csrc/internal.hpp b/sprsolve_amd/csrc/internal.hpp
--- a/sprsolve_amd/csrc/internal.hpp
+++ b/sprsolve_amd/csrc/internal.hpp
@@ -182,6 +182,7 @@
     int64_t max_off = -1;
     sprs_tile_plan tile_pair, tile_off;
     sprs_chain_plan chain_pair;
+    sprs_chain_plan chain_off;
     void *owide_desc = nullptr;
     int n_owide = 0;
     void *off_desc = nullptr;
@@ -276,6 +277,8 @@
                     double *part0, double *part1, const int *status, const Fin &fin);
 int launch_chain_pair(const sprs_csr *A, const SpmvRoute &r, const double *x, double *y, int dot_mode, const double *u,
                       double *part0, double *part1, const int *status, const Fin &fin);
+int launch_chain_off(const sprs_csr *A, const SpmvRoute &r, const double *x, double *y, int dot_mode, const double *u,
+                     double *part0, double *part1, const int *status, const Fin &fin);
 
 template <class T>
 int launch_spmm(const sprs_csr *A, const T *x, T *y, int ld, int k, int dot_mode, const T *u, T *part, const int *running);
diff --git a/sprsolve_amd/csrc/spmv.hip b/sprsolve_amd/csrc/spmv.hip
--- a/sprsolve_amd/csrc/spmv.hip
+++ b/sprsolve_amd/csrc/spmv.hip
@@ -543,7 +543,10 @@
         else if (c->spmv_dict != -1 || !dtype_is_complex(A->dtype)) r.format = 1;
     }
     const bool pair = r.format == 2;
-    const sprs_chain_plan *chain = pair && !P && c->spmv_chain != 0 && tiles && uni && D->chain_pair.n_tile > 0 ? &D->chain_pair : nullptr;
+    const bool off_tiles = r.format == 1 && f64 && wideload && uni && tiles && D->owide_desc && !conj_x;
+    const sprs_chain_plan *chain = P || c->spmv_chain == 0 || !tiles || !uni ? nullptr
+                                 : pair ? (D->chain_pair.n_tile > 0 ? &D->chain_pair : nullptr)
+                                 : (off_tiles && D->tile_off.n_tile > 0 && D->chain_off.n_tile > 0 ? &D->chain_off : nullptr);
     const sprs_tile_plan *tile = !tiles ? nullptr
                                : pair ? (D->tile_pair.n_tile > 0 ? &D->tile_pair : nullptr)
                                : (r.format == 1 && wideload && uni && D->tile_off.n_tile > 0 ? &D->tile_off : nullptr);
@@ -590,6 +593,7 @@
     if (f64 && !pair && wideload) {
         r.kernel = SpmvKernel::DictWide;
         if (tp && D->owide_desc && uni && !conj_x) { r.kernel = SpmvKernel::TileOff; r.tile = tp; }
+        if (chain && whole && tp) r.kernel = SpmvKernel::Chain, r.chain = chain;
     }
     return r;
 }
@@ -626,7 +630,8 @@
             case SpmvKernel::Pair2: return launch_pair2(A, r, x, y, dot_mode, u, part0, part1, status, fin);
             case SpmvKernel::TilePair: return launch_tile_pair(A, r, x, y, dot_mode, u, part0, part1, status, fin);
             case SpmvKernel::TileOff: return launch_tile_off(A, r, x, y, dot_mode, u, part0, part1, status, fin);
-            case SpmvKernel::Chain: return launch_chain_pair(A, r, x, y, dot_mode, u, part0, part1, status, fin);
+            case SpmvKernel::Chain: return r.format == 1 ? launch_chain_off(A, r, x, y, dot_mode, u, part0, part1, status, fin)
+                                                         : launch_chain_pair(A, r, x, y, dot_mode, u, part0, part1, status, fin);
             default: break;
         }
     }
diff --git a/sprsolve_amd/csrc/spmv_chain.hip b/sprsolve_amd/csrc/spmv_chain.hip
--- a/sprsolve_amd/csrc/spmv_chain.hip
+++ b/sprsolve_amd/csrc/spmv_chain.hip
@@ -266,6 +266,7 @@
 
 int launch_chain_k4f(const sprs_csr *A, const SpmvRoute &rt, const BicgK3<double, double, false> &pro, const double *r, const double *v, double *s_out,
                      double *t, double *partTT, double *partTR, const int *status) {
+    if (rt.format == 1) return launch_chain_off_k4f(A, rt, pro, r, v, s_out, t, partTT, partTR, status);
     sprs_ctx *c = A->ctx;
     const sprs_dict *D = A->dict;
     const sprs_chain_plan &CP = *rt.chain;
@@ -288,6 +289,7 @@
 
 int launch_chain_k2f(const sprs_csr *A, const SpmvRoute &rt, const BicgK1<double, double, false> &pro, const double *v_old, const double *p, const double *r,
                      double *p_out, double *v_out, const double *r0, double *partB, const int *status) {
+    if (rt.format == 1) return launch_chain_off_k2f(A, rt, pro, v_old, p, r, p_out, v_out, r0, partB, status);
     sprs_ctx *c = A->ctx;
     const sprs_dict *D = A->dict;
     const sprs_chain_plan &CP = *rt.chain;
diff --git a/sprsolve_amd/csrc/spmv_chain_off.hip b/sprsolve_amd/csrc/spmv_chain_off.hip
--- /dev/null
+++ b/sprsolve_amd/csrc/spmv_chain_off.hip
@@ -0,0 +1,326 @@
+#include "spmv_dict_dev.hpp"
+#include "bicg_fuse.hpp"
+
+namespace sprs {
+namespace {
+
+constexpr int CHO_ROWS = CHO_B * 2 * WAVE;
+constexpr int CHO_W = TILE_W;
+constexpr int CHO_WL = CHO_ROWS + 2 * CHO_W;
+
+struct NoProOff { __device__ __forceinline__ bool prologue() { return true; } };
+template <int FUSE, class PRO, int DOT, bool UX, int UL, bool TRI>
+__global__ __launch_bounds__(BLOCK) void spmv_chain_off_kernel(const int4 *__restrict__ tiles, const int2 *__restrict__ segs, const int32_t *__restrict__ xstart,
+                                                               const BlkDesc *__restrict__ desc, const TilePat pat,
+                                                               int n_left, const int32_t *__restrict__ left_order, const BlkDesc *__restrict__ desc64,
+                                                               const int32_t *__restrict__ row_ptr, const uint8_t *__restrict__ code,
+                                                               const int32_t *__restrict__ off_tab, const double *__restrict__ val,
+                                                               const double *__restrict__ x, double *__restrict__ y, const double *__restrict__ u,
+                                                               double *__restrict__ part0, double *__restrict__ part1,
+                                                               const int *__restrict__ status, int ncols, const Fin fin,
+                                                               const V2d *__restrict__ tail2, int g2_last,
+                                                               PRO pro, const double *__restrict__ in1, const double *__restrict__ in2,
+                                                               double *__restrict__ own) {
+    using T = double;
+    constexpr int NVEC = FUSE == 0 ? 1 : FUSE;
+    static_assert(FUSE == 0 || (FUSE == 2 && DOT == 2 && UX) || (FUSE == 3 && DOT == 1 && !UX), "fused flavours: K3 into K4, K1 into K2");
+    constexpr int W = CHO_W, WL = CHO_WL;
+    constexpr int NW = WL / 2 / BLOCK;
+    constexpr int NQ = CHO_B / NWAVE;
+    constexpr int NN = UL - 2;
+    constexpr int TC = NN / 2;
+    constexpr int VROW = 2 * WAVE * UL;
+    constexpr int NV = (VROW / 2 + 1 + WAVE - 1) / WAVE;
+    constexpr int CAPD = nnz_cap<T>::value;
+    constexpr int CWD = (CAPD + 3 + CPAD + 3) / 4;
+    constexpr int VS = (VROW + 2 + 15) / 16 * 16 > CAPD + 16 ? (VROW + 2 + 15) / 16 * 16 : CAPD + 16;
+    static_assert(WL % (2 * BLOCK) == 0 && CHO_B % NWAVE == 0 && NN >= 1 && UL <= 8 && (!TRI || (NN & 1)), "chain shape");
+    static_assert(sizeof(T) * WL >= sizeof(uint32_t) * NWAVE * CWD + sizeof(int32_t) * TAB, "the left walk's code slices and offset table live in the first window");
+    __shared__ __attribute__((aligned(16))) T win[3][WL];
+    __shared__ __attribute__((aligned(16))) T vsl[NWAVE][VS];
+    __shared__ T red[NWAVE];
+    const int run_state = status != nullptr ? *status : (int)ST_RUNNING;
+    const int tid = threadIdx.x, lane = tid & (WAVE - 1);
+    const int wv = __builtin_amdgcn_readfirstlane(tid >> 6);
+    for (int i = lane; i < VS; i += WAVE) vsl[wv][i] = 0.0;
+    if (run_state != ST_RUNNING) { fin_idle(fin, DOT == 2); return; }
+    [[maybe_unused]] T c0 = 0.0, c1 = 0.0;
+    if constexpr (FUSE != 0) {
+        if (!pro.prologue()) return;
+        if constexpr (FUSE == 2) c0 = pro.na; else { c0 = pro.a; c1 = pro.beta; }
+    }
+    T d0 = 0.0, d1 = 0.0;
+
+    const int Pf = pat.off[UL - 1];
+    const int xhi = (ncols - 2) & ~1;
+    const int xcd = blockIdx.x & 7;
+    const int sstep = gridDim.x >> 3;
+    const int send = xstart[xcd + 1];
+    T *vs = vsl[wv];
+    constexpr int PF = FUSE == 3 ? 1 : 2;
+    struct WinRegs { u4v a[NW]; u4v b[NVEC >= 2 ? NW : 1]; u4v c[NVEC == 3 ? NW : 1]; };
+    WinRegs R0;
+    [[maybe_unused]] WinRegs R1;
+    auto issue = [&](int tw, WinRegs &R) {
+#pragma unroll
+        for (int i = 0; i < NW; ++i) {
+            int g = tw - W + 2 * (tid + i * BLOCK);
+            g = g < 0 ? 0 : (g > xhi ? xhi : g);
+            R.a[i] = *reinterpret_cast<const u4v *>(x + g);
+            if constexpr (NVEC >= 2) R.b[i] = *reinterpret_cast<const u4v *>(in1 + g);
+            if constexpr (NVEC == 3) R.c[i] = *reinterpret_cast<const u4v *>(in2 + g);
+        }
+    };
+    auto stage = [&](int slot, const WinRegs &R) {
+#pragma unroll
+        for (int i = 0; i < NW; ++i) {
+            if constexpr (FUSE == 0) {
+                *reinterpret_cast<u4v *>(&win[slot][2 * (tid + i * BLOCK)]) = R.a[i];
+            } else {
+                D2 a, b, cc{0.0, 0.0};
+                __builtin_memcpy(&a, &R.a[i], 16); __builtin_memcpy(&b, &R.b[i], 16);
+                if constexpr (NVEC == 3) __builtin_memcpy(&cc, &R.c[i], 16);
+                const D2 o = FUSE == 2 ? D2{comb_k3(a.lo, b.lo, c0), comb_k3(a.hi, b.hi, c0)}
+                                       : D2{comb_k1(a.lo, b.lo, cc.lo, c0, c1), comb_k1(a.hi, b.hi, cc.hi, c0, c1)};
+                *reinterpret_cast<D2 *>(&win[slot][2 * (tid + i * BLOCK)]) = o;
+            }
+        }
+    };
+    u4v vreg[NV];
+    auto load_vals = [&](int vb) {
+        const u4v *v2 = reinterpret_cast<const u4v *>(val) + (vb >> 1);
+#pragma unroll
+        for (int i = 0; i < NV; ++i) vreg[i] = __builtin_nontemporal_load(v2 + min(lane + i * WAVE, VROW / 2));
+    };
+    for (int s = xstart[xcd] + (blockIdx.x >> 3); s < send; s += sstep) {
+        const int2 sg = segs[s];
+        const int t0 = __builtin_amdgcn_readfirstlane(sg.x), L = __builtin_amdgcn_readfirstlane(sg.y);
+        int4 ent = tiles[t0];
+        uint32_t rbw[NQ]; int nnw[NQ], vbw[NQ];
+        auto load_words = [&](int b0, int ts) {
+#pragma unroll
+            for (int q = 0; q < NQ; ++q) {
+                const BlkDesc d = desc[b0 + q * NWAVE + wv];
+                rbw[q] = (uint32_t)d.rb; nnw[q] = d.nn; vbw[q] = row_ptr[ts + ((q * NWAVE + wv) << 7)];
+            }
+        };
+        load_words(__builtin_amdgcn_readfirstlane(ent.x), __builtin_amdgcn_readfirstlane(ent.y));
+        load_vals(__builtin_amdgcn_readfirstlane(vbw[0]));
+        __syncthreads();
+        int ts_prev = __builtin_amdgcn_readfirstlane(ent.y) - Pf;
+        int sp = 0, sc = 1, sn = 2;
+        issue(ts_prev, R0); stage(sp, R0);
+        issue(__builtin_amdgcn_readfirstlane(ent.y), R0); stage(sc, R0);
+        issue(__builtin_amdgcn_readfirstlane(ent.z), R0);
+        if constexpr (PF == 2) { if (L > 1) issue(tiles[t0 + 1].z, R1); }
+        auto body = [&](int k, WinRegs &RS) {
+            const int ts = __builtin_amdgcn_readfirstlane(ent.y), ts_next = __builtin_amdgcn_readfirstlane(ent.z);
+            uint32_t rbc[NQ]; int nnc[NQ], vbc[NQ];
+#pragma unroll
+            for (int q = 0; q < NQ; ++q) { rbc[q] = rbw[q]; nnc[q] = nnw[q]; vbc[q] = __builtin_amdgcn_readfirstlane(vbw[q]); }
+            stage(sn, RS);
+            __syncthreads();
+            if (k + PF < L) issue(tiles[t0 + k + PF].z, RS);
+            const bool more = k + 1 < L;
+            if (more) {
+                ent = tiles[t0 + k + 1];
+                load_words(__builtin_amdgcn_readfirstlane(ent.x), __builtin_amdgcn_readfirstlane(ent.y));
+            }
+            const int dlo = ts - Pf - ts_prev, dhi = ts + Pf - ts_next;
+            const T *wp = &win[sp][W + dlo], *wc = &win[sc][W], *wn = &win[sn][W + dhi];
+            D2 uu[NQ];
+            if (DOT != 0 && !UX) {
+#pragma unroll
+                for (int q = 0; q < NQ; ++q) {
+                    const u4v w4 = __builtin_nontemporal_load(reinterpret_cast<const u4v *>(u + (ts + ((q * NWAVE + wv) << 7) + 2 * lane)));
+                    __builtin_memcpy(&uu[q], &w4, 16);
+                }
+            }
+            T opl[UL], oph[UL], ux0 = 0.0, ux1 = 0.0;
+            auto read_ops = [&](int q) {
+                const int l = ((q * NWAVE + wv) << 7) + 2 * lane;
+                const D2 f0 = *reinterpret_cast<const D2 *>(wp + l), f1 = *reinterpret_cast<const D2 *>(wn + l);
+                opl[0] = f0.lo; oph[0] = f0.hi; opl[UL - 1] = f1.lo; oph[UL - 1] = f1.hi;
+                if constexpr (TRI) {
+#pragma unroll
+                    for (int t = 0; t < NN; ++t) {
+                        if (t == TC - 1 || t == TC + 1) continue;
+                        const D2 v2 = *reinterpret_cast<const D2 *>(wc + l + pat.off[1 + t]);
+                        opl[1 + t] = v2.lo; oph[1 + t] = v2.hi;
+                    }
+                    if constexpr (NN >= 3) {
+                        const int oc = pat.off[1 + TC];
+                        opl[TC] = wc[l + oc - 1]; oph[TC] = opl[1 + TC];
+                        opl[2 + TC] = oph[1 + TC]; oph[2 + TC] = wc[l + oc + 2];
+                    }
+                } else {
+#pragma unroll
+                    for (int t = 0; t < NN; ++t) { opl[1 + t] = wc[l + pat.off[1 + t]]; oph[1 + t] = wc[l + pat.off[1 + t] + 1]; }
+                }
+                if ((DOT != 0 && UX) || FUSE != 0) { const D2 c2 = *reinterpret_cast<const D2 *>(wc + l); ux0 = c2.lo; ux1 = c2.hi; }
+            };
+            read_ops(0);
+#pragma unroll
+            for (int q = 0; q < NQ; ++q) {
+#pragma unroll
+                for (int i = 0; i < NV; ++i) *reinterpret_cast<u4v *>(&vs[2 * min(lane + i * WAVE, VROW / 2)]) = vreg[i];
+                if (q + 1 < NQ) load_vals(vbc[q + 1 < NQ ? q + 1 : q]);
+                else if (more) load_vals(__builtin_amdgcn_readfirstlane(vbw[0]));
+                wave_lds_fence();
+                const uint32_t rbq = (uint32_t)__builtin_amdgcn_readfirstlane((int)rbc[q]);
+                const bool seam = (rbq & SEAM2) != 0;
+                const int shift = vbc[q] & 1;
+                T pl[UL], ph[UL];
+#pragma unroll
+                for (int t = 0; t < UL; ++t) { pl[t] = opl[t]; ph[t] = oph[t]; }
+                const T u0 = (DOT != 0 && !UX) ? uu[q].lo : ux0, u1 = (DOT != 0 && !UX) ? uu[q].hi : ux1;
+                [[maybe_unused]] const D2 mine{ux0, ux1};
+                if (q + 1 < NQ) read_ops(q + 1);
+                T acc0 = 0.0, acc1 = 0.0;
+                if (!seam) {
+                    const T *v0 = vs + shift + 2 * lane * UL;
+#pragma unroll
+                    for (int t = 0; t < UL; ++t) {
+                        acc0 = acc0 + pl[t] * v0[t];
+                        acc1 = acc1 + ph[t] * v0[UL + t];
+                    }
+                } else {
+                    const int seam1 = __builtin_amdgcn_readfirstlane(nnc[q]) >> 16, seam2 = (int)(rbq & 0x3ffffffu);
+                    const int kk = seam1 & 127, full = (1 << UL) - 1, maskA = (seam1 >> 7) & full, maskB = seam2 & full;
+                    const int cA = UL - __builtin_popcount(maskA), cB = UL - __builtin_popcount(maskB);
+                    const int i0 = 2 * lane, i1 = i0 + 1;
+                    int p0 = shift + i0 * UL - (i0 > kk ? cA : 0) - (i0 > kk + 1 ? cB : 0);
+                    int p1 = shift + i1 * UL - (i1 > kk ? cA : 0) - (i1 > kk + 1 ? cB : 0);
+                    const int pm0 = i0 == kk ? maskA : (i0 == kk + 1 ? maskB : full), pm1 = i1 == kk ? maskA : (i1 == kk + 1 ? maskB : full);
+#pragma unroll
+                    for (int t = 0; t < UL; ++t) {
+                        const T n0 = acc0 + pl[t] * vs[p0], n1 = acc1 + ph[t] * vs[p1];
+                        const bool h0 = ((pm0 >> t) & 1) != 0, h1 = ((pm1 >> t) & 1) != 0;
+                        acc0 = h0 ? n0 : acc0; p0 += h0 ? 1 : 0;
+                        acc1 = h1 ? n1 : acc1; p1 += h1 ? 1 : 0;
+                    }
+                }
+                const D2 yy{acc0, acc1};
+                u4v qv;
+                __builtin_memcpy(&qv, &yy, 16);
+                __builtin_nontemporal_store(qv, reinterpret_cast<u4v *>(y + (ts + ((q * NWAVE + wv) << 7) + 2 * lane)));
+                if constexpr (FUSE == 3) {
+                    u4v ov;
+                    __builtin_memcpy(&ov, &mine, 16);
+                    __builtin_nontemporal_store(ov, reinterpret_cast<u4v *>(own + (ts + ((q * NWAVE + wv) << 7) + 2 * lane)));
+                }
+                if (DOT == 1) { d0 = d0 + u0 * acc0; d0 = d0 + u1 * acc1; }
+                if (DOT == 2) { d0 = d0 + acc0 * acc0; d1 = d1 + acc0 * u0; d0 = d0 + acc1 * acc1; d1 = d1 + acc1 * u1; }
+                wave_lds_fence();
+            }
+            __syncthreads();
+            ts_prev = ts;
+            const int o = sp; sp = sc; sc = sn; sn = o;
+        };
+        if constexpr (PF == 2) {
+            for (int k = 0; k < L; k += 2) { body(k, R0); if (k + 1 < L) body(k + 1, R1); }
+        } else {
+            for (int k = 0; k < L; ++k) body(k, R0);
+        }
+    }
+    if (n_left > 0) {
+        __syncthreads();
+        uint32_t (*s_c)[CWD] = reinterpret_cast<uint32_t (*)[CWD]>(&win[0][0]);
+        int32_t *s_off8 = reinterpret_cast<int32_t *>(&s_c[NWAVE][0]);
+        s_off8[tid] = off_tab[tid] * (int32_t)sizeof(T);
+        for (int i = lane; i < CWD; i += WAVE) s_c[wv][i] = 0;
+        __syncthreads();
+        if constexpr (FUSE == 0)
+            dict_walk<T, DOT, false, false, true>(n_left, 0, desc64, left_order, row_ptr, code, val, x, y, u, tail2, g2_last,
+                                                 (const PairEnt<T> *)nullptr, s_off8, s_c, &vsl[0][0], VS, d0, d1);
+        else
+            dict_walk<T, DOT, false, false, true, NoScale, XFused<NVEC>>(n_left, 0, desc64, left_order, row_ptr, code, val, x, y, UX ? nullptr : u, tail2, g2_last,
+                                                 (const PairEnt<T> *)nullptr, s_off8, s_c, &vsl[0][0], VS, d0, d1, nullptr, NoScale{},
+                                                 XFused<NVEC>{reinterpret_cast<const char *>(x), reinterpret_cast<const char *>(in1), reinterpret_cast<const char *>(in2), c0, c1}, own);
+    }
+    if (DOT >= 1) {
+        d0 = block_sum(d0, red);
+        if (tid == 0) st_partial(fin, part0 + blockIdx.x, d0);
+    }
+    if (DOT == 2) {
+        d1 = block_sum(d1, red);
+        if (tid == 0) st_partial(fin, part1 + blockIdx.x, d1);
+    }
+    if (DOT >= 1 && fin.counter) finalize_last_block<T, T>(fin, DOT == 2, red, red);
+}
+
+struct ChainOffArgs {
+    const int4 *tiles; const int2 *segs; const int32_t *xstart; const BlkDesc *owd; TilePat tp; int n_left; const int32_t *left;
+    const BlkDesc *desc64; const int32_t *row_ptr; const uint8_t *code; const int32_t *off_tab; const double *val; int ncols;
+    const V2d *tail2; int g2_last; int ul; bool tri; int grid;
+};
+ChainOffArgs chain_off_args(const sprs_csr *A, const SpmvRoute &r) {
+    const sprs_dict *D = A->dict;
+    const sprs_chain_plan &CP = *r.chain;
+    ChainOffArgs a;
+    a.tiles = reinterpret_cast<const int4 *>(CP.tiles); a.segs = reinterpret_cast<const int2 *>(CP.segs); a.xstart = CP.xstart;
+    a.owd = reinterpret_cast<const BlkDesc *>(D->owide_desc);
+    for (int t = 0; t < 8; ++t) { a.tp.off[t] = CP.off[t]; a.tp.val[t] = 0.0; }
+    a.n_left = CP.n_left; a.left = CP.left;
+    a.desc64 = r.desc;
+    a.row_ptr = A->row_ptr; a.code = D->idx_code; a.off_tab = D->off_tab; a.val = reinterpret_cast<const double *>(A->val);
+    a.ncols = (int)A->ncols;
+    a.tail2 = dict_tail2(A, a.g2_last);
+    a.ul = CP.ul; a.tri = CP.tri != 0; a.grid = r.grid;
+    return a;
+}
+#define SPRS_CO_HEAD(a) a.tiles, a.segs, a.xstart, a.owd, a.tp, a.n_left, a.left, a.desc64, a.row_ptr, a.code, a.off_tab, a.val
+
+}
+
+int launch_chain_off(const sprs_csr *A, const SpmvRoute &r, const double *x, double *y, int dot_mode, const double *u,
+                     double *part0, double *part1, const int *status, const Fin &fin) {
+    sprs_ctx *c = A->ctx;
+    const ChainOffArgs a = chain_off_args(A, r);
+    const bool ux = dot_mode != 0 && u == x;
+#define SPRS_COSPMV(DM, UXV, U, TR) SPRS_LAUNCH_SPMV(c, (spmv_chain_off_kernel<0, NoProOff, DM, UXV, U, TR>), a.grid, SPRS_CO_HEAD(a), x, y, u, part0, part1, status, \
+                                                     a.ncols, fin, a.tail2, a.g2_last, NoProOff{}, nullptr, nullptr, nullptr)
+#define SPRS_COSHAPE(U, TR)                                                                                          \
+    if (a.ul == U && a.tri == TR) {                                                                                  \
+        if (dot_mode == 0) SPRS_COSPMV(0, false, U, TR);                                                             \
+        else if (dot_mode == 1) { if (ux) SPRS_COSPMV(1, true, U, TR); else SPRS_COSPMV(1, false, U, TR); }          \
+        else if (ux) SPRS_COSPMV(2, true, U, TR); else SPRS_COSPMV(2, false, U, TR);                                 \
+    }
+    SPRS_CHAIN_SHAPES(SPRS_COSHAPE)
+#undef SPRS_COSHAPE
+#undef SPRS_COSPMV
+    SPRS_HIP_TRY(c, hipGetLastError());
+    return SPRS_OK;
+}
+
+int launch_chain_off_k4f(const sprs_csr *A, const SpmvRoute &rt, const BicgK3<double, double, false> &pro, const double *r, const double *v, double *s_out,
+                         double *t, double *partTT, double *partTR, const int *status) {
+    sprs_ctx *c = A->ctx;
+    const ChainOffArgs a = chain_off_args(A, rt);
+    typedef BicgK3<double, double, false> K3;
+#define SPRS_CO4F(U, TR)                                                                                                \
+    if (a.ul == U && a.tri == TR)                                                                                       \
+        SPRS_LAUNCH_SPMV(c, (spmv_chain_off_kernel<2, K3, 2, true, U, TR>), a.grid, SPRS_CO_HEAD(a), r, t, (const double *)nullptr, partTT, partTR, status, \
+                         a.ncols, Fin{}, a.tail2, a.g2_last, pro, v, (const double *)nullptr, s_out);
+    SPRS_CHAIN_SHAPES(SPRS_CO4F)
+#undef SPRS_CO4F
+    SPRS_HIP_TRY(c, hipGetLastError());
+    return SPRS_OK;
+}
+
+int launch_chain_off_k2f(const sprs_csr *A, const SpmvRoute &rt, const BicgK1<double, double, false> &pro, const double *v_old, const double *p, const double *r,
+                         double *p_out, double *v_out, const double *r0, double *partB, const int *status) {
+    sprs_ctx *c = A->ctx;
+    const ChainOffArgs a = chain_off_args(A, rt);
+    typedef BicgK1<double, double, false> K1;
+#define SPRS_CO2F(U, TR)                                                                                                \
+    if (a.ul == U && a.tri == TR)                                                                                       \
+        SPRS_LAUNCH_SPMV(c, (spmv_chain_off_kernel<3, K1, 1, false, U, TR>), a.grid, SPRS_CO_HEAD(a), v_old, v_out, r0, partB, (double *)nullptr, status, \
+                         a.ncols, Fin{}, a.tail2, a.g2_last, pro, p, r, p_out);
+    SPRS_CHAIN_SHAPES(SPRS_CO2F)
+#undef SPRS_CO2F
+    SPRS_HIP_TRY(c, hipGetLastError());
+    return SPRS_OK;
+}
+
+}
diff --git a/sprsolve_amd/csrc/spmv_dict.hip b/sprsolve_amd/csrc/spmv_dict.hip
--- a/sprsolve_amd/csrc/spmv_dict.hip
+++ b/sprsolve_amd/csrc/spmv_dict.hip
@@ -573,7 +573,7 @@
 
 template <class MakeLeft>
 static int build_chain_plan(sprs_csr *A, sprs_chain_plan &CP, const std::vector<BlkDescHost2> &wd, const std::vector<uint8_t> &flag, int UL,
-                            const int32_t *off, const double *val, MakeLeft &&make_left) {
+                            const int32_t *off, const double *val, int chb, MakeLeft &&make_left) {
     sprs_ctx *c = A->ctx;
     const int nw = (int)wd.size();
     const int64_t Pf = off[UL - 1];
@@ -584,7 +584,7 @@
     SPRS_CHAIN_SHAPES(SPRS_CH_HAS)
 #undef SPRS_CH_HAS
     if (!shape_ok) return SPRS_OK;
-    const int CHR = CH_B * 2 * WAVE;
+    const int CHR = chb * 2 * WAVE;
     const int NN = UL - 2, TC = NN / 2;
     bool tri = (off[1 + TC] & 1) == 0;
     for (int t = 0; t < NN && tri; ++t) {
@@ -601,7 +601,7 @@
         int e = j + 1;
         while (e < nw && flag[(size_t)e] && wd[(size_t)e].ra == wd[(size_t)e - 1].ra + 2 * WAVE) ++e;
         flagged += e - j;
-        for (int b = j; b + CH_B <= e; b += CH_B) {
+        for (int b = j; b + chb <= e; b += chb) {
             const int64_t ra = wd[(size_t)b].ra;
             if (ra - Pf < 0 || ra + CHR + Pf > A->ncols) continue;
             tb.push_back(b);
@@ -667,8 +667,8 @@
                     const int32_t ra = wd[(size_t)b0].ra;
                     const int32_t ra_next = next[(size_t)ti] >= 0 ? wd[(size_t)tb[(size_t)next[(size_t)ti]]].ra : (int32_t)(ra + Pf);
                     tiles.push_back(b0); tiles.push_back(ra); tiles.push_back(ra_next); tiles.push_back(0);
-                    for (int qb = 0; qb < CH_B; ++qb) in_chain[(size_t)(b0 + qb)] = 1;
-                    covered += CH_B;
+                    for (int qb = 0; qb < chb; ++qb) in_chain[(size_t)(b0 + qb)] = 1;
+                    covered += chb;
                 }
                 ++n_seg;
             }
@@ -757,8 +757,8 @@
     TILE_TRY(hipStreamSynchronize(c->stream));
     if (!val_tab)
         for (int j = 0; j < nw; ++j) if ((int64_t)wd[(size_t)j].pa + 2 * WAVE * UL + 2 > A->nnz) flag[(size_t)j] = 0;
-    if (CP && c->spmv_chain != 0 && val_tab) {
-        if (const int st = build_chain_plan(A, *CP, wd, flag, UL, TP.off, TP.val, make_left)) { drop(); return st; }
+    if (CP && c->spmv_chain != 0) {
+        if (const int st = build_chain_plan(A, *CP, wd, flag, UL, TP.off, TP.val, val_tab ? CH_B : CHO_B, make_left)) { drop(); return st; }
     }
     std::vector<int32_t> starts;
     std::vector<char> in_tile((size_t)nw, 0);
@@ -1100,7 +1100,7 @@
                         left.push_back(2 * j);
                         if (2 * j + 1 < nb64) left.push_back(2 * j + 1);
                     }
-                })) { cleanup2(); free_dict(A); return st; }
+                }, A->dist ? nullptr : &D->chain_off)) { cleanup2(); free_dict(A); return st; }
             if (D->tile_off.n_tile == 0) { (void)hipFree(D->owide_desc); D->owide_desc = nullptr; D->n_owide = 0; }
             tr.lap("    tile plan (offset stream)");
         }
@@ -1120,7 +1120,8 @@
     for (void *q : {(void *)D->idx_code, (void *)D->pair_code, (void *)D->off_tab, (void *)D->pair_off, D->pair_val, D->wide_desc, D->off_desc, (void *)D->wide_order, (void *)D->off_order,
                     (void *)D->tile_pair.list, (void *)D->tile_pair.xstart, (void *)D->tile_pair.left,
                     (void *)D->tile_off.list, (void *)D->tile_off.xstart, (void *)D->tile_off.left, D->owide_desc,
-                    (void *)D->chain_pair.tiles, (void *)D->chain_pair.segs, (void *)D->chain_pair.xstart, (void *)D->chain_pair.left, D->rowval})
+                    (void *)D->chain_pair.tiles, (void *)D->chain_pair.segs, (void *)D->chain_pair.xstart, (void *)D->chain_pair.left,
+                    (void *)D->chain_off.tiles, (void *)D->chain_off.segs, (void *)D->chain_off.xstart, (void *)D->chain_off.left, D->rowval})
         if (q) (void)hipFree(q);
     delete D;
     A->dict = nullptr;
diff --git a/sprsolve_amd/csrc/spmv_dict_dev.hpp b/sprsolve_amd/csrc/spmv_dict_dev.hpp
--- a/sprsolve_amd/csrc/spmv_dict_dev.hpp
+++ b/sprsolve_amd/csrc/spmv_dict_dev.hpp
@@ -25,10 +25,13 @@
     int s;
     T uu;
     T rv;
+    T ow;
     uint32_t wc[2];
     int di[2];
     T vv[PAIR ? 1 : ITEMS];
 };
+
+struct XMem { static constexpr bool FUSED = false; };
 
 struct NoScale { static constexpr bool ON = false; };
 template <class T>
@@ -37,14 +40,16 @@
     Real<T> scale;
 };
 
-template <class T, int DOT, bool CONJX, bool PAIR, bool WV, class EW = NoScale>
+template <class T, int DOT, bool CONJX, bool PAIR, bool WV, class EW = NoScale, class XS = XMem>
 __device__ __forceinline__ void dict_walk(int n_rowblk, int xcd_chunk, const BlkDesc *__restrict__ desc, const int32_t *__restrict__ order,
                                           const int32_t *__restrict__ row_ptr, const uint8_t *__restrict__ code,
                                           const T *__restrict__ val, const T *__restrict__ x, T *__restrict__ y, const T *__restrict__ u,
                                           const V2d *__restrict__ tail2, int g2_last,
                                           const PairEnt<T> *s_pair, const int32_t *s_off8, uint32_t (*s_c)[(nnz_cap<T>::value + 3 + CPAD + 3) / 4],
-                                          T *s_v, int s_v_stride, T &d0, T &d1, const T *__restrict__ rowval = nullptr, const EW ew = EW{}) {
+                                          T *s_v, int s_v_stride, T &d0, T &d1, const T *__restrict__ rowval = nullptr, const EW ew = EW{},
+                                          const XS xs = XS{}, T *__restrict__ own = nullptr) {
     static_assert(!EW::ON || DOT == 1, "the scaled operand is also the dot operand: u == x");
+    static_assert(!XS::FUSED || (!EW::ON && !CONJX && !PAIR), "the fused operand: f64 offset codes, plain gathers");
     constexpr int CAP = nnz_cap<T>::value;
     constexpr bool RV = PAIR && is_complex<T>::value;
     constexpr int ITEMS = CAP / WAVE;
@@ -90,7 +95,12 @@
         const int rcl = r < L.rb ? r : L.rb - 1;
         if (uni) L.s = L.pa + (rcl - L.ra) * L.ulen;
         else L.s = *reinterpret_cast<const int32_t *>(reinterpret_cast<const char *>(row_ptr) + (uint32_t)rcl * 4u);
-        if (DOT != 0) L.uu = *reinterpret_cast<const T *>(reinterpret_cast<const char *>(u) + (uint32_t)rcl * (uint32_t)sizeof(T));
+        if constexpr (XS::FUSED) {
+            L.ow = xs.ld1((uint32_t)rcl * (uint32_t)sizeof(T));
+            if (DOT != 0) L.uu = u != nullptr ? *reinterpret_cast<const T *>(reinterpret_cast<const char *>(u) + (uint32_t)rcl * (uint32_t)sizeof(T)) : L.ow;
+        } else {
+            if (DOT != 0) L.uu = *reinterpret_cast<const T *>(reinterpret_cast<const char *>(u) + (uint32_t)rcl * (uint32_t)sizeof(T));
+        }
         if constexpr (RV) L.rv = *reinterpret_cast<const T *>(reinterpret_cast<const char *>(rowval) + (uint32_t)rcl * (uint32_t)sizeof(T));
         const int shift = L.pa & 3;
         const int nd = max((shift + (uni ? L.ulen : L.nn) + 3) >> 2, 1);
@@ -149,8 +159,10 @@
     bool c_uni = false;
     T c_uu = szero<T>();
     [[maybe_unused]] T c_rv = szero<T>();
+    [[maybe_unused]] T c_ow = szero<T>();
     auto adopt = [&](const Loads &L) {
         if constexpr (RV) c_rv = L.rv;
+        if constexpr (XS::FUSED) c_ow = L.ow;
         const int r = L.ra + lane;
         c_ra = L.ra; c_rb = L.rb; c_shift = L.pa & 3; c_uni = L.ulen > 0;
         if constexpr (WV) c_vsh = L.pa & 1;
@@ -206,7 +218,8 @@
                 }
                 else { off8 = s_off8[cd]; av[t] = vs[(WV ? c_vsh : 0) + kb + t]; }
                 const uint32_t vo = valid ? r8 + (uint32_t)off8 : 0u;
-                xg[t] = *reinterpret_cast<const T *>(xbytes + vo);
+                if constexpr (XS::FUSED) xg[t] = xs.ld1(vo);
+                else xg[t] = *reinterpret_cast<const T *>(xbytes + vo);
             }
             __builtin_amdgcn_sched_barrier(0);
 #pragma unroll
@@ -219,6 +232,7 @@
         }
         if (r < c_rb) {
             *reinterpret_cast<T *>(reinterpret_cast<char *>(y) + r8) = acc;
+            if constexpr (XS::FUSED) { if (own != nullptr) *reinterpret_cast<T *>(reinterpret_cast<char *>(own) + r8) = c_ow; }
             if constexpr (EW::ON) c_uu = smulr(c_uu, ew.scale);
             if (DOT == 1) d0 = sadd(d0, smul(sconj(c_uu), acc));
             if (DOT == 2) { d0 = sadd(d0, smul(sconj(acc), acc)); d1 = sadd(d1, smul(sconj(acc), c_uu)); }
@@ -595,7 +609,7 @@
 
 #define SPRS_TILE_SHAPES(X) X(7, 1, 1) X(5, 1, 1) X(5, 0, 0) X(3, 0, 0) X(3, 1, 1) X(7, 0, 0)
 #define SPRS_TILE_SHAPES_WIDE(X) X(7, 1, 1) X(5, 1, 1) X(5, 0, 0) X(7, 0, 0)
-constexpr int CH_B = 16;
+constexpr int CH_B = 16, CHO_B = 8;
 #define SPRS_CHAIN_SHAPES(X) X(7, true) X(7, false) X(5, true) X(5, false) X(3, true)
 }
 
```

Result: no change. 830.8 (median of 2 runs) (-0.9%).
